# xaskasdf/ntransformer

Measured on AMD Instinct MI355X. Metric: decode tokens/sec (Llama-3.1-8B Q8_0 class, resident weights, greedy, batch 1), higher is better.
Workload: dtype f32; 1 GPU; Llama-3.1-8B-shaped Q8_0 GGUF tensors (seed 20260925), resident in HBM, 16-token prompt, greedy decode; ctx=4096, replicas=1, hipgraph=True

## Files before the change

include/ntk_engine.h:

```cpp
#ifndef NTK_ENGINE_H
#define NTK_ENGINE_H

#include "ntk.h"

#if defined(__GNUC__)
#pragma GCC visibility push(default)
#endif
#ifdef __cplusplus
extern "C" {
#endif

int ntk_rope_kv_store(float* q, const float* k, const float* v, const int* positions, int seq_len, int n_heads, int n_kv_heads, int head_dim,
                      float theta_base, float freq_scale, int interleaved, void* k_cache, void* v_cache, int start_pos, int max_seq, void* stream);
typedef struct ntk_gemv_seg {
    const void* W;
    float*      y;
    int         rows;
    int         dtype;
} ntk_gemv_seg;

int ntk_gemv_fused(const ntk_gemv_seg* segs, int nseg, const float* x, int in_features, const float* norm_w,
                   float eps, const float* resid, int silu_pair, void* stream);

size_t ntk_q8l_bytes(int rows, int in_features);
int ntk_q8l_pack(void* dst, const void* raw, int rows, int in_features, void* stream);
int ntk_q8l_unpack(void* raw, const void* packed, int rows, int in_features, void* stream);

size_t ntk_rp_bytes(int dtype, int rows, int in_features);
int ntk_rp_pack(void* dst, const void* raw, int rows, int in_features, int dtype, void* stream);
int ntk_rp_dequant(float* out, const void* rp, int rows, int in_features, int dtype, void* stream);
int ntk_rp_unpack(void* raw, const void* rp, int rows, int in_features, int dtype, void* stream);
int ntk_gemv_rp(float* y, const void* rp, const float* x, int out_features, int in_features, int weight_dtype, void* stream);
int ntk_gemv_rp_fused(const ntk_gemv_seg* segs, int nseg, const float* x, int in_features, const float* norm_w, float eps,
                      const float* resid, int silu_pair, void* stream);
int ntk_debug_rp_prologue(uint8_t* out, const float* x, const float* norm_w, float eps, int in_features, int nsub, int nwaves, void* stream);
int ntk_debug_mfma_i8_probe(int* D, const int8_t* A, const int8_t* B, void* stream);

int ntk_attention_decode_fused(float* output, const float* q, const float* k, const float* v, void* k_cache,
                               void* v_cache, const int* d_pos, const float* inv_freq, int n_heads, int n_kv_heads,
                               int head_dim, int max_seq, float scale, float theta_base, float freq_scale,
                               void* stream);

size_t ntk_attention_split_scratch_bytes(int n_heads, int head_dim, int nsplit);
int ntk_attention_decode_split(float* output, const float* q, const float* k, const float* v, void* k_cache,
                               void* v_cache, const int* d_pos, const float* inv_freq, int n_heads, int n_kv_heads,
                               int head_dim, int max_seq, float scale, float theta_base, float freq_scale, int nsplit,
                               float* scratch, void* stream);
int ntk_attention_split_scratch_init(float* scratch, int n_heads, void* stream);
int ntk_attention_decode_split_merged(float* output, const float* q, const float* k, const float* v, void* k_cache,
                                      void* v_cache, const int* d_pos, const float* inv_freq, int n_heads, int n_kv_heads,
                                      int head_dim, int max_seq, float scale, float theta_base, float freq_scale, int nsplit,
                                      float* scratch, void* stream);

#define NTK_ATTN_BATCH_MAX 16
typedef struct ntk_kv_batch {
    void* k[NTK_ATTN_BATCH_MAX];
    void* v[NTK_ATTN_BATCH_MAX];
} ntk_kv_batch;
int ntk_attention_decode_batch(float* output, const float* q, const float* k, const float* v, const ntk_kv_batch* caches, const int* positions,
                               int n_rows, const float* inv_freq, int n_heads, int n_kv_heads, int head_dim, int max_seq, float scale,
                               float theta_base, float freq_scale, int nsplit, float* scratch, void* stream);

typedef struct ntk_kv_segments {
    int   n_seg;
    int   row0[NTK_ATTN_BATCH_MAX];
    int   n_rows[NTK_ATTN_BATCH_MAX];
    int   start_pos[NTK_ATTN_BATCH_MAX];
    void* k[NTK_ATTN_BATCH_MAX];
    void* v[NTK_ATTN_BATCH_MAX];
} ntk_kv_segments;
int ntk_kv_segments_validate(const ntk_kv_segments* segs, int total_rows, int max_seq);
int ntk_rope_kv_store_segments(float* q, const float* k, const float* v, const ntk_kv_segments* segs, int n_heads, int n_kv_heads, int head_dim,
                               float theta_base, float freq_scale, int interleaved, int max_seq, void* stream);
int ntk_attention_prefill_segments(float* output, const float* Q, const ntk_kv_segments* segs, int n_heads, int n_kv_heads, int head_dim, int max_seq,
                                   float scale, void* stream);

size_t ntk_kv_q8_cache_bytes(int max_seq, int n_kv_heads, int head_dim);
int ntk_kv_store_q8(void* k_cache, void* v_cache, const float* k, const float* v, int seq_len, int n_kv_heads, int head_dim, int start_pos,
                    int max_seq, void* stream);
int ntk_rope_kv_store_q8(float* q, const float* k, const float* v, const int* positions, int seq_len, int n_heads, int n_kv_heads, int head_dim,
                         float theta_base, float freq_scale, int interleaved, void* k_cache, void* v_cache, int start_pos, int max_seq,
                         void* stream);
int ntk_attention_decode_q8(float* output, const float* q, const float* k, const float* v, void* k_cache, void* v_cache, const int* d_pos,
                            const float* inv_freq, int n_heads, int n_kv_heads, int head_dim, int max_seq, float scale, float theta_base,
                            float freq_scale, int nsplit, float* scratch, void* stream);
int ntk_kv_dequant_q8_f16(void* k_f16, void* v_f16, const void* k_cache, const void* v_cache, int n_rows, int n_kv_heads, int head_dim,
                          int max_seq, void* stream);
int ntk_attention_decode_q8_batch(float* output, const float* q, const float* k, const float* v, const ntk_kv_batch* caches, const int* positions,
                                  int n_rows, const float* inv_freq, int n_heads, int n_kv_heads, int head_dim, int max_seq, float scale,
                                  float theta_base, float freq_scale, int nsplit, float* scratch, void* stream);

int ntk_kv_shift(uint16_t* k_cache, uint16_t* v_cache, int n_layers, int max_seq, int n_kv_heads, int head_dim, int src0, int dst0, int n_rows,
                 const float* inv_freq, float theta_base, float freq_scale, int interleaved, void* stream);
int ntk_kv_shift_q8(void* k_cache_q8, void* v_cache_q8, int n_layers, int max_seq, int n_kv_heads, int head_dim, int src0, int dst0, int n_rows,
                    const float* inv_freq, float theta_base, float freq_scale, int interleaved, void* stream);

int ntk_debug_gemv_fused_form(const ntk_gemv_seg* segs, int nseg, const float* x, int in_features, const float* norm_w, float eps,
                              const float* resid, int silu_pair, int integer_activations, void* stream);

size_t   ntk_tp_comm_bytes(size_t max_floats);
void*    ntk_tp_comm_alloc(size_t bytes);
int      ntk_tp_comm_reset(void* comm, void* stream);
float*   ntk_tp_slot(void* comm, size_t max_floats, unsigned call_index);
int      ntk_tp_allreduce_add(float* hidden, void* const* peers, int rank, int world, size_t max_floats, unsigned call_index, int n, void* stream);
int      ntk_tp_advance_epoch(void* comm, void* stream);
unsigned ntk_tp_error(void* comm);
int      ntk_ipc_export(void* devptr, void* handle64);
int      ntk_ipc_open(const void* handle64, void** devptr);
int      ntk_ipc_close(void* devptr);

int ntk_gemm_quant(float* Y, const void* W, const float* X, int n_tokens, int out_features, int in_features,
                   int weight_dtype, const float* resid, void* stream);

typedef struct ntk_gemm_partials {
    const float* part[3];
    float*       y[3];
    int          rows[3];
    int          nseg, n_tokens, nsplit;
} ntk_gemm_partials;
typedef struct ntk_gemm_desc {
    const ntk_gemv_seg* segs;
    int                 nseg;
    const float*        X;
    int                 n_tokens, in_features;
    const float*        resid;
    void*               workspace;
    size_t              workspace_bytes;
    int                 reuse_x;
    const float*        row_max;
    ntk_gemm_partials*  partials;
    int                 weights_repacked;
    int                 full_form;
} ntk_gemm_desc;
size_t ntk_gemm_quant_workspace_bytes(int in_features, int out_features);
int ntk_gemm_quant_f16(const ntk_gemm_desc* desc, void* stream);
int ntk_reduce_rmsnorm_rowmax(float* hidden, const ntk_gemm_partials* partials, const float* weight, float eps, float* x_out, float* row_max,
                              float* zero_tokens, void* stream);
int ntk_reduce_silu_mul_rowmax(float* output, const ntk_gemm_partials* partials, float* row_max, void* stream);
int ntk_rmsnorm_rowmax(float* output, const float* input, const float* weight, int n_tokens, int hidden_size, float eps, float* row_max,
                       float* zero_tokens, void* stream);
int ntk_silu_mul_rowmax(float* output, const float* gate, const float* up, int n_tokens, int width, float* row_max, void* stream);
int ntk_gemm_prepare_x(const float* X, int n_tokens, int in_features, void* workspace, void* stream);
int ntk_rmsnorm_prepare_x(float* output, const float* input, const float* weight, int n_tokens, int hidden_size, float eps, void* workspace, void* stream);
int ntk_reduce_rmsnorm_prepare_x(float* hidden, const ntk_gemm_partials* partials, const float* weight, float eps, float* x_out, void* workspace, void* stream);
int ntk_silu_mul_prepare_x(float* output, const float* gate, const float* up, int n_tokens, int width, void* workspace, void* stream);
int ntk_reduce_silu_mul_prepare_x(float* output, const ntk_gemm_partials* partials, void* workspace, void* stream);

int ntk_embed_rows(float* out, const void* table, const int* tokens, int n_tokens, int hidden, int dtype,
                   void* stream);

int ntk_argmax(const float* logits, int n, int* d_out_token, int* h_mirror, float* scratch, void* stream);

int ntk_logprob_rows(const float* logits, int n_rows, int vocab, int ld, const int* targets, float* logprob, int* top1, void* stream);

size_t ntk_sample_scratch_bytes(int n);
int ntk_sample_top_k(float* logits, int n, const int* d_recent, int n_recent, float repeat_penalty, float temperature,
                     int top_k, float top_p, float r, int* d_out_token, int* h_mirror, void* scratch, void* stream);
int ntk_repeat_penalty(float* logits, int n, const int* d_recent, int n_recent, float repeat_penalty, void* stream);

#define NTK_SAMPLE_ROWS_MAX 16
typedef struct ntk_sample_rows {
    float temperature[NTK_SAMPLE_ROWS_MAX], top_p[NTK_SAMPLE_ROWS_MAX], repeat_penalty[NTK_SAMPLE_ROWS_MAX], r[NTK_SAMPLE_ROWS_MAX];
    int   top_k[NTK_SAMPLE_ROWS_MAX], n_recent[NTK_SAMPLE_ROWS_MAX];
} ntk_sample_rows;
size_t ntk_sample_rows_scratch_bytes(int n_rows, int vocab);
int ntk_sample_rows_top_k(float* logits, int n_rows, int vocab, int ld, const int* d_recent, int recent_ld, const ntk_sample_rows* rows, int* d_out,
                          int* h_mirror, void* scratch, void* stream);

int ntk_argmax_advance(const float* logits, int n, int* d_out_token, int* h_mirror, unsigned long long* h_ring4, int* d_pos,
                       float* scratch, void* stream);

int ntk_debug_sclk(unsigned long long* d_out2, void* stream);
int ntk_debug_sclk_begin(unsigned* d_flag, unsigned long long* d_out2, void* side_stream);
int ntk_debug_sclk_end(unsigned* d_flag, void* other_stream);

void ntk_debug_malloc_budget(long long bytes);

int ntk_advance_pos(int* d_pos, void* stream);

#ifdef __cplusplus
}
#endif
#if defined(__GNUC__)
#pragma GCC visibility pop
#endif
#endif
```

ntransformer_amd/_lib.py:

```python
from __future__ import annotations

import ctypes as C
import os

_HERE = os.path.dirname(os.path.abspath(__file__))
LIB_PATH = os.environ.get("NTK_LIB_PATH") or os.path.join(_HERE, "libntransformer_hip.so")

NTK_OK = 0
_STATUS = {0: "ok", -1: "unsupported dtype", -2: "bad shape", -3: "HIP launch/runtime error", -4: "misaligned pointer",
           -5: "null pointer", -6: "no usable GPU", -7: "out of memory", -8: "I/O error", -9: "malformed GGUF"}


class NtkError(RuntimeError):
    def __init__(self, status: int, what: str = ""):
        self.status = status
        super().__init__("ntk status %d (%s)%s" % (status, _STATUS.get(status, "?"), (": " + what) if what else ""))


def check(status: int, what: str = "") -> None:
    if status != NTK_OK:
        raise NtkError(status, what)


class KvBatch(C.Structure):
    _fields_ = [("k", C.c_void_p * 16), ("v", C.c_void_p * 16)]


class KvSegments(C.Structure):
    _fields_ = [("n_seg", C.c_int), ("row0", C.c_int * 16), ("n_rows", C.c_int * 16), ("start_pos", C.c_int * 16), ("k", C.c_void_p * 16),
                ("v", C.c_void_p * 16)]


class SampleRows(C.Structure):
    _fields_ = [("temperature", C.c_float * 16), ("top_p", C.c_float * 16), ("repeat_penalty", C.c_float * 16), ("r", C.c_float * 16),
                ("top_k", C.c_int * 16), ("n_recent", C.c_int * 16)]


class GemvSeg(C.Structure):
    _fields_ = [("W", C.c_void_p), ("y", C.c_void_p), ("rows", C.c_int), ("dtype", C.c_int)]


class GemmPartials(C.Structure):
    _fields_ = [("part", C.c_void_p * 3), ("y", C.c_void_p * 3), ("rows", C.c_int * 3), ("nseg", C.c_int), ("n_tokens", C.c_int), ("nsplit", C.c_int)]


class GemmDesc(C.Structure):
    _fields_ = [("segs", C.POINTER(GemvSeg)), ("nseg", C.c_int), ("X", C.c_void_p), ("n_tokens", C.c_int), ("in_features", C.c_int), ("resid", C.c_void_p),
                ("workspace", C.c_void_p), ("workspace_bytes", C.c_size_t), ("reuse_x", C.c_int), ("row_max", C.c_void_p),
                ("partials", C.POINTER(GemmPartials)), ("weights_repacked", C.c_int), ("full_form", C.c_int)]


_lib = None


def lib() -> C.CDLL:
    global _lib
    if _lib is not None:
        return _lib
    if not os.path.exists(LIB_PATH):
        raise ImportError("%s is missing: run `python -c 'import __graft_entry__ as g; g.build()'` "
                          "(hipcc --offload-arch=gfx950); there is no CPU fallback" % LIB_PATH)
    L = C.CDLL(LIB_PATH, mode=C.RTLD_GLOBAL)
    vp, i, f, sz = C.c_void_p, C.c_int, C.c_float, C.c_size_t
    sig = {
        "ntk_abi_version": (i, []),
        "ntk_status_string": (C.c_char_p, [i]),
        "ntk_row_bytes": (sz, [i, C.c_int64]),
        "ntk_device_count": (i, []),
        "ntk_device_init": (i, [i]),
        "ntk_device_name": (i, [C.c_char_p, sz]),
        "ntk_device_mem_info": (i, [C.POINTER(sz), C.POINTER(sz)]),
        "ntk_stream": (vp, [i]),
        "ntk_stream_synchronize": (i, [vp]),
        "ntk_device_synchronize": (i, []),
        "ntk_event_create": (vp, []),
        "ntk_event_destroy": (i, [vp]),
        "ntk_event_record": (i, [vp, vp]),
        "ntk_event_synchronize": (i, [vp]),
        "ntk_event_elapsed_ms": (i, [vp, vp, C.POINTER(f)]),
        "nt_hip_malloc": (vp, [sz]), "nt_hip_free": (None, [vp]),
        "nt_hip_memcpy_h2d": (None, [vp, vp, sz]), "nt_hip_memcpy_d2h": (None, [vp, vp, sz]),
        "nt_hip_memcpy_d2d": (None, [vp, vp, sz]), "nt_hip_memset": (None, [vp, i, sz]),
        "nt_hip_malloc_host": (vp, [sz]), "nt_hip_free_host": (None, [vp]),
        "ntk_memcpy_h2d_async": (i, [vp, vp, sz, vp]), "ntk_memcpy_d2h_async": (i, [vp, vp, sz, vp]),
        "nt_cuda_malloc": (vp, [sz]), "nt_cuda_free": (None, [vp]),
        "nt_cuda_memcpy_h2d": (None, [vp, vp, sz]), "nt_cuda_memcpy_d2h": (None, [vp, vp, sz]),
        "nt_cuda_memcpy_d2d": (None, [vp, vp, sz]), "nt_cuda_memset": (None, [vp, i, sz]),
        "nt_cuda_malloc_host": (vp, [sz]), "nt_cuda_free_host": (None, [vp]),
        "ntk_rmsnorm": (i, [vp, vp, vp, i, i, f, vp]),
        "ntk_rmsnorm_f16": (i, [vp, vp, vp, i, i, f, vp]),
        "ntk_rope": (i, [vp, vp, vp, i, i, i, i, i, f, f, i, vp]),
        "ntk_softmax": (i, [vp, vp, i, i, vp]),
        "ntk_masked_softmax": (i, [vp, vp, vp, i, i, vp]),
        "ntk_gemv": (i, [vp, vp, vp, i, i, i, vp]),
        "ntk_gemv_add": (i, [vp, vp, vp, i, i, i, vp]),
        "ntk_gemm_f32": (i, [vp, vp, vp, i, i, i, vp]),
        "ntk_silu_mul": (i, [vp, vp, vp, i, vp]),
        "ntk_rmsnorm_rowmax": (i, [vp, vp, vp, i, i, f, vp, vp, vp]),
        "ntk_rope_kv_store": (i, [vp, vp, vp, vp, i, i, i, i, f, f, i, vp, vp, i, i, vp]),
        "ntk_silu_mul_rowmax": (i, [vp, vp, vp, i, i, vp, vp]),
        "ntk_add_bias": (i, [vp, vp, i, vp]),
        "ntk_attention_decode": (i, [vp, vp, vp, vp, i, i, i, i, i, f, vp]),
        "ntk_attention_prefill": (i, [vp, vp, vp, vp, i, i, i, i, i, i, f, vp]),
        "ntk_copy_to_kv_cache": (i, [vp, vp, vp, vp, i, i, i, i, i, vp]),
        "ntk_add": (i, [vp, vp, vp, i, vp]),
        "ntk_add_inplace": (i, [vp, vp, i, vp]),
        "ntk_copy": (i, [vp, vp, i, vp]),
        "ntk_cosine_similarity": (i, [vp, vp, vp, i, vp]),
        "ntk_gemv_fused": (i, [C.POINTER(GemvSeg), i, vp, i, vp, f, vp, i, vp]),
        "ntk_debug_gemv_fused_form": (i, [C.POINTER(GemvSeg), i, vp, i, vp, f, vp, i, i, vp]),
        "ntk_q8l_bytes": (sz, [i, i]),
        "ntk_q8l_pack": (i, [vp, vp, i, i, vp]),
        "ntk_q8l_unpack": (i, [vp, vp, i, i, vp]),
        "ntk_rp_bytes": (sz, [i, i, i]),
        "ntk_rp_pack": (i, [vp, vp, i, i, i, vp]),
        "ntk_rp_dequant": (i, [vp, vp, i, i, i, vp]),
        "ntk_rp_unpack": (i, [vp, vp, i, i, i, vp]),
        "ntk_gemv_rp": (i, [vp, vp, vp, i, i, i, vp]),
        "ntk_gemv_rp_fused": (i, [C.POINTER(GemvSeg), i, vp, i, vp, f, vp, i, vp]),
        "ntk_debug_rp_prologue": (i, [vp, vp, vp, f, i, i, i, vp]),
        "ntk_debug_mfma_i8_probe": (i, [vp, vp, vp, vp]),
        "ntk_gemm_quant": (i, [vp, vp, vp, i, i, i, i, vp, vp]),
        "ntk_attention_decode_split": (i, [vp, vp, vp, vp, vp, vp, vp, vp, i, i, i, i, f, f, f, i, vp, vp]),
        "ntk_attention_split_scratch_bytes": (C.c_size_t, [i, i, i]),
        "ntk_attention_split_scratch_init": (i, [vp, i, vp]),
        "ntk_attention_decode_split_merged": (i, [vp, vp, vp, vp, vp, vp, vp, vp, i, i, i, i, f, f, f, i, vp, vp]),
        "ntk_attention_decode_fused": (i, [vp, vp, vp, vp, vp, vp, vp, vp, i, i, i, i, f, f, f, vp]),
        "ntk_attention_decode_batch": (i, [vp, vp, vp, vp, vp, vp, i, vp, i, i, i, i, f, f, f, i, vp, vp]),
        "ntk_kv_segments_validate": (i, [vp, i, i]),
        "ntk_rope_kv_store_segments": (i, [vp, vp, vp, vp, i, i, i, f, f, i, i, vp]),
        "ntk_attention_prefill_segments": (i, [vp, vp, vp, i, i, i, i, f, vp]),
        "ntk_kv_q8_cache_bytes": (C.c_size_t, [i, i, i]),
        "ntk_kv_store_q8": (i, [vp, vp, vp, vp, i, i, i, i, i, vp]),
        "ntk_rope_kv_store_q8": (i, [vp, vp, vp, vp, i, i, i, i, f, f, i, vp, vp, i, i, vp]),
        "ntk_attention_decode_q8": (i, [vp, vp, vp, vp, vp, vp, vp, vp, i, i, i, i, f, f, f, i, vp, vp]),
        "ntk_kv_dequant_q8_f16": (i, [vp, vp, vp, vp, i, i, i, i, vp]),
        "ntk_attention_decode_q8_batch": (i, [vp, vp, vp, vp, vp, vp, i, vp, i, i, i, i, f, f, f, i, vp, vp]),
        "ntk_kv_shift": (i, [vp, vp, i, i, i, i, i, i, i, vp, f, f, i, vp]),
        "ntk_kv_shift_q8": (i, [vp, vp, i, i, i, i, i, i, i, vp, f, f, i, vp]),
        "ntk_embed_rows": (i, [vp, vp, vp, i, i, i, vp]),
        "ntk_argmax": (i, [vp, i, vp, vp, vp, vp]),
        "ntk_logprob_rows": (i, [vp, i, i, i, vp, vp, vp, vp]),
        "ntk_sample_rows_scratch_bytes": (C.c_size_t, [i, i]),
        "ntk_sample_rows_top_k": (i, [vp, i, i, i, vp, i, C.POINTER(SampleRows), vp, vp, vp, vp]),
        "ntk_advance_pos": (i, [vp, vp]),
        "ntk_debug_sclk": (i, [vp, vp]),
        "ntk_debug_sclk_begin": (i, [vp, vp, vp]),
        "ntk_debug_sclk_end": (i, [vp, vp]),
    }
    for name, (res, args) in sig.items():
        fn = getattr(L, name)
        fn.restype = res
        fn.argtypes = args
    _lib = L
    return L


EXPORTS_NTK_H = None
```

ntransformer_amd/csrc/engine/capi.cpp:

```cpp
#include "../../../include/ntransformer.h"
#include "../../../include/ntk_engine.h"
#include "engine.h"

#include <cstdlib>
#include <cstring>
#include <new>
#include <thread>

using nt::Engine;

namespace {
Engine* E(nt_engine_t e) { return static_cast<Engine*>(e); }
nt::SynthSpec to_spec(const nt_synth_spec& s) {
    nt::SynthSpec o;
    o.hidden = s.hidden; o.inter = s.inter; o.layers = s.layers; o.heads = s.heads; o.kv_heads = s.kv_heads;
    o.vocab = s.vocab; o.ctx = s.ctx; o.eps = s.eps; o.theta = s.theta; o.bos = s.bos; o.eos = s.eos;
    o.mix = s.mix ? s.mix : "Q8_0";
    o.seed = s.seed;
    return o;
}
int threads_or_default(int n) {
    if (n > 0) return n;
    const int h = (int)std::thread::hardware_concurrency();
    return h > 0 ? h : 8;
}
}

extern "C" {

nt_engine_t nt_engine_create(void) { return new (std::nothrow) Engine(); }
void nt_engine_destroy(nt_engine_t e) { delete E(e); }

int nt_engine_load(nt_engine_t e, const char* path) { return nt_engine_load_ex(e, path, 4096); }

int nt_engine_load_ex(nt_engine_t e, const char* path, int max_context) {
    if (!e || !path) return NTK_E_NULL;
    try { return E(e)->load(path, max_context > 0 ? max_context : 4096); } catch (...) { return NTK_E_NOMEM; }
}

int nt_engine_load_synthetic(nt_engine_t e, const nt_synth_spec* spec, int max_context) {
    if (!e || !spec) return NTK_E_NULL;
    try { return E(e)->load_synthetic(to_spec(*spec), max_context > 0 ? max_context : 4096); } catch (...) { return NTK_E_NOMEM; }
}

int nt_engine_load_shared(nt_engine_t e, nt_engine_t src, int max_context) {
    if (!e || !src || e == src) return NTK_E_NULL;
    try { return E(e)->load_shared(*E(src), max_context > 0 ? max_context : 4096); } catch (...) { return NTK_E_NOMEM; }
}

int nt_engine_set_option(nt_engine_t e, const char* key, const char* value) {
    if (!e || !key || !value) return NTK_E_NULL;
    const bool on = atoi(value) != 0;
    const std::string k = key;
    if (k == "fused") E(e)->options().fused = on;
    else if (k == "graph") E(e)->options().graph = on;
    else if (k == "batched_prefill") { E(e)->options().batched_prefill = on; E(e)->model().set_batched_prefill(on); }
    else if (k == "device_sampling") E(e)->options().device_sampling = on;
    else if (k == "f16_prefill" || k == "bf16_prefill") E(e)->model().set_bf16_prefill(on);
    else if (k == "fuse_attention") { const int rc = E(e)->model().set_fuse_attention(on); if (rc != NTK_OK) E(e)->set_error(E(e)->model().error()); return rc; }
    else if (k == "kv_cache") {
        const int rc = E(e)->loaded() ? (E(e)->set_error("kv_cache must be set before the model is loaded"), NTK_E_SHAPE) : E(e)->model().set_kv_cache(value);
        if (rc != NTK_OK && !E(e)->loaded()) E(e)->set_error(E(e)->model().error());
        return rc;
    }
    else if (k == "sequences") {
        const int rc = E(e)->loaded() ? (E(e)->set_error("sequences must be set before the model is loaded"), NTK_E_SHAPE) : E(e)->model().set_sequences(atoi(value));
        if (rc != NTK_OK && !E(e)->loaded()) E(e)->set_error(E(e)->model().error());
        return rc;
    }
    else if (k == "batch_kv_q8") {
        const std::string v = value;
        if (v != "0" && v != "1") { E(e)->set_error("batch_kv_q8 must be 0 or 1"); return NTK_E_SHAPE; }
        const int rc = E(e)->loaded() ? (E(e)->set_error("batch_kv_q8 must be set before the model is loaded"), NTK_E_SHAPE) : E(e)->model().set_batch_kv_q8(on);
        if (rc != NTK_OK && !E(e)->loaded()) E(e)->set_error(E(e)->model().error());
        return rc;
    }
    else if (k == "batch_prefill") {
        const std::string v = value;
        if (v != "0" && v != "1") { E(e)->set_error("batch_prefill must be 0 or 1"); return NTK_E_SHAPE; }
        E(e)->options().batch_prefill = on;
    }
    else if (k == "context_shift") {
        const std::string v = value;
        if (v != "0" && v != "1") { E(e)->set_error("context_shift must be 0 or 1"); return NTK_E_SHAPE; }
        E(e)->options().context_shift = on;
    }
    else if (k == "context_keep") {
        char* end = nullptr;
        const long n = strtol(value, &end, 10);
        if (end == value || *end != 0 || n < 0 || n > 0x7FFFFFFF) { E(e)->set_error("context_keep must be an integer >= 0"); return NTK_E_SHAPE; }
        E(e)->options().context_keep = (int)n;
    }
    else if (k == "prefill_row_max") E(e)->model().set_prefill_row_max(on);
    else if (k == "prefill_fused_split") E(e)->model().set_prefill_fused_split(on);
    else if (k == "attention_merge") return E(e)->model().set_attention_merge(on);
    else if (k == "repack") return E(e)->model().set_repack(atoi(value));
    else if (k == "persistent") { E(e)->options().persistent = on; E(e)->model().set_persistent(atoi(value)); }
    else if (k == "score_rows") {
        const int rc = E(e)->model().set_score_rows(atoi(value));
        if (rc != NTK_OK) E(e)->set_error(E(e)->model().error());
        return rc;
    }
    else if (k == "synth_threads") E(e)->options().synth_threads = atoi(value);
    else return NTK_E_SHAPE;
    return NTK_OK;
}

const char* nt_engine_last_error(nt_engine_t e) { return e ? E(e)->error().c_str() : "null engine"; }

void nt_gen_params_default(nt_gen_params* p) {
    if (!p) return;
    const nt::GenerateConfig d;
    p->max_tokens = d.max_tokens; p->temperature = d.temperature; p->top_k = d.top_k; p->top_p = d.top_p;
    p->repeat_penalty = d.repeat_penalty; p->repeat_window = d.repeat_window; p->seed = d.seed; p->stop_at_eos = 1;
}

char* nt_engine_generate(nt_engine_t e, const char* prompt, int max_tokens, float temperature, int top_k, float top_p) {
    if (!e || !prompt || !E(e)->loaded()) return nullptr;
    try {
        nt::GenerateConfig c;
        c.max_tokens = max_tokens; c.temperature = temperature; c.top_k = top_k; c.top_p = top_p;
        c.verbose = false;
        const std::string out = E(e)->generate(prompt, c);
        char* r = static_cast<char*>(malloc(out.size() + 1));
        if (!r) return nullptr;
        memcpy(r, out.c_str(), out.size() + 1);
        return r;
    } catch (...) { return nullptr; }
}
void nt_free(char* p) { free(p); }

int nt_engine_vocab_size(nt_engine_t e) { return e && E(e)->loaded() ? E(e)->model().config().vocab_size : -1; }
int nt_engine_n_layers(nt_engine_t e) { return e && E(e)->loaded() ? E(e)->model().config().n_layers : -1; }
int nt_engine_hidden_size(nt_engine_t e) { return e && E(e)->loaded() ? E(e)->model().config().hidden_size : -1; }
int nt_engine_max_context(nt_engine_t e) { return e && E(e)->loaded() ? E(e)->model().config().max_seq_len : -1; }

int nt_engine_generate_tokens(nt_engine_t e, const int* prompt, int n_prompt, const nt_gen_params* p, int* out, int out_cap) {
    if (!e || !prompt || !p || (!out && out_cap > 0)) return NTK_E_NULL;
    if (n_prompt <= 0) return NTK_E_SHAPE;
    try {
        nt::GenerateConfig c;
        c.max_tokens = p->max_tokens; c.temperature = p->temperature; c.top_k = p->top_k; c.top_p = p->top_p;
        c.repeat_penalty = p->repeat_penalty; c.repeat_window = p->repeat_window; c.seed = p->seed;
        std::vector<int> gen;
        const int rc = E(e)->generate_tokens(std::vector<int>(prompt, prompt + n_prompt), c, gen, p->stop_at_eos != 0);
        if (rc != NTK_OK) return rc;
        const int n = (int)std::min<size_t>(gen.size(), (size_t)out_cap);
        for (int i = 0; i < n; ++i) out[i] = gen[i];
        return n;
    } catch (...) { return NTK_E_NOMEM; }
}

int nt_engine_last_stats(nt_engine_t e, nt_stats* o) {
    if (!e || !o) return NTK_E_NULL;
    const nt::Stats& s = E(e)->last_stats();
    o->prompt_tokens = s.prompt_tokens; o->gen_tokens = s.gen_tokens; o->prefill_ms = s.prefill_ms;
    o->decode_ms = s.decode_ms; o->decode_tok_s = s.decode_tok_s();
    return NTK_OK;
}

int nt_engine_forward(nt_engine_t e, const int* tokens, int n, int start_pos, float* logits_out) {
    if (!e || !tokens || !logits_out) return NTK_E_NULL;
    if (!E(e)->loaded()) return NTK_E_NULL;
    float* d = E(e)->model().forward(tokens, n, start_pos);
    if (!d) return NTK_E_LAUNCH;
    return E(e)->model().copy_logits(logits_out);
}

int nt_engine_seq_forward(nt_engine_t e, int slot, const int* tokens, int n, int start_pos, float* logits_out) {
    if (!e || !tokens || !logits_out) return NTK_E_NULL;
    if (!E(e)->loaded()) return NTK_E_NULL;
    if (slot < 0 || slot >= E(e)->model().sequences()) { E(e)->set_error("seq_forward: no such sequence slot"); return NTK_E_SHAPE; }
    float* d = E(e)->model().forward(tokens, n, start_pos, slot);
    if (!d) { E(e)->set_error(E(e)->model().error()); return NTK_E_LAUNCH; }
    return E(e)->model().copy_logits(logits_out);
}

int nt_engine_decode_batch(nt_engine_t e, const int* slots, const int* tokens, const int* positions, int n, float* logits_out, int* next_out) {
    if (!e || !E(e)->loaded()) return NTK_E_NULL;
    try {
        const int rc = E(e)->model().decode_batch(slots, tokens, positions, n, logits_out, next_out);
        if (rc != NTK_OK) E(e)->set_error(E(e)->model().error());
        return rc;
    } catch (...) { return NTK_E_NOMEM; }
}

int nt_engine_forward_batch(nt_engine_t e, const int* slots, const int* tokens, const int* lens, const int* start_pos, int n, float* logits_out,
                            int* next_out) {
    if (!e || !E(e)->loaded()) return NTK_E_NULL;
    try {
        E(e)->model().set_batched_prefill(E(e)->options().batched_prefill);
        const int rc = E(e)->model().forward_batch(slots, tokens, lens, start_pos, n, logits_out, next_out);
        if (rc != NTK_OK) E(e)->set_error(E(e)->model().error());
        return rc;
    } catch (...) { return NTK_E_NOMEM; }
}

int nt_forward_batch_validate(const int* slots, const int* lens, const int* start_pos, int n, int sequences, int max_seq) {
    return nt::Model::validate_forward_batch(slots, lens, start_pos, n, sequences, max_seq, nullptr);
}

int nt_engine_generate_batch(nt_engine_t e, const int* const* prompts, const int* prompt_lens, int n, const nt_gen_params* p, int* out, int out_stride,
                             int* out_counts) {
    if (!e || !prompts || !prompt_lens || !p || !out || !out_counts) return NTK_E_NULL;
    try { return E(e)->generate_batch(prompts, prompt_lens, n, *p, out, out_stride, out_counts); } catch (...) { return NTK_E_NOMEM; }
}

int nt_engine_decode_batch_sample(nt_engine_t e, const int* slots, const int* tokens, const int* positions, int n, const nt_gen_params* params,
                                  const int* const* recent, const int* n_recent, const float* r, float* logits_out, int* next_out) {
    if (!e || !E(e)->loaded()) return NTK_E_NULL;
    try { return E(e)->decode_batch_sample(slots, tokens, positions, n, params, recent, n_recent, r, logits_out, next_out); } catch (...) { return NTK_E_NOMEM; }
}

int nt_engine_generate_batch_ex(nt_engine_t e, const int* const* prompts, const int* prompt_lens, int n, const nt_gen_params* params, int* out, int out_stride,
                                int* out_counts) {
    if (!e || !prompts || !prompt_lens || !params || !out || !out_counts) return NTK_E_NULL;
    try { return E(e)->generate_batch_ex(prompts, prompt_lens, n, params, out, out_stride, out_counts); } catch (...) { return NTK_E_NOMEM; }
}

int nt_engine_kv_shift(nt_engine_t e, int slot, int keep, int discard, int n_past) {
    if (!e || !E(e)->loaded()) return NTK_E_NULL;
    try {
        const int rc = E(e)->model().kv_shift(slot, keep, discard, n_past);
        if (rc < 0) E(e)->set_error(E(e)->model().error());
        return rc;
    } catch (...) { return NTK_E_NOMEM; }
}

int nt_engine_kv_copy(nt_engine_t e, int src_slot, int dst_slot, int pos0, int n) {
    if (!e || !E(e)->loaded()) return NTK_E_NULL;
    try {
        const int rc = E(e)->model().kv_copy(src_slot, dst_slot, pos0, n);
        if (rc < 0) E(e)->set_error(E(e)->model().error());
        return rc;
    } catch (...) { return NTK_E_NOMEM; }
}

int nt_kv_shift_validate(int slot, int keep, int discard, int n_past, int sequences, int max_seq) {
    return nt::Model::validate_kv_shift(slot, keep, discard, n_past, sequences, max_seq, nullptr);
}
int nt_kv_copy_validate(int src_slot, int dst_slot, int pos0, int n, int sequences, int max_seq) {
    return nt::Model::validate_kv_copy(src_slot, dst_slot, pos0, n, sequences, max_seq, nullptr);
}
int nt_context_shift_discard(int n_past, int keep) { return nt::Model::context_shift_discard(n_past, keep); }

int nt_batch_validate(const int* slots, const int* tokens, const int* positions, int n, int sequences, int max_seq, int vocab) {
    return nt::Model::validate_batch(slots, tokens, positions, n, sequences, max_seq, vocab, nullptr);
}

int nt_engine_score_tokens(nt_engine_t e, const int* tokens, const int* targets, int n, int start_pos, float* logprob_out, int* top1_out) {
    if (!e || !tokens || !targets || !logprob_out) return NTK_E_NULL;
    try {
        const int rc = E(e)->score(tokens, targets, n, start_pos, logprob_out, top1_out);
        if (rc != NTK_OK) return rc;
        int scored = 0;
        for (int i = 0; i < n; ++i) scored += targets[i] >= 0;
        return scored;
    } catch (...) { return NTK_E_NOMEM; }
}

int nt_engine_decode_fused(nt_engine_t e, int token, int pos, int use_graph, float* logits_out) {
    if (!e || !logits_out || !E(e)->loaded()) return NTK_E_NULL;
    nt::Model& m = E(e)->model();
    if (pos < 0 || pos >= m.config().max_seq_len) return NTK_E_SHAPE;
    m.set_device_pos(pos);
    int rc = m.set_device_token(token);
    if (rc != NTK_OK) return rc;
    rc = m.decode_step_fused(false, use_graph != 0);
    if (rc != NTK_OK) return rc;
    rc = m.copy_logits(logits_out);
    if (rc != NTK_OK) return rc;
    return m.check_persistent();
}

int nt_engine_debug_run_layers(nt_engine_t e, const float* hidden_in, int n_tokens, int start_pos, int first_layer, int n_layers, int mode,
                               float* hidden_out) {
    if (!e || !E(e)->loaded()) return NTK_E_NULL;
    return E(e)->model().debug_run_layers(hidden_in, n_tokens, start_pos, first_layer, n_layers, mode, hidden_out);
}
int nt_engine_debug_kv_read(nt_engine_t e, int layer, int pos0, int n, uint16_t* k_out, uint16_t* v_out) {
    if (!e || !E(e)->loaded()) return NTK_E_NULL;
    return E(e)->model().debug_kv(layer, pos0, n, k_out, v_out, false);
}
int nt_engine_debug_kv_read_slot(nt_engine_t e, int slot, int layer, int pos0, int n, uint16_t* k_out, uint16_t* v_out) {
    if (!e || !E(e)->loaded()) return NTK_E_NULL;
    return E(e)->model().debug_kv(layer, pos0, n, k_out, v_out, false, slot);
}
int nt_engine_debug_kv_write(nt_engine_t e, int layer, int pos0, int n, const uint16_t* k, const uint16_t* v) {
    if (!e || !E(e)->loaded()) return NTK_E_NULL;
    return E(e)->model().debug_kv(layer, pos0, n, const_cast<uint16_t*>(k), const_cast<uint16_t*>(v), true);
}
int nt_engine_debug_kv_write_slot(nt_engine_t e, int slot, int layer, int pos0, int n, const uint16_t* k, const uint16_t* v) {
    if (!e || !E(e)->loaded()) return NTK_E_NULL;
    return E(e)->model().debug_kv(layer, pos0, n, const_cast<uint16_t*>(k), const_cast<uint16_t*>(v), true, slot);
}
int nt_engine_debug_kv_inputs_capture(nt_engine_t e, int layer) {
    if (!e || !E(e)->loaded()) return NTK_E_NULL;
    return E(e)->model().debug_kv_inputs_capture(layer);
}
int nt_engine_debug_kv_inputs_read(nt_engine_t e, int n, float* k_out, float* v_out) {
    if (!e || !E(e)->loaded()) return NTK_E_NULL;
    return E(e)->model().debug_kv_inputs_read(n, k_out, v_out);
}
int nt_engine_debug_kv_read_q8(nt_engine_t e, int layer, int pos0, int n, void* k_blocks, void* v_blocks) {
    if (!e || !E(e)->loaded()) return NTK_E_NULL;
    return E(e)->model().debug_kv_q8(layer, pos0, n, static_cast<uint8_t*>(k_blocks), static_cast<uint8_t*>(v_blocks), false);
}
int nt_engine_debug_kv_write_q8(nt_engine_t e, int layer, int pos0, int n, const void* k_blocks, const void* v_blocks) {
    if (!e || !E(e)->loaded()) return NTK_E_NULL;
    return E(e)->model().debug_kv_q8(layer, pos0, n, static_cast<uint8_t*>(const_cast<void*>(k_blocks)), static_cast<uint8_t*>(const_cast<void*>(v_blocks)), true);
}
int nt_engine_debug_kv_read_q8_slot(nt_engine_t e, int slot, int layer, int pos0, int n, void* k_blocks, void* v_blocks) {
    if (!e || !E(e)->loaded()) return NTK_E_NULL;
    return E(e)->model().debug_kv_q8(layer, pos0, n, static_cast<uint8_t*>(k_blocks), static_cast<uint8_t*>(v_blocks), false, slot);
}
int nt_engine_debug_kv_write_q8_slot(nt_engine_t e, int slot, int layer, int pos0, int n, const void* k_blocks, const void* v_blocks) {
    if (!e || !E(e)->loaded()) return NTK_E_NULL;
    return E(e)->model().debug_kv_q8(layer, pos0, n, static_cast<uint8_t*>(const_cast<void*>(k_blocks)), static_cast<uint8_t*>(const_cast<void*>(v_blocks)), true, slot);
}

void* nt_engine_persistent_plan(nt_engine_t e) { return e && E(e)->loaded() ? E(e)->model().persistent_plan() : nullptr; }
int nt_engine_persistent_kind(nt_engine_t e) { return e && E(e)->loaded() ? E(e)->model().persistent_kind() : 0; }
const char* nt_engine_decode_path(nt_engine_t e) { return e && E(e)->loaded() ? E(e)->model().decode_path() : ""; }

int nt_engine_tp_configure(nt_engine_t e, int rank, int world) { return e ? E(e)->model().tp_configure(rank, world) : NTK_E_NULL; }
int nt_engine_tp_export(nt_engine_t e, void* handle64, void** raw) {
    if (!e || !E(e)->loaded()) return NTK_E_NULL;
    return E(e)->model().tp_export(handle64, raw);
}
int nt_engine_tp_connect(nt_engine_t e, const void* handles, void* const* raws) {
    if (!e || !E(e)->loaded()) return NTK_E_NULL;
    return E(e)->model().tp_connect(handles, raws);
}
unsigned nt_engine_tp_error(nt_engine_t e) { return e && E(e)->loaded() ? E(e)->model().tp_error() : 0u; }
int nt_tp_slice_columns(void* dst, const void* src, int dtype, int64_t out_features, int64_t in_features, int rank, int world) {
    return nt::Model::slice_columns(dst, src, dtype, out_features, in_features, rank, world);
}

int nt_engine_decode_greedy_steps(nt_engine_t e, int token, int pos, int n, int* out) {
    if (!e || !E(e)->loaded()) return NTK_E_NULL;
    return E(e)->decode_greedy_steps(token, pos, n, out);
}

int nt_engine_profile_token(nt_engine_t e, int token, int pos, int coarse, float* ms4, int* calls4) {
    if (!e || !ms4 || !calls4 || !E(e)->loaded()) return NTK_E_NULL;
    nt::Model& m = E(e)->model();
    if (pos < 0 || pos >= m.config().max_seq_len) return NTK_E_SHAPE;
    m.set_device_pos(pos);
    const int rc = m.set_device_token(token);
    if (rc != NTK_OK) return rc;
    return m.profile_token(ms4, calls4, coarse != 0);
}

int nt_engine_tokenize(nt_engine_t e, const char* text, int add_bos, int* out, int cap) {
    if (!e || !text || !E(e)->loaded()) return NTK_E_NULL;
    const std::vector<int> ids = E(e)->tokenizer().encode(text, add_bos != 0);
    for (int i = 0; i < (int)ids.size() && i < cap; ++i) out[i] = ids[i];
    return (int)ids.size();
}

int nt_engine_detokenize(nt_engine_t e, const int* ids, int n, char* out, int cap) {
    if (!e || !ids || !E(e)->loaded()) return NTK_E_NULL;
    const std::string s = E(e)->tokenizer().decode(std::vector<int>(ids, ids + n));
    if (out && cap > 0) {
        const size_t k = std::min<size_t>(s.size(), (size_t)cap - 1);
        memcpy(out, s.data(), k);
        out[k] = 0;
    }
    return (int)s.size();
}

uint64_t nt_engine_bytes_per_token(nt_engine_t e, int pos) { return e && E(e)->loaded() ? E(e)->model().bytes_per_token(pos) : 0; }
uint64_t nt_engine_kv_cache_bytes(nt_engine_t e) { return e && E(e)->loaded() ? E(e)->model().kv_cache_bytes() : 0; }
uint64_t nt_engine_weight_bytes(nt_engine_t e) { return e && E(e)->loaded() ? E(e)->model().weight_bytes() : 0; }
uint64_t nt_engine_resident_weight_bytes(nt_engine_t e) { return e && E(e)->loaded() ? E(e)->model().resident_weight_bytes() : 0; }
uint64_t nt_engine_repacked_bytes(nt_engine_t e) { return e && E(e)->loaded() ? E(e)->model().repack_bytes() : 0; }
// ... 137 lines not shown
```

ntransformer_amd/csrc/engine/model.cpp:

```cpp
#include "model_impl.h"
#include <thread>

namespace nt {

Model::~Model() { free_all(); }

void Model::drop_graphs(int slot) {
    for (auto& row : graphs_)
        for (int k = 0; k <= kAttnRegimes; ++k) {
            if (slot >= 0 && k != slot) continue;
            if (row[k]) (void)hipGraphExecDestroy(reinterpret_cast<hipGraphExec_t>(row[k]));
            row[k] = nullptr;
        }
}

void Model::free_all() {
    drop_graphs();
    destroy_persistent_plan();
    persistent_on_ = false;
    for (int r = 0; r < 8; ++r) {
        if (tp_peer_opened_[r] && tp_peers_[r]) (void)ntk_ipc_close(tp_peers_[r]);
        tp_peers_[r] = nullptr;
        tp_peer_opened_[r] = false;
    }
    tp_connected_ = false;
    tp_comm_ = nullptr;
    tp_call_ = 0;
    if (own_stream_ && stream_) (void)hipStreamDestroy(static_cast<hipStream_t>(stream_));
    own_stream_ = false;
    stream_ = nullptr;
    for (void* p : allocs_) nt_hip_free(p);
    allocs_.clear();
    auto free_host = [](auto*& p) { if (p) nt_hip_free_host(p); p = nullptr; };
    free_host(h_token_); free_host(h_ring_); free_host(h_recent_); free_host(h_batch_recent_); free_host(h_batch_next_);
    sample_scratch_ = gemm_ws_ = gemm_ws2_ = nullptr;
    d_recent_ = nullptr;
    attn_sync_ = nullptr;
    shares_weights_ = false;
    layers_.clear();
    token_embd_ = output_norm_ = output_ = DevTensor();
    weight_bytes_ = repack_bytes_ = raw_freed_bytes_ = 0;
    raw_scratch_ = nullptr; raw_scratch_bytes_ = raw_cursor_ = 0; raw_err_ = 0;
    repack_done_ = output_tied_ = false;
    host_pos_ = attn_regime_ = 0;
    kv_.reset();
    batch_logits_ = batch_logprob_ = batch_attn_scratch_ = nullptr; batch_in_ = batch_next_ = batch_recent_ = nullptr; batch_sample_scratch_ = nullptr;
    kv_capture_ = nullptr; kv_capture_layer_ = -1; kv_capture_T_ = 0;
    hidden_ = residual_ = workspace_ = logits_ = argmax_scratch_ = rope_inv_freq_ = attn_scratch_ = row_max_ = nullptr;
    positions_ = tokens_dev_ = d_pos_ = d_token_ = nullptr;
    score_logits_ = score_logprob_ = nullptr; score_targets_ = score_top1_ = nullptr; score_cap_ = 0;
    score_ws_ = nullptr; score_ws_bytes_ = 0;
}

int Model::share_weights(const Model& src, int max_context) {
    if (&src == this) { err_ = "share_weights: a model cannot share its own weights"; return NTK_E_NULL; }
    free_all();
    if (src.layers_.empty()) { err_ = "share_weights: the source model is not loaded"; return NTK_E_NULL; }
    if (src.tp_world_ != 1 || src.shares_weights_) {
        err_ = "share_weights: the source must hold whole tensors of its own (no tensor parallelism, not itself a sharing sequence)";
        return NTK_E_SHAPE;
    }
    cfg_ = src.cfg_;
    cfg_full_ = src.cfg_;
    if (max_context > 0) cfg_.max_seq_len = max_context;
    vocab_ = src.vocab_;
    layers_ = src.layers_;
    token_embd_ = src.token_embd_; output_norm_ = src.output_norm_; output_ = src.output_;
    output_tied_ = src.output_tied_;
    weight_bytes_ = src.weight_bytes_;
    repack_ = src.repack_; repack_wanted_ = src.repack_; repack_done_ = true;
    repack_bytes_ = 0;
    shares_weights_ = true;
    if (src.raw_freed_bytes_ > 0 && src.raw_scratch_bytes_ > 0) {
        void* d = nt_hip_malloc(src.raw_scratch_bytes_);
        if (!d) { err_ = "share_weights: no device memory for the unpack scratch"; free_all(); return NTK_E_NOMEM; }
        allocs_.push_back(d);
        raw_scratch_ = d; raw_scratch_bytes_ = src.raw_scratch_bytes_;
        raw_freed_bytes_ = src.raw_freed_bytes_;
    }
    int rc = own_stream();
    if (rc == NTK_OK) rc = alloc_buffers();
    if (rc != NTK_OK) free_all();
    return rc;
}

int Model::set_attention_merge(bool on) {
    if (on == attn_merge_) return NTK_OK;
    if (!layers_.empty()) {
        NT_TRY(sync());
        drop_graphs();
    }
    attn_merge_ = on;
    return NTK_OK;
}

int Model::set_repack(int level) {
    level = level < 0 ? 0 : level > 3 ? 3 : level;
    if (shares_weights_) { err_ = "set_repack: this sequence shares another model's tensors"; return NTK_E_SHAPE; }
    repack_wanted_ = level;
    if (layers_.empty()) { repack_ = level; return NTK_OK; }
    if (level == 3) level = 2;
    if (level == repack_) return NTK_OK;
    NT_TRY(sync());
    drop_graphs();
    int rc = NTK_OK;
    if (level < 2 && raw_freed_bytes_ > 0) rc = restore_raw_all();
    if (rc == NTK_OK && level > 0 && !repack_done_) {
        rc = repack_all();
        if (rc == NTK_E_NOMEM) { fprintf(stderr, "warning: decode repack incomplete (device memory): the rest stays on the raw path\n"); rc = NTK_OK; err_.clear(); }
    }
    if (rc != NTK_OK) { err_ = std::string("set_repack: ") + ntk_status_string(rc); return rc; }
    repack_ = level;
    if (level == 2) {
        destroy_persistent_plan();
        persistent_on_ = false;
        rc = drop_raw_all();
    }
    return rc;
}

uint64_t Model::bytes_per_token(int pos) const {
    uint64_t b = 0;
    for (const auto& L : layers_)
        for (auto m : kLayerMatrices) b += (L.*m).nbytes;
    b += output_.nbytes;
    b += (uint64_t)(2 * cfg_.n_layers + 1) * cfg_.hidden_size * 4;
    const uint64_t kv_row = kv_.row_bytes();
    b += 2ull * cfg_.n_layers * kv_row * (uint64_t)(pos + 1) + 2ull * cfg_.n_layers * kv_row;
    b += ntk_row_bytes(token_embd_.dtype, cfg_.hidden_size);
    return b;
}

int Model::set_device_token(int token) {
    if (token < 0 || token >= cfg_.vocab_size) { err_ = "token id out of range"; return NTK_E_SHAPE; }
    *h_token_ = token;
    return ntk_memcpy_h2d_async(d_token_, h_token_, 4, stream_);
}
int Model::set_device_pos(int pos) {
    host_pos_ = pos;
    NT_TRY(ntk_memcpy_h2d_async(d_pos_, &pos, 4, stream_));
    NT_TRY(ntk_stream_synchronize(stream_));
    if (h_ring_) memset(h_ring_, 0, 64);
    return NTK_OK;
}
int Model::sync() { return ntk_stream_synchronize(stream_); }
int Model::host_token() const { return *h_token_; }
int Model::copy_logits(float* host) {
    NT_TRY(ntk_memcpy_d2h_async(host, logits_, (size_t)cfg_.vocab_size * 4, stream_));
    return ntk_stream_synchronize(stream_);
}

int Model::sample_on_device(const int* recent, int n_recent, float repeat_penalty, float temperature, int top_k, float top_p, float r) {
    if (!sample_scratch_ || !d_recent_ || !h_recent_) return NTK_E_NOMEM;
    if (n_recent > kRecentCap) { recent += n_recent - kRecentCap; n_recent = kRecentCap; }
    void* s = stream_;
    if (repeat_penalty > 1.0f && n_recent > 0) {
        memcpy(h_recent_, recent, (size_t)n_recent * 4);
        NT_TRY(ntk_memcpy_h2d_async(d_recent_, h_recent_, (size_t)n_recent * 4, s));
    } else {
        n_recent = 0;
    }
    if (temperature <= 0.0f) {
        NT_TRY(ntk_repeat_penalty(logits_, cfg_.vocab_size, d_recent_, n_recent, repeat_penalty, s));
        return ntk_argmax(logits_, cfg_.vocab_size, d_token_, h_token_, argmax_scratch_, s);
    }
    return ntk_sample_top_k(logits_, cfg_.vocab_size, d_recent_, n_recent, repeat_penalty, temperature, top_k, top_p, r, d_token_,
                            h_token_, sample_scratch_, s);
}

int Model::wait_token(int pos, int* token) {
    volatile unsigned long long* slot = h_ring_ + (pos & 3);
    const unsigned want = (unsigned)(pos + 1);
    for (unsigned spins = 0;; ++spins) {
        const unsigned long long v = *slot;
        if ((unsigned)(v >> 32) == want) { *token = (int)(unsigned)v; return NTK_OK; }
#if defined(__x86_64__) || defined(__i386__)
        __builtin_ia32_pause();
#else
        std::this_thread::yield();
#endif
        if ((spins & 0xFFFFu) == 0xFFFFu) {
            const auto now = std::chrono::steady_clock::now();
            if (spins == 0xFFFFu) wait_t0_ = now;
            else if (std::chrono::duration<double>(now - wait_t0_).count() > 2.0) break;
        }
    }
    static bool warned = false;
    if (!warned) { warned = true; fprintf(stderr, "warning: the pinned token ring was not seen updating for 2 s (host memory not coherent with a running kernel?); falling back to a stream synchronisation per token\n"); }
    NT_TRY(ntk_stream_synchronize(stream_));
    const unsigned long long v = *slot;
    if ((unsigned)(v >> 32) != want) { err_ = "decode step finished without publishing its token"; return NTK_E_LAUNCH; }
    *token = (int)(unsigned)v;
    return NTK_OK;
}

int Model::set_sequences(int n) {
    if (n < 1 || n > kMaxSequences) { err_ = "sequences must lie in 1 .. " + std::to_string(kMaxSequences); return NTK_E_SHAPE; }
    sequences_ = n;
    return NTK_OK;
}

int Model::set_batch_kv_q8(bool on) {
    if (!layers_.empty()) { err_ = "batch_kv_q8 must be set before the model is loaded"; return NTK_E_SHAPE; }
    batch_kv_q8_ = on;
    return NTK_OK;
}

int Model::set_kv_cache(const std::string& kind) {
    if (kind != "f16" && kind != "q8_0") { err_ = "kv_cache: unknown format '" + kind + "' (f16 or q8_0)"; return NTK_E_DTYPE; }
    if (!layers_.empty()) { err_ = "kv_cache must be set before the model is loaded"; return NTK_E_SHAPE; }
    const bool q8 = kind == "q8_0";
    if (q8 && fuse_attention_) { err_ = "kv_cache=q8_0 is not supported with the attention-inside-Wo launch (fuse_attention)"; return NTK_E_SHAPE; }
    kv_q8_ = q8;
    return NTK_OK;
}

int Model::set_fuse_attention(bool on) {
    if (on && kv_q8_) { err_ = "fuse_attention (attention inside the Wo launch) is not supported with kv_cache=q8_0"; return NTK_E_SHAPE; }
    fuse_attention_ = on;
    return NTK_OK;
}

bool Model::use_persistent_now() const {
    return persistent_plan_ && persistent_on_ && attn_regime_ == 0 && !prof_;
}

void Model::set_persistent(int level) {
    const bool on = level != 0;
    persistent_on_ = false;
    persistent_wanted_ = level;
    if (on && !experiments_built()) fprintf(stderr, "note: the persistent token kernels are built by experiments/Makefile only (experiments/libntransformer_hip_exp.so); this library decodes with fused launches\n");
    if (persistent_plan_ && persistent_kind_ != (level == 2 ? 2 : 1)) {
        (void)sync();
        destroy_persistent_plan();
    }
    if (!on || tp_world_ != 1 || layers_.empty()) return;
    if (kv_q8_) { fprintf(stderr, "note: the persistent token kernels read the F16 KV cache; kv_cache=q8_0 decodes with fused launches\n"); return; }
    if (raw_freed_bytes_ > 0) (void)set_repack(1);
    if (!persistent_plan_) (void)build_persistent_plan(level == 2 ? 2 : 1);
    persistent_on_ = persistent_plan_ != nullptr;
}

const char* Model::decode_path() const {
    if (persistent_plan_ && persistent_on_ && persistent_kind_ == 2)
        return attn_regime_ == 0 ? "persistent layer engine (1 launch per token: loader / consumer waves, granule hand-offs; fused launches beyond the single-pass attention regime)"
                                 : "fused (5 launches/layer; persistent layer engine below the split-attention regime)";
    if (persistent_plan_ && persistent_on_)
        return attn_regime_ == 0 ? "persistent (1 launch per token in the single-pass attention regime, fused launches beyond)"
                                 : "fused (5 launches/layer; persistent below the split-attention regime)";
    return "fused (5 launches/layer)";
}

int Model::check_persistent() {
    NT_TRY(check_tp());
    return check_experiments();
}

Model::Views Model::views(int T) const {
    const size_t qd = (size_t)T * cfg_.n_heads * cfg_.head_dim, kvd = (size_t)T * cfg_.n_kv_heads * cfg_.head_dim;
    float* const q = workspace_;
    return {q, q + qd, q + qd + kvd, q + qd + 2 * kvd, workspace_, workspace_ + (size_t)T * cfg_.intermediate_size};
}

int Model::init_device() {
    const char* e = getenv("NTK_DEVICE");
    const int st = ntk_device_init(e ? atoi(e) : 0);
    if (st != NTK_OK) err_ = "no usable GPU (HIP device init failed)";
    return st;
}

int Model::own_stream() {
    hipStream_t own = nullptr;
    if (hipStreamCreateWithFlags(&own, hipStreamNonBlocking) != hipSuccess) { err_ = "stream creation failed"; return NTK_E_LAUNCH; }
    stream_ = own;
    own_stream_ = true;
    return NTK_OK;
}

}
```

ntransformer_amd/csrc/engine/model.h:

```cpp
#pragma once
#include <algorithm>
#include <array>
#include <chrono>
#include <cstdint>
#include <string>
#include <vector>
#include "gguf.h"
#include "kv_cache.h"
#include "synth.h"

struct ntk_sample_rows;
struct ntk_kv_segments;

struct ihipGraphExec_t;

namespace nt {

struct DevTensor {
    void* ptr = nullptr;
    int dtype = 0;
    int64_t in_f = 0, out_f = 0;
    size_t nbytes = 0;
    void* rp = nullptr;
    size_t rp_bytes = 0;
};

struct LayerWeights {
    DevTensor attn_norm, wq, wk, wv, wo, ffn_norm, w_gate, w_up, w_down;
};
inline constexpr std::array<DevTensor LayerWeights::*, 7> kLayerMatrices = {&LayerWeights::wq, &LayerWeights::wk, &LayerWeights::wv, &LayerWeights::wo,
                                                                            &LayerWeights::w_gate, &LayerWeights::w_up, &LayerWeights::w_down};

enum Shard { WHOLE, ROWS, COLS };

class Model {
public:
    Model() = default;
    ~Model();
    Model(const Model&) = delete;
    Model& operator=(const Model&) = delete;

    int load(const std::string& gguf_path, int max_context);
    int load_synthetic(const SynthSpec& spec, int max_context, int nthreads);
    int share_weights(const Model& src, int max_context);

    float* forward(const int* tokens, int seq_len, int start_pos, int slot = 0);

    int score(const int* tokens, const int* targets, int seq_len, int start_pos, float* logprob_out, int* top1_out, int slot = 0);

    static constexpr int kMaxSequences = 16;
    int set_sequences(int n);
    int sequences() const { return sequences_; }
    int set_batch_kv_q8(bool on);
    bool batch_kv_q8() const { return batch_kv_q8_; }
    int decode_batch(const int* slots, const int* tokens, const int* positions, int B, float* logits_out, int* next_out);
    static constexpr int kMaxRecent = 4096;
    int decode_batch_sample(const int* slots, const int* tokens, const int* positions, int B, const ntk_sample_rows& rows, const int* const* recent,
                            float* logits_out, float* const* row_logits, int* next_out);
    static int validate_batch(const int* slots, const int* tokens, const int* positions, int B, int sequences, int max_seq, int vocab, std::string* why);
    int forward_batch(const int* slots, const int* tokens_flat, const int* lens, const int* start_pos, int n, float* logits_out, int* next_out);
    static int validate_forward_batch(const int* slots, const int* lens, const int* start_pos, int n, int sequences, int max_seq, std::string* why);
    int kv_shift(int slot, int keep, int discard, int n_past);
    int kv_copy(int src_slot, int dst_slot, int pos0, int n);
    static int validate_kv_shift(int slot, int keep, int discard, int n_past, int sequences, int max_seq, std::string* why);
    static int validate_kv_copy(int src_slot, int dst_slot, int pos0, int n, int sequences, int max_seq, std::string* why);
    static int context_shift_discard(int n_past, int keep) { return std::max(1, (n_past - keep) / 2); }
    int set_score_rows(int rows);

    int decode_step_fused(bool greedy, bool use_graph);
    int set_device_token(int token);
    int set_device_pos(int pos);
    static constexpr int kAttnRegimes = 3;
    static int attention_regime(int pos, int head_dim) {
        if (pos < 544) return 0;
        return pos < (head_dim == 128 ? 3072 : 16384) ? 1 : 2;
    }
    static int attention_splits(int regime, int head_dim) { return regime <= 1 ? 8 : head_dim == 128 ? 32 : 16; }
    static constexpr int kMaxAttnSplits = 32;
    void pick_attention_regime();
    int sync();
    int host_token() const;
    int wait_token(int pos, int* token);
    float* logits_ptr() { return logits_; }
    int copy_logits(float* host);
    int sample_on_device(const int* recent, int n_recent, float repeat_penalty, float temperature, int top_k, float top_p, float r);
    static bool device_sampler_supports(float temperature, int top_k, int vocab) {
        return temperature <= 0.0f || (top_k > 0 && top_k <= 64 && top_k < vocab && vocab <= 131072);
    }

    const ModelConfig& config() const { return cfg_; }
    const GgufVocab& vocab() const { return vocab_; }
    const std::string& error() const { return err_; }
    uint64_t weight_bytes() const { return weight_bytes_; }
    uint64_t bytes_per_token(int pos) const;
    void set_batched_prefill(bool on) { batched_prefill_ = on; }
    void set_persistent(int level);
    int persistent_kind() const { return persistent_plan_ ? persistent_kind_ : 0; }
    int set_fuse_attention(bool on);
    int set_kv_cache(const std::string& kind);
    bool kv_q8() const { return kv_q8_; }
    static int kv_q8_splits(int regime) { return regime == 0 ? 4 : regime == 1 ? 16 : 32; }
    uint64_t kv_cache_bytes() const { return kv_.bytes(); }
    int debug_kv_inputs_capture(int layer);
    int debug_kv_inputs_read(int n, float* k, float* v);
    int debug_kv_q8(int layer, int pos0, int n, uint8_t* k_blocks, uint8_t* v_blocks, bool write, int slot = 0);
    void set_prefill_row_max(bool on) { prefill_row_max_ = on; }
    void set_prefill_fused_split(bool on) { prefill_fused_split_ = on; }
    int set_attention_merge(bool on);
    int set_repack(int level);
    bool repack() const { return repack_ != 0; }
    int repack_level() const { return repack_; }
    uint64_t repack_bytes() const { return repack_bytes_; }
    uint64_t resident_weight_bytes() const { return weight_bytes_ - raw_freed_bytes_ + repack_bytes_ + raw_scratch_bytes_; }
    void set_bf16_prefill(bool on) { bf16_prefill_ = on; }
    bool persistent_available() const { return persistent_plan_ != nullptr; }
    void* persistent_plan() const { return persistent_plan_; }
    const char* decode_path() const;
    int check_persistent();
    int check_tp();
    int debug_run_layers(const float* hidden_in, int T, int start_pos, int first, int count, int mode, float* hidden_out);
    int debug_kv(int layer, int pos0, int n, uint16_t* k, uint16_t* v, bool write, int slot = 0);
    int profile_token(float ms[4], int calls[4], bool coarse);
    void* stream() const { return stream_; }

    int tp_configure(int rank, int world);
    int tp_rank() const { return tp_rank_; }
    int tp_world() const { return tp_world_; }
    int tp_export(void* handle64, void** raw);
    int tp_connect(const void* handles, void* const* raws);
    unsigned tp_error();
    static int slice_columns(void* dst, const void* src, int dtype, int64_t out_f, int64_t in_f, int rank, int world);

private:
    int load_impl(const std::string& gguf_path, int max_context);
    int finish_load();
    int init_device();
    int own_stream();
    int alloc_buffers();
    int upload(DevTensor& dst, const void* host, int dtype, int64_t in_f, int64_t out_f, size_t nbytes);
    int upload_shard(DevTensor& dst, const void* host_full, int dtype, int64_t in_f, int64_t out_f, size_t nbytes_full, Shard how);
    struct TensorSlot { DevTensor* dst; Shard how; int64_t in_f, out_f; };
    bool slot_of(const std::string& name, TensorSlot* slot);
    template <class F> void for_each_projection(F&& fn) { for (auto& L : layers_) for (auto m : kLayerMatrices) fn(L.*m); fn(output_); }
    int repack_all();
    int repack_one(DevTensor& t);
    int drop_raw_all();
    int restore_raw_all();
    void raw_begin() { raw_cursor_ = 0; }
    const void* raw_of(const DevTensor& t);
    int tp_check_shapes();
    int tp_allreduce(float* hidden, int n);
    float* tp_slot() const;
    void free_all();
    void drop_graphs(int slot = -1);
    struct Views { float *q, *k, *v, *attn_out, *gate, *up; };
    Views views(int T) const;
    int enqueue_token(bool greedy);
    int enqueue_layers(int first, int last);
    int decode_project(const DevTensor* const* ws, float* const* ys, int n, const float* x, const DevTensor* norm, const float* resid, int kind,
                       int silu_pair = 0, bool timed = true);
    struct KvTarget { int slot; const int* slots; int max_pos; const ntk_kv_segments* segs; };
    int layers_1to1(int T, int start_pos, int first, int last, const KvTarget& kv = KvTarget{0, nullptr, 0, nullptr});
    int lm_head(float* logits, const float* X, int n, const float* row_max);
    bool lm_head_f16() const;
    int lm_head_workspace(const char* who);
    int batch_buffers();
    int batch_logits(const int* slots, const int* tokens, const int* positions, int B);
    int batch_sample_buffers();
    int score_buffers();
    void prof_mark(int cls, bool begin);
    bool use_persistent_now() const;
    static bool experiments_built();
    int build_persistent_plan(int kind);
    void destroy_persistent_plan();
    int launch_persistent();
    int attention_in_wo(const LayerWeights& L, int layer);
    int check_experiments();

    ModelConfig cfg_;
    GgufVocab vocab_;
    std::string err_;
    std::vector<LayerWeights> layers_;
    DevTensor token_embd_, output_norm_, output_;
    bool output_tied_ = false;
    uint64_t weight_bytes_ = 0;
    std::vector<void*> allocs_;
    bool shares_weights_ = false;

    KvCache kv_;
    bool kv_q8_ = false;
    int sequences_ = 1;
    float* batch_logits_ = nullptr;
    int* batch_in_ = nullptr;
    int batch_host_[3 * 16] = {};
    std::vector<int> packed_tokens_;
    float* batch_logprob_ = nullptr;
    int* batch_next_ = nullptr;
    float* batch_attn_scratch_ = nullptr;
    int* batch_recent_ = nullptr;
    int* h_batch_recent_ = nullptr;
    void* batch_sample_scratch_ = nullptr;
    int* h_batch_next_ = nullptr;
    bool batch_kv_q8_ = false;
    float* kv_capture_ = nullptr;
    int kv_capture_layer_ = -1, kv_capture_T_ = 0;
    float* hidden_ = nullptr;
    float* residual_ = nullptr;
    float* workspace_ = nullptr;
    size_t workspace_floats_ = 0;
    float* logits_ = nullptr;
    int score_rows_ = 256;
    float* score_logits_ = nullptr;
    int score_cap_ = 0;
    int* score_targets_ = nullptr;
    float* score_logprob_ = nullptr;
    int* score_top1_ = nullptr;
    void* score_ws_ = nullptr;
    size_t score_ws_bytes_ = 0;
    int* positions_ = nullptr;
    int* tokens_dev_ = nullptr;
    int* d_pos_ = nullptr;
    int* d_token_ = nullptr;
    int* h_token_ = nullptr;
    unsigned long long* h_ring_ = nullptr;
    std::chrono::steady_clock::time_point wait_t0_;
    float* argmax_scratch_ = nullptr;
    void* sample_scratch_ = nullptr;
    int* d_recent_ = nullptr;
    int* h_recent_ = nullptr;
    static constexpr int kRecentCap = kMaxRecent;
    float* rope_inv_freq_ = nullptr;
    void* stream_ = nullptr;
    bool batched_prefill_ = true;
    struct Timed { int cls; void* a; void* b; int n; bool shared_a; };
    bool prof_coarse_ = false;
    std::vector<Timed>* prof_ = nullptr;
    static constexpr int kPersistentSlot = kAttnRegimes;
    ihipGraphExec_t* graphs_[2][kAttnRegimes + 1] = {};
    int host_pos_ = 0;
    int attn_regime_ = 0;
    float* attn_scratch_ = nullptr;
    bool prefill_row_max_ = true;
    float* row_max_ = nullptr;
    void* gemm_ws_ = nullptr;
    void* gemm_ws2_ = nullptr;
    bool prefill_fused_split_ = true;
    size_t gemm_ws_bytes_ = 0;
    bool bf16_prefill_ = true;
    unsigned* attn_sync_ = nullptr;
    int repack_ = 3;
    int repack_wanted_ = 3;
    bool repack_done_ = false;
    uint64_t repack_bytes_ = 0;
    uint64_t raw_freed_bytes_ = 0;
    void* raw_scratch_ = nullptr;
    size_t raw_scratch_bytes_ = 0, raw_cursor_ = 0;
    int raw_err_ = 0;
    bool attn_merge_ = false;
    bool fuse_attention_ = false;
    int tp_rank_ = 0, tp_world_ = 1;
    void* tp_comm_ = nullptr;
    size_t tp_max_floats_ = 0;
    void* tp_peers_[8] = {nullptr, nullptr, nullptr, nullptr, nullptr, nullptr, nullptr, nullptr};
    bool tp_peer_opened_[8] = {false, false, false, false, false, false, false, false};
    bool tp_connected_ = false;
    unsigned tp_call_ = 0;
    bool own_stream_ = false;
    ModelConfig cfg_full_;
    void* persistent_plan_ = nullptr;
    bool persistent_on_ = false;
    int persistent_wanted_ = 0;
    int persistent_kind_ = 1;
};

}
```

ntransformer_amd/csrc/engine/model_debug.cpp:

```cpp
#include "model_impl.h"

namespace nt {

int Model::debug_run_layers(const float* hidden_in, int T, int start_pos, int first, int count, int mode, float* hidden_out) {
    if (!hidden_in || !hidden_out) return NTK_E_NULL;
    if (T <= 0 || start_pos < 0 || start_pos + T > cfg_.max_seq_len || first < 0 || count < 0 || first + count > cfg_.n_layers) return NTK_E_SHAPE;
    if (mode != 0 && T != 1) return NTK_E_SHAPE;
    if (tp_world_ > 1) return NTK_E_SHAPE;
    const size_t bytes = (size_t)T * cfg_.hidden_size * 4;
    void* s = stream_;
    NT_TRY(ntk_memcpy_h2d_async(hidden_, hidden_in, bytes, s));
    int rc;
    if (mode == 0) {
        std::vector<int> pos(T);
        for (int i = 0; i < T; ++i) pos[i] = start_pos + i;
        NT_TRY(ntk_memcpy_h2d_async(positions_, pos.data(), (size_t)T * 4, s));
        NT_TRY(ntk_stream_synchronize(s));
        rc = layers_1to1(T, start_pos, first, first + count);
    } else {
        NT_TRY(set_device_pos(start_pos));
        pick_attention_regime();
        if (mode == 1) {
            rc = enqueue_layers(first, first + count);
        } else {
            hipStream_t st = static_cast<hipStream_t>(s);
            hipGraphExec_t ex = nullptr;
            rc = capture_graph(st, hipStreamCaptureModeThreadLocal, [&] { return enqueue_layers(first, first + count); }, &ex);
            if (rc == NTK_OK && hipGraphLaunch(ex, st) != hipSuccess) rc = NTK_E_LAUNCH;
            if (rc == NTK_OK) rc = ntk_stream_synchronize(s);
            if (ex) (void)hipGraphExecDestroy(ex);
        }
    }
    if (rc != NTK_OK) return rc;
    NT_TRY(ntk_memcpy_d2h_async(hidden_out, hidden_, bytes, s));
    return ntk_stream_synchronize(s);
}

int Model::debug_kv(int layer, int pos0, int n, uint16_t* k, uint16_t* v, bool write, int slot) {
    if (!k || !v) return NTK_E_NULL;
    if (kv_q8_) { err_ = "debug_kv: the KV cache is q8_0 (use the _q8 form)"; return NTK_E_DTYPE; }
    if (layer < 0 || layer >= cfg_.n_layers || pos0 < 0 || n < 0 || pos0 + n > cfg_.max_seq_len || slot < 0 || slot >= kv_.slots()) return NTK_E_SHAPE;
    KvRange r[2];
    kv_.row_ranges(pos0, n, r);
    uint8_t* const kd = static_cast<uint8_t*>(kv_.k(slot, layer)) + r[0].off;
    uint8_t* const vd = static_cast<uint8_t*>(kv_.v(slot, layer)) + r[0].off;
    void* s = stream_;
    NT_TRY(write ? ntk_memcpy_h2d_async(kd, k, r[0].bytes, s) : ntk_memcpy_d2h_async(k, kd, r[0].bytes, s));
    NT_TRY(write ? ntk_memcpy_h2d_async(vd, v, r[0].bytes, s) : ntk_memcpy_d2h_async(v, vd, r[0].bytes, s));
    return ntk_stream_synchronize(s);
}

int Model::debug_kv_q8(int layer, int pos0, int n, uint8_t* k_blocks, uint8_t* v_blocks, bool write, int slot) {
    if (!k_blocks || !v_blocks) return NTK_E_NULL;
    if (!kv_q8_) { err_ = "debug_kv_q8: the KV cache is f16"; return NTK_E_DTYPE; }
    if (layer < 0 || layer >= cfg_.n_layers || pos0 < 0 || n < 0 || pos0 + n > cfg_.max_seq_len || slot < 0 || slot >= kv_.slots()) return NTK_E_SHAPE;
    if (n == 0) return NTK_OK;
    const size_t nb = (size_t)cfg_.n_kv_heads * cfg_.head_dim / 32;
    KvRange r[2];
    kv_.row_ranges(pos0, n, r);
    const size_t qbytes = r[0].bytes, sbytes = r[1].bytes;
    void* s = stream_;
    std::vector<uint8_t> qh(qbytes), sh(sbytes);
    for (int side = 0; side < 2; ++side) {
        uint8_t* base = static_cast<uint8_t*>(side ? kv_.v(slot, layer) : kv_.k(slot, layer));
        uint8_t *qd = base + r[0].off, *sd = base + r[1].off;
        uint8_t* blocks = side ? v_blocks : k_blocks;
        if (write) {
            for (size_t b = 0; b < (size_t)n * nb; ++b) {
                memcpy(&sh[2 * b], blocks + 34 * b, 2);
                memcpy(&qh[32 * b], blocks + 34 * b + 2, 32);
            }
            NT_TRY(ntk_memcpy_h2d_async(qd, qh.data(), qbytes, s));
            NT_TRY(ntk_memcpy_h2d_async(sd, sh.data(), sbytes, s));
            NT_TRY(ntk_stream_synchronize(s));
        } else {
            NT_TRY(ntk_memcpy_d2h_async(qh.data(), qd, qbytes, s));
            NT_TRY(ntk_memcpy_d2h_async(sh.data(), sd, sbytes, s));
            NT_TRY(ntk_stream_synchronize(s));
            for (size_t b = 0; b < (size_t)n * nb; ++b) {
                memcpy(blocks + 34 * b, &sh[2 * b], 2);
                memcpy(blocks + 34 * b + 2, &qh[32 * b], 32);
            }
        }
    }
    return NTK_OK;
}

int Model::debug_kv_inputs_capture(int layer) {
    if (layers_.empty()) return NTK_E_NULL;
    if (layer >= cfg_.n_layers) return NTK_E_SHAPE;
    kv_capture_layer_ = layer < 0 ? -1 : layer;
    kv_capture_T_ = 0;
    if (layer >= 0 && !kv_capture_) {
        const size_t bytes = 2 * (size_t)cfg_.max_seq_len * cfg_.n_kv_heads * cfg_.head_dim * 4;
        kv_capture_ = (float*)nt_hip_malloc(bytes);
        if (!kv_capture_) { err_ = "debug_kv_inputs_capture: out of device memory"; return NTK_E_NOMEM; }
        allocs_.push_back(kv_capture_);
    }
    return NTK_OK;
}
int Model::debug_kv_inputs_read(int n, float* k, float* v) {
    if (!k || !v) return NTK_E_NULL;
    if (!kv_capture_ || kv_capture_layer_ < 0 || n < 0 || n > kv_capture_T_) return NTK_E_SHAPE;
    const size_t kvd = (size_t)cfg_.n_kv_heads * cfg_.head_dim;
    NT_TRY(ntk_memcpy_d2h_async(k, kv_capture_, (size_t)n * kvd * 4, stream_));
    NT_TRY(ntk_memcpy_d2h_async(v, kv_capture_ + (size_t)cfg_.max_seq_len * kvd, (size_t)n * kvd * 4, stream_));
    return ntk_stream_synchronize(stream_);
}

}
```

ntransformer_amd/csrc/engine/model_decode.cpp:

```cpp
#include "model_impl.h"

namespace nt {

void Model::prof_mark(int cls, bool begin) {
    if (!prof_) return;
    void* s = stream_;
    if (prof_coarse_) {
        if (!begin) return;
        if (!prof_->empty() && prof_->back().cls == cls) { ++prof_->back().n; return; }
        void* e = ntk_event_create();
        ntk_event_record(e, s);
        const bool shared = !prof_->empty();
        if (shared) prof_->back().b = e;
        prof_->push_back({cls, e, nullptr, 1, shared});
        return;
    }
    void* e = ntk_event_create();
    ntk_event_record(e, s);
    if (begin) prof_->push_back({cls, e, nullptr, 1, false}); else prof_->back().b = e;
}

int Model::enqueue_token(bool greedy) {
    const int H = cfg_.hidden_size;
    void* s = stream_;
    tp_call_ = 0;
    prof_mark(2, true);
    const int est = ntk_embed_rows(hidden_, token_embd_.ptr, d_token_, 1, H, token_embd_.dtype, s);
    prof_mark(2, false);
    if (est != NTK_OK && est != NTK_E_DTYPE) return est;
    if (use_persistent_now()) {
        NT_TRY(launch_persistent());
    } else {
        NT_TRY(enqueue_layers(0, cfg_.n_layers));
        const DevTensor* const w = &output_;
        const bool timed = is_quant(w->dtype);
        if (timed) prof_mark(0, true);
        NT_TRY(decode_project(&w, &logits_, 1, hidden_, &output_norm_, nullptr, 16, 0, false));
        if (timed) prof_mark(0, false);
    }
    prof_mark(2, true);
    if (greedy) NT_TRY(ntk_argmax_advance(logits_, cfg_.vocab_size, d_token_, h_token_, h_ring_, d_pos_, argmax_scratch_, s));
    else NT_TRY(ntk_advance_pos(d_pos_, s));
    if (tp_world_ > 1) NT_TRY(ntk_tp_advance_epoch(tp_comm_, s));
    prof_mark(2, false);
    return NTK_OK;
}

int Model::decode_project(const DevTensor* const* ws, float* const* ys, int n, const float* x, const DevTensor* norm, const float* resid, int kind,
                          int silu_pair, bool timed) {
    const int H = cfg_.hidden_size;
    void* s = stream_;
    auto mark = [&](bool begin) { if (timed) prof_mark(0, begin); };
    const float* nw = norm ? (const float*)norm->ptr : nullptr;
    auto one_launch = [&](bool rp, const float* r, int silu) {
        ntk_gemv_seg segs[3];
        if (!rp) raw_begin();
        for (int a = 0; a < n; ++a) segs[a] = {rp ? ws[a]->rp : raw_of(*ws[a]), ys[a], (int)ws[a]->out_f, ws[a]->dtype};
        mark(true);
        const int st = (rp ? ntk_gemv_rp_fused : ntk_gemv_fused)(segs, n, x, (int)ws[0]->in_f, nw, cfg_.norm_eps, r, silu, s);
        mark(false);
        return st;
    };
    bool all_rp = repack_ && (rp_mask() & kind), all_quant = true, mixed = false;
    for (int a = 0; a < n; ++a) {
        all_rp = all_rp && ws[a]->rp != nullptr && ws[a]->in_f == ws[0]->in_f;
        all_quant = all_quant && is_quant(ws[a]->dtype);
        mixed = mixed || ws[a]->dtype != ws[0]->dtype;
    }
    if (all_rp) {
        const int st = one_launch(true, resid, silu_pair);
        if (!not_taken(st)) return st;
    }
    if (n > 1 && !resid && all_quant && mixed) {
        const int st = one_launch(false, nullptr, 0);
        if (!not_taken(st)) return st;
    }
    bool done[3] = {false, false, false};
    for (int a = 0; a < n; ++a) {
        if (done[a]) continue;
        const DevTensor& w = *ws[a];
        if (!is_quant(w.dtype)) {
            const float* xin = x;
            if (nw) {
                NT_TRY(ntk_rmsnorm(residual_ + H, x, nw, 1, (int)w.in_f, cfg_.norm_eps, s));
                xin = residual_ + H;
            }
            float* y = resid ? residual_ : ys[a];
            raw_begin();
            NT_TRY(ntk_gemv(y, raw_of(w), xin, (int)w.out_f, (int)w.in_f, w.dtype, s));
            if (resid) NT_TRY(ntk_add(ys[a], resid, residual_, (int)w.out_f, s));
            done[a] = true;
            continue;
        }
        ntk_gemv_seg segs[3];
        int m = 0;
        raw_begin();
        for (int b = a; b < n; ++b) {
            if (done[b] || ws[b]->dtype != w.dtype) continue;
            segs[m++] = {raw_of(*ws[b]), ys[b], (int)ws[b]->out_f, ws[b]->dtype};
            done[b] = true;
        }
        mark(true);
        NT_TRY(ntk_gemv_fused(segs, m, x, (int)w.in_f, nw, cfg_.norm_eps, resid, silu_pair, s));
        mark(false);
    }
    return NTK_OK;
}

int Model::enqueue_layers(int first, int last_layer) {
    const int H = cfg_.hidden_size, I = cfg_.intermediate_size, hd = cfg_.head_dim, nh = cfg_.n_heads, nkv = cfg_.n_kv_heads;
    void* s = stream_;
    const float scale = 1.0f / sqrtf((float)hd);
    const Views act = views(1);
    auto project_add = [&](const DevTensor& w, const float* x, int kind) -> int {
        const DevTensor* const wp = &w;
        float* y = tp_world_ > 1 ? tp_slot() : hidden_;
        NT_TRY(decode_project(&wp, &y, 1, x, nullptr, tp_world_ > 1 ? nullptr : hidden_, kind));
        return tp_world_ > 1 ? tp_allreduce(hidden_, H) : (int)NTK_OK;
    };

    for (int i = first; i < last_layer; ++i) {
        const LayerWeights& L = layers_[i];
        const DevTensor* const qkv[3] = {&L.wq, &L.wk, &L.wv};
        float* const qkv_out[3] = {act.q, act.k, act.v};
        NT_TRY(decode_project(qkv, qkv_out, 3, hidden_, &L.attn_norm, nullptr, 1));
        const int fused = fuse_attention_ ? attention_in_wo(L, i) : (int)NTK_E_SHAPE;
        if (fused != NTK_OK) {
            if (!not_taken(fused)) return fused;
            prof_mark(1, true);
            if (kv_q8_)
                NT_TRY(ntk_attention_decode_q8(act.attn_out, act.q, act.k, act.v, kv_.k(0, i), kv_.v(0, i), d_pos_, rope_inv_freq_, nh, nkv, hd,
                                               cfg_.max_seq_len, scale, cfg_.rope_theta, cfg_.rope_freq_scale, kv_q8_splits(attn_regime_), attn_scratch_, s));
            else if (attn_regime_ == 0)
                NT_TRY(ntk_attention_decode_fused(act.attn_out, act.q, act.k, act.v, kv_.k_f16(0, i), kv_.v_f16(0, i), d_pos_, rope_inv_freq_, nh, nkv, hd,
                                                  cfg_.max_seq_len, scale, cfg_.rope_theta, cfg_.rope_freq_scale, s));
            else
                NT_TRY((attn_merge_ ? ntk_attention_decode_split_merged : ntk_attention_decode_split)(
                    act.attn_out, act.q, act.k, act.v, kv_.k_f16(0, i), kv_.v_f16(0, i), d_pos_, rope_inv_freq_, nh, nkv, hd, cfg_.max_seq_len, scale,
                    cfg_.rope_theta, cfg_.rope_freq_scale, attention_splits(attn_regime_, hd), attn_scratch_, s));
            prof_mark(1, false);
            NT_TRY(project_add(L.wo, act.attn_out, 2));
        }
        const DevTensor* const ffn[2] = {&L.w_gate, &L.w_up};
        float* const ffn_out[2] = {act.gate, act.up};
        const bool pair = is_quant(L.w_gate.dtype) && L.w_gate.dtype == L.w_up.dtype;
        if (pair) prof_mark(0, true);
        NT_TRY(decode_project(ffn, ffn_out, 2, hidden_, &L.ffn_norm, nullptr, 4, pair, !pair));
        if (pair) prof_mark(0, false);
        else NT_TRY(ntk_silu_mul(act.gate, act.gate, act.up, I, s));
        NT_TRY(project_add(L.w_down, act.gate, 8));
    }
    return NTK_OK;
}

void Model::pick_attention_regime() {
    attn_regime_ = (attn_scratch_ && (cfg_.head_dim == 64 || cfg_.head_dim == 128 || cfg_.head_dim == 256))
                       ? attention_regime(host_pos_, cfg_.head_dim) : 0;
    ++host_pos_;
}

int Model::decode_step_fused(bool greedy, bool use_graph) {
    pick_attention_regime();
    if (!use_graph) return enqueue_token(greedy);
    ihipGraphExec_t*& slot = graphs_[greedy ? 1 : 0][use_persistent_now() ? kPersistentSlot : attn_regime_];
    hipStream_t st = static_cast<hipStream_t>(stream_);
    if (!slot) {
        hipGraphExec_t ex = nullptr;
        NT_TRY(capture_graph(st, tp_world_ > 1 ? hipStreamCaptureModeRelaxed : hipStreamCaptureModeThreadLocal, [&] { return enqueue_token(greedy); }, &ex));
        slot = reinterpret_cast<ihipGraphExec_t*>(ex);
    }
    return hipGraphLaunch(reinterpret_cast<hipGraphExec_t>(slot), st) == hipSuccess ? NTK_OK : NTK_E_LAUNCH;
}

int Model::profile_token(float ms[4], int calls[4], bool coarse) {
    std::vector<Timed> rec;
    rec.reserve(1024);
    prof_ = &rec;
    prof_coarse_ = coarse;
    pick_attention_regime();
    int rc = enqueue_token(true);
    if (coarse && !rec.empty()) {
        void* e = ntk_event_create();
        ntk_event_record(e, stream_);
        rec.back().b = e;
    }
    prof_ = nullptr;
    prof_coarse_ = false;
    if (rc == NTK_OK) rc = ntk_stream_synchronize(stream_);
    for (int c = 0; c < 4; ++c) { ms[c] = 0.0f; calls[c] = 0; }
    for (auto& t : rec) {
        float m = 0.0f;
        if (t.a && t.b && ntk_event_elapsed_ms(t.a, t.b, &m) == NTK_OK) { ms[t.cls] += m; calls[t.cls] += t.n; }
        ++calls[3];
    }
    for (auto& t : rec) {
        if (t.a && !t.shared_a) ntk_event_destroy(t.a);
        if (t.b) ntk_event_destroy(t.b);
    }
    return rc;
}

}
```

ntransformer_amd/csrc/engine/model_load.cpp:

```cpp
#include "model_impl.h"

namespace nt {

int Model::upload(DevTensor& dst, const void* host, int dtype, int64_t in_f, int64_t out_f, size_t nbytes) {
    void* d = nt_hip_malloc(padded_bytes(nbytes));
    if (!d) { err_ = "out of device memory"; return NTK_E_NOMEM; }
    allocs_.push_back(d);
    if (host && nbytes) {
        if (hipMemcpy(d, host, nbytes, hipMemcpyHostToDevice) != hipSuccess) { err_ = "weight upload (H2D copy) failed"; return NTK_E_LAUNCH; }
    }
    dst.ptr = d; dst.dtype = dtype; dst.in_f = in_f; dst.out_f = out_f; dst.nbytes = nbytes;
    weight_bytes_ += nbytes;
    return NTK_OK;
}

int Model::slice_columns(void* dst, const void* src, int dtype, int64_t out_f, int64_t in_f, int rank, int world) {
    if (!dst || !src) return NTK_E_NULL;
    if (world < 1 || rank < 0 || rank >= world || in_f % world != 0) return NTK_E_SHAPE;
    const int64_t in_l = in_f / world;
    const size_t rb_full = ntk_row_bytes(dtype, in_f), rb_loc = ntk_row_bytes(dtype, in_l);
    if (!rb_full || !rb_loc || rb_loc * (size_t)world != rb_full) return NTK_E_SHAPE;
    const uint8_t* s8 = static_cast<const uint8_t*>(src);
    uint8_t* d8 = static_cast<uint8_t*>(dst);
    for (int64_t r = 0; r < out_f; ++r) memcpy(d8 + (size_t)r * rb_loc, s8 + (size_t)r * rb_full + (size_t)rank * rb_loc, rb_loc);
// ... 32 lines not shown
    const int st = load_impl(path, max_context);
    if (st != NTK_OK) free_all();
    return st;
}

int Model::load_impl(const std::string& path, int max_context) {
    free_all();
    fprintf(stderr, "Loading model: %s\n", path.c_str());
    GgufFile f;
    int st = f.open(path);
    if (st != NTK_OK) { err_ = f.error(); fprintf(stderr, "%s\n", err_.c_str()); return st; }
    cfg_ = f.config();
    vocab_ = f.vocab();
    if (cfg_.max_seq_len > max_context) {
        fprintf(stderr, "Note: Capping context from %d to %d tokens (use --ctx-size to change)\n", cfg_.max_seq_len, max_context);
        cfg_.max_seq_len = max_context;
    }
    cfg_.print();
    f.print_info();
    st = init_device();
    if (st != NTK_OK) { fprintf(stderr, "%s\n", err_.c_str()); return st; }

    NT_TRY(tp_check_shapes());
    auto take = [&](const std::string& name) -> int {
        const GgufTensor* t = f.find(name);
        TensorSlot sl;
        if (!t || !slot_of(name, &sl)) { err_ = "Tensor not found: " + name; return NTK_E_FORMAT; }
        const int64_t in_f = sl.in_f, out_f = sl.out_f;
        const bool vec = out_f == 1;
        if (t->numel() != in_f * out_f || (!vec && (t->dims.size() != 2 || t->dims[0] != in_f))) {
            err_ = "Unexpected shape for " + name;
            return NTK_E_SHAPE;
        }
        if (vec && t->dtype != NTK_DT_F32) { err_ = name + " must be F32"; return NTK_E_DTYPE; }
        if (t->nbytes == 0 || !t->known_type) { err_ = "Unsupported tensor type for " + name; return NTK_E_DTYPE; }
        return upload_shard(*sl.dst, f.data(*t), t->dtype, in_f, out_f, t->nbytes, sl.how);
    };
    layers_.resize(cfg_.n_layers);
    NT_TRY(take("token_embd.weight"));
    if (f.find("output.weight")) {
        NT_TRY(take("output.weight"));
    } else {
        output_ = token_embd_;
        output_tied_ = true;
    }
    NT_TRY(take("output_norm.weight"));
    for (int i = 0; i < cfg_.n_layers; ++i)
        for (const auto& e : kLayerTensors) NT_TRY(take("blk." + std::to_string(i) + "." + e.name));
    return finish_load();
}

bool Model::slot_of(const std::string& name, TensorSlot* sl) {
    const int64_t H = cfg_.hidden_size, hd = cfg_.head_dim;
    auto extent = [&](char c) -> int64_t { return c == 'h' ? H : c == 'q' ? cfg_.n_heads * hd : c == 'k' ? cfg_.n_kv_heads * hd : c == 'i' ? cfg_.intermediate_size : 1; };
    if (name == "token_embd.weight") { *sl = {&token_embd_, WHOLE, H, cfg_.vocab_size}; return true; }
    if (name == "output.weight") { *sl = {&output_, WHOLE, H, cfg_.vocab_size}; return true; }
    if (name == "output_norm.weight") { *sl = {&output_norm_, WHOLE, H, 1}; return true; }
    int li = -1, at = 0;
    if (sscanf(name.c_str(), "blk.%d.%n", &li, &at) != 1 || at == 0 || li < 0 || li >= (int)layers_.size()) return false;
    for (const auto& e : kLayerTensors)
        if (name.compare(at, std::string::npos, e.name) == 0) { *sl = {&(layers_[li].*e.member), e.how, extent(e.in), extent(e.out)}; return true; }
    return false;
}

int Model::load_synthetic(const SynthSpec& spec, int max_context, int nthreads) {
    free_all();
    std::vector<SynthTensor> plan;
    if (!synth_plan(spec, plan)) { err_ = "bad synthetic spec"; return NTK_E_SHAPE; }
    cfg_ = ModelConfig();
    cfg_.model_name = "synthetic-" + spec.mix;
    cfg_.vocab_size = spec.vocab; cfg_.hidden_size = spec.hidden; cfg_.intermediate_size = spec.inter;
    cfg_.n_layers = spec.layers; cfg_.n_heads = spec.heads; cfg_.n_kv_heads = spec.kv_heads;
    cfg_.head_dim = spec.hidden / spec.heads;
    cfg_.norm_eps = spec.eps; cfg_.rope_theta = spec.theta;
    cfg_.max_seq_len = std::min(spec.ctx, max_context);
    cfg_.bos_token_id = spec.bos; cfg_.eos_token_id = spec.eos;
    synth_vocab(spec, vocab_.tokens, vocab_.token_types);
    NT_TRY(init_device());
    NT_TRY(tp_check_shapes());

    size_t biggest = 0;
    for (const auto& t : plan) biggest = std::max(biggest, t.nbytes);
    void* stage = nt_hip_malloc_host(biggest);
    if (!stage) { err_ = "pinned staging allocation failed"; return NTK_E_NOMEM; }
    layers_.resize(cfg_.n_layers);
    int rc = NTK_OK;
    for (const auto& t : plan) {
        synth_fill(stage, t, spec.seed, nthreads);
        TensorSlot sl;
        if (!slot_of(t.name, &sl)) { rc = NTK_E_FORMAT; break; }
        rc = upload_shard(*sl.dst, stage, ggml_type_to_dtype((uint32_t)t.ggml_type), t.in_f, t.out_f, t.nbytes, sl.how);
        if (rc != NTK_OK) break;
    }
    nt_hip_free_host(stage);
    if (rc == NTK_OK) rc = finish_load();
    if (rc != NTK_OK) free_all();
    return rc;
}

int Model::finish_load() {
    cfg_full_ = cfg_;
    if (tp_world_ > 1) {
        cfg_.n_heads /= tp_world_;
        cfg_.n_kv_heads /= tp_world_;
        cfg_.intermediate_size /= tp_world_;
        NT_TRY(own_stream());
    } else {
        stream_ = ntk_stream(0);
    }
    if (!stream_) { err_ = "no compute stream"; return NTK_E_NODEVICE; }
    NT_TRY(alloc_buffers());
    repack_ = repack_wanted_;
    if (repack_) {
        const int st = repack_all();
        if (st == NTK_E_NOMEM) {
            int kept = 0;
            for (auto& L : layers_) for (auto m : kLayerMatrices) kept += (L.*m).rp ? 0 : 1;
            fprintf(stderr, "warning: not enough device memory for the decode repack of every matrix: %d projection tensors stay on the raw-GGUF path\n", kept);
            err_.clear();
        } else if (st != NTK_OK) {
            return st;
        }
        if (repack_ == 3) repack_ = 2;
        if (repack_ == 2) NT_TRY(drop_raw_all());
    }
    if (persistent_wanted_) set_persistent(persistent_wanted_);
    size_t fr = 0, tot = 0;
    ntk_device_mem_info(&fr, &tot);
    uint64_t q8_twice = 0;
    for_each_projection([&](DevTensor& t) { if (t.rp && t.ptr && t.dtype == NTK_DT_Q8_0) q8_twice += t.rp_bytes; });
    fprintf(stderr, "Model loaded successfully! (resident on MI355X: %.2f GB of weights%s%s)\nFree VRAM: %.1f GB\n",
            (weight_bytes_ - raw_freed_bytes_) / 1073741824.0, repack_bytes_ ? (" + " + std::to_string(repack_bytes_ / 1073741824.0).substr(0, 5) + " GB repacked for decode").c_str() : "",
            q8_twice ? (", of which " + std::to_string(q8_twice / 1073741824.0).substr(0, 5) + " GB extra: Q8_0 matrices keep their GGUF bytes beside the repack").c_str() : "",
            fr / 1073741824.0);
    return NTK_OK;
}

int Model::repack_one(DevTensor& t) {
    if (t.rp || !t.ptr) return NTK_OK;
    if (t.out_f <= 0 || t.out_f > 0x7FFFFFFF || t.in_f <= 0 || t.in_f > 32768) return NTK_OK;
    const bool q8 = t.dtype == NTK_DT_Q8_0;
    const size_t n = q8 ? ntk_q8l_bytes((int)t.out_f, (int)t.in_f) : ntk_rp_bytes(t.dtype, (int)t.out_f, (int)t.in_f);
    if (n == 0 || n > 0xFFFFFFF0ull) return NTK_OK;
    void* d = nt_hip_malloc(n + 256);
    if (!d) return NTK_E_NOMEM;
    allocs_.push_back(d);
    const int st = q8 ? ntk_q8l_pack(d, t.ptr, (int)t.out_f, (int)t.in_f, stream_) : ntk_rp_pack(d, t.ptr, (int)t.out_f, (int)t.in_f, t.dtype, stream_);
    if (st != NTK_OK) { err_ = std::string("decode repack failed: ") + ntk_status_string(st); return st; }
    t.rp = d;
    t.rp_bytes = n;
    repack_bytes_ += n;
    return NTK_OK;
}

int Model::repack_all() {
    int rc = NTK_OK;
    auto one = [&](DevTensor& t) { const int st = repack_one(t); if (st != NTK_OK && rc == NTK_OK) rc = st; return st; };
    for (auto& L : layers_) {
        if (one(L.*kLayerMatrices[0]) == NTK_E_NOMEM) break;
        for (size_t k = 1; k < kLayerMatrices.size(); ++k) one(L.*kLayerMatrices[k]);
        if (rc == NTK_E_NOMEM) break;
    }
    if (rc != NTK_E_NOMEM) one(output_);
    repack_done_ = true;
    const int sy = ntk_stream_synchronize(stream_);
    return rc != NTK_OK ? rc : sy;
}

int Model::drop_raw_all() {
    size_t need = 0;
    auto goes = [&](const DevTensor& t) { return t.rp && t.dtype != NTK_DT_Q8_0 && !(output_tied_ && t.ptr == token_embd_.ptr); };
    auto grp = [&](std::initializer_list<DevTensor*> ts) {
        size_t g = 0;
        for (DevTensor* t : ts) if (goes(*t)) g += padded_bytes(t->nbytes);
        need = std::max(need, g);
    };
    for (auto& L : layers_) { grp({&L.wq, &L.wk, &L.wv}); grp({&L.wo}); grp({&L.w_gate, &L.w_up}); grp({&L.w_down}); }
    grp({&output_});
    if (need == 0) return NTK_OK;
    if (!raw_scratch_ || raw_scratch_bytes_ < need) {
        void* d = nt_hip_malloc(need);
        if (!d) { fprintf(stderr, "warning: no device memory for the unpack scratch: the GGUF bytes stay resident beside the repack\n"); repack_ = 1; return NTK_OK; }
        allocs_.push_back(d);
        raw_scratch_ = d; raw_scratch_bytes_ = need;
    }
    auto drop = [&](DevTensor& t) {
        if (!t.ptr || !goes(t)) return;
        auto it = std::find(allocs_.begin(), allocs_.end(), t.ptr);
        if (it != allocs_.end()) allocs_.erase(it);
        nt_hip_free(t.ptr);
        t.ptr = nullptr;
        raw_freed_bytes_ += t.nbytes;
    };
    NT_TRY(ntk_stream_synchronize(stream_));
    for_each_projection(drop);
    return NTK_OK;
}

int Model::restore_raw_all() {
    int rc = NTK_OK;
    auto back = [&](DevTensor& t) {
        if (t.ptr || !t.rp || rc != NTK_OK) return;
        void* d = nt_hip_malloc(padded_bytes(t.nbytes));
        if (!d) { rc = NTK_E_NOMEM; return; }
        const int st = ntk_rp_unpack(d, t.rp, (int)t.out_f, (int)t.in_f, t.dtype, stream_);
        if (st != NTK_OK) { nt_hip_free(d); rc = st; return; }
        allocs_.push_back(d);
        t.ptr = d;
        raw_freed_bytes_ -= t.nbytes;
    };
    for_each_projection(back);
    const int sy = ntk_stream_synchronize(stream_);
    return rc != NTK_OK ? rc : sy;
}

const void* Model::raw_of(const DevTensor& t) {
    if (t.ptr) return t.ptr;
    if (!t.rp || !raw_scratch_) { raw_err_ = NTK_E_NULL; return nullptr; }
    const size_t n = padded_bytes(t.nbytes);
    if (raw_cursor_ + n > raw_scratch_bytes_) {
        if (!raw_err_) raw_err_ = NTK_E_NOMEM;
        return nullptr;
    }
    void* d = static_cast<uint8_t*>(raw_scratch_) + raw_cursor_;
    raw_cursor_ += n;
    const int st = ntk_rp_unpack(d, t.rp, (int)t.out_f, (int)t.in_f, t.dtype, stream_);
    if (st != NTK_OK) { raw_err_ = st; return nullptr; }
    return d;
}

int Model::alloc_buffers() {
    const size_t S = (size_t)cfg_.max_seq_len, H = (size_t)cfg_.hidden_size;
    const size_t per = (size_t)cfg_.n_kv_heads * cfg_.head_dim;
    auto dev = [&](size_t bytes, bool zero) -> void* {
        void* p = nt_hip_malloc(bytes + 256);
        if (p) { allocs_.push_back(p); if (zero) nt_hip_memset(p, 0, bytes); }
        return p;
    };
    if (S * per * sizeof(uint16_t) >= 0xF0000000ull) { err_ = "context too long: one layer's K cache must stay below 3.75 GiB (32-bit row offsets)"; return NTK_E_SHAPE; }
    if (kv_q8_) {
        if (cfg_.head_dim != 128 || cfg_.n_kv_heads <= 0 || cfg_.n_heads % cfg_.n_kv_heads != 0 || cfg_.n_heads / cfg_.n_kv_heads > 16) {
            err_ = "kv_cache=q8_0 needs head_dim 128 and at most 16 query heads per KV head (this model: head_dim " + std::to_string(cfg_.head_dim) +
                   ", " + std::to_string(cfg_.n_kv_heads > 0 ? cfg_.n_heads / cfg_.n_kv_heads : 0) + " query heads per KV head)";
            return NTK_E_SHAPE;
        }
        if (tp_world_ > 1) { err_ = "kv_cache=q8_0 is not supported with tensor parallelism"; return NTK_E_SHAPE; }
        if (fuse_attention_) { err_ = "kv_cache=q8_0 is not supported with the attention-inside-Wo launch (fuse_attention)"; return NTK_E_SHAPE; }
    }
    if (sequences_ > 1) {
        if (kv_q8_ && !batch_kv_q8_) { err_ = "sequences > 1 is not supported with kv_cache=q8_0"; return NTK_E_SHAPE; }
        if (tp_world_ > 1) { err_ = "sequences > 1 is not supported with tensor parallelism"; return NTK_E_SHAPE; }
        if ((size_t)sequences_ > S) { err_ = "sequences = " + std::to_string(sequences_) + " needs a context of at least as many positions (this load: " + std::to_string(S) + ")"; return NTK_E_SHAPE; }
    }
    NT_TRY(kv_.allocate(KvGeom{cfg_.n_layers, cfg_.max_seq_len, cfg_.n_kv_heads, cfg_.head_dim}, kv_q8_, sequences_, dev, &err_));
    hidden_ = (float*)dev(std::max<size_t>(S, 2) * H * 4, false);
    residual_ = (float*)dev(std::max<size_t>(S, 2) * H * 4, false);
    logits_ = (float*)dev((size_t)cfg_.vocab_size * 4, false);
    const size_t attn_ws = S * (size_t)(2 * cfg_.n_heads + 2 * cfg_.n_kv_heads) * cfg_.head_dim;
    const size_t ffn_ws = 2 * S * (size_t)cfg_.intermediate_size;
    workspace_floats_ = std::max(attn_ws, ffn_ws);
    workspace_ = (float*)dev(workspace_floats_ * 4, false);
    positions_ = (int*)dev(S * 4, false);
    tokens_dev_ = (int*)dev(S * 4, false);
    d_pos_ = (int*)dev(64, true);
    d_token_ = (int*)dev(64, true);
    argmax_scratch_ = (float*)dev(2 * 1024 * 4, false);
    rope_inv_freq_ = (float*)dev((size_t)cfg_.head_dim / 2 * 4 + 64, false);
    row_max_ = (float*)dev((size_t)S * 2 * 4, true);
    attn_scratch_ = (float*)dev(ntk_attention_split_scratch_bytes(cfg_.n_heads, cfg_.head_dim, kMaxAttnSplits), true);
    h_token_ = (int*)nt_hip_malloc_host(64);
    h_ring_ = (unsigned long long*)nt_hip_malloc_host(64);
    if (h_ring_) memset(h_ring_, 0, 64);
    sample_scratch_ = dev(ntk_sample_scratch_bytes(cfg_.vocab_size), false);
    attn_sync_ = (unsigned*)dev(4096, true);
    {
        const int H = cfg_.hidden_size, I = cfg_.intermediate_size, qkv = (cfg_.n_heads + 2 * cfg_.n_kv_heads) * cfg_.head_dim;
        const int shapes[][2] = {{H, qkv}, {H, cfg_.n_heads * cfg_.head_dim}, {H, cfg_.n_kv_heads * cfg_.head_dim}, {cfg_.n_heads * cfg_.head_dim, H},
                                 {H, 2 * I}, {H, I}, {I, H}};
        gemm_ws_bytes_ = 0;
        for (const auto& sh : shapes) gemm_ws_bytes_ = std::max(gemm_ws_bytes_, ntk_gemm_quant_workspace_bytes(sh[0], sh[1]));
    }
    gemm_ws_ = dev(gemm_ws_bytes_, false);
    gemm_ws2_ = dev(gemm_ws_bytes_, false);
    if (tp_world_ > 1) {
        tp_max_floats_ = S * H;
        tp_comm_ = ntk_tp_comm_alloc(ntk_tp_comm_bytes(tp_max_floats_));
        if (tp_comm_) allocs_.push_back(tp_comm_);
        if (!tp_comm_ || ntk_tp_comm_reset(tp_comm_, nullptr) != NTK_OK || ntk_device_synchronize() != NTK_OK) { err_ = "communication buffer allocation failed"; return NTK_E_NOMEM; }
    }
    d_recent_ = (int*)dev(kRecentCap * 4, false);
    h_recent_ = (int*)nt_hip_malloc_host(kRecentCap * 4);
    if (!kv_.k(0) || !kv_.v(0) || !hidden_ || !residual_ || !logits_ || !workspace_ || !positions_ || !tokens_dev_ ||
        !d_pos_ || !d_token_ || !argmax_scratch_ || !h_token_ || !h_ring_) {
        err_ = "buffer allocation failed";
        return NTK_E_NOMEM;
    }
    *h_token_ = 0;
    if (rope_inv_freq_) {
        std::vector<float> f((size_t)cfg_.head_dim / 2);
        for (int i = 0; i < cfg_.head_dim / 2; ++i) f[i] = 1.0f / powf(cfg_.rope_theta, (2.0f * i) / cfg_.head_dim);
        nt_hip_memcpy_h2d(rope_inv_freq_, f.data(), f.size() * 4);
    }
    if (sequences_ > 1) { NT_TRY(batch_buffers()); NT_TRY(batch_sample_buffers()); }
    return NTK_OK;
}

}
```

ntransformer_amd/csrc/gemv.hip:

```cpp
#include "gemv_core.hip.h"
#ifdef NTK_EXPERIMENTS
#include "ntk_experiments.h"
#endif
#include <algorithm>
#include <cmath>
#include <cstdio>
#include <cstdlib>

namespace ntk {

#ifdef NTK_EXPERIMENTS
#include "gemv_attfuse.hip.h"
#else
struct AttnFuse {};
#endif

enum { NS_ANY = 0, NS_ONE = 1, NS_SPLIT = 2 };
template <int DT, bool NORM, bool XFAST, bool A16, bool ATT = false, bool XI = false, bool LM = false, int NSF = NS_ANY>
__device__ __forceinline__ void gemv_quant_body(const GemvParams& p, const int bid, const int nblk, const AttnFuse* attp = nullptr) {
    using F = Fmt<DT>;
    static_assert(!LM || (DT == NTK_DT_Q8_0 && !A16 && !ATT && !XI), "lane-major rows: Q8_0");
    static_assert(NSF == NS_ANY || LM, "compile-time slice forms: the lane-major kernels");
    constexpr int NL = LM ? 4 : F::NL;
    constexpr int STAGE = LM ? 0 : NL * 1024 + 64;
    extern __shared__ __attribute__((aligned(16))) uint8_t smem[];
#ifdef NTK_GEMV_TRACE
    unsigned long long gv_t[GT_EV] = {0, 0, 0, 0, 0, 0, 0, 0, 0, 0, 0, 0, 0, 0};
#endif
    GV_STAMP(0);
#ifndef NTK_GEMV_NO_KARG_PREFETCH
    {
        const auto* ka = __builtin_amdgcn_kernarg_segment_ptr();
        unsigned d0, d1, d2, d3, d4;
        asm volatile("s_load_dword %0, %5, 0x0\n\ts_load_dword %1, %5, 0x40\n\ts_load_dword %2, %5, 0x80\n\ts_load_dword %3, %5, 0xc0\n\t"
                     "s_load_dword %4, %5, 0x100\n\ts_waitcnt lgkmcnt(0)"
                     : "=&s"(d0), "=&s"(d1), "=&s"(d2), "=&s"(d3), "=&s"(d4) : "s"(ka) : "memory");
        __builtin_amdgcn_sched_barrier(0);
    }
#endif

    const int tid = threadIdx.x;
    constexpr int XIT = 8, WIT = 4;
    u32x4 xv[XIT], wv[WIT];
    if constexpr (XFAST && !ATT) {
        const int step0 = (int)blockDim.x * 4;
#pragma unroll
        for (int i = 0; i < XIT; ++i) {
            xv[i] = u32x4{0u, 0u, 0u, 0u};
            if (i * step0 < p.in) xv[i] = *reinterpret_cast<const u32x4*>(p.x + min(tid * 4 + i * step0, p.in - 4));
        }
        if constexpr (NORM) {
#pragma unroll
            for (int i = 0; i < WIT; ++i) {
                wv[i] = u32x4{0u, 0u, 0u, 0u};
                if (i * step0 < p.in) wv[i] = *reinterpret_cast<const u32x4*>(p.norm_w + min(tid * 4 + i * step0, p.in - 4));
            }
        }
        GV_STAMP(7);
    }
    const int lane = tid & 63;
    const int wave = __builtin_amdgcn_readfirstlane(tid >> 6);
    const int ns = NSF == NS_ONE ? 1 : p.ns;
    const bool single = NSF == NS_ANY ? p.ns == 1 : NSF == NS_ONE;
    const int nwaves = ns * p.rw;
    const int s = wave % ns;
    const int g = wave / ns;
    constexpr bool norm = NORM;

    const size_t image_bytes = (size_t)std::min(ns, 4) * 64 * XPITCH * 4;
    const size_t stage0 = single ? image_bytes : 0;
    const size_t regionA = single ? image_bytes + (size_t)nwaves * STAGE : std::max((size_t)nwaves * STAGE, image_bytes);
    float* part = reinterpret_cast<float*>(smem + regionA);
    float* red = part + 2 * p.rw * ns * RB;
    const size_t lds_floats_total = regionA / 4 + (size_t)(2 * p.rw * ns * RB + 16 + 16);

    uint8_t* stage = smem + stage0 + (size_t)wave * STAGE;
    const int my_len = min(p.slice_cols, p.in - s * p.slice_cols);
    const int ncols = min(64, max(0, my_len - 64 * lane));
    const unsigned slice_byte0 = (unsigned)((size_t)s * p.slice_cols / F::BW * F::BB);
    const unsigned slice_bytes = (unsigned)(my_len / F::BW * F::BB);
    const int group = bid * p.rw + g;
    const int ngroups = nblk * p.rw;
    const int mats = p.silu_pair ? 2 : 1;
    const int n_my = (p.total_rows > group) ? ((p.total_rows - 1 - group) / ngroups + 1) * mats : 0;

    static_assert(MAX_SEG == 3, "locate / seg_y: unrolled for three segments");
    const int seg_rows0 = p.seg[0].rows, seg_rows1 = p.seg[1].rows;
    float* const seg_y0 = p.seg[0].y;
    float* const seg_y1 = p.seg[1].y;
    float* const seg_y2 = p.seg[2].y;
    auto locate = [&](int q, int& seg, int& row) {
        int r = group + (q >> (mats - 1)) * ngroups;
        if (p.silu_pair) { seg = q & 1; row = r; return; }
        seg = 0;
        if (p.nseg > 1 && r >= seg_rows0) {
            r -= seg_rows0; seg = 1;
            if (p.nseg > 2 && r >= seg_rows1) { r -= seg_rows1; seg = 2; }
        }
        row = r;
    };
    auto seg_y = [&](int seg) { return seg == 0 ? seg_y0 : seg == 1 ? seg_y1 : seg_y2; };
    int cu_seg = 0, cu_row = group, cu_rows = p.silu_pair ? 0x7fffffff : p.seg[0].rows;
    auto cursor_normalise = [&]() {
        while (cu_seg + 1 < p.nseg && cu_row >= cu_rows) { cu_row -= cu_rows; ++cu_seg; cu_rows = p.seg[cu_seg].rows; }
    };
    if (!p.silu_pair) cursor_normalise();
    auto cursor_advance = [&]() {
        if (p.silu_pair) {
            if (cu_seg == 0) { cu_seg = 1; } else { cu_seg = 0; cu_row += ngroups; }
        } else {
            cu_row += ngroups;
            cursor_normalise();
        }
    };

    u32x4 pf[NL], pf2[LM ? NL : 1];
    uint32_t pf_sc = 0u, pf2_sc = 0u;
    const int lm_nl = my_len >> 6, lm_lane = min(lane, max(lm_nl - 1, 0));
    unsigned pre_off[NL];
    if constexpr (A16) {
        const unsigned last0 = (slice_bytes - 1u) & ~15u;
#pragma unroll
        for (int j = 0; j < NL; ++j) pre_off[j] = min(16u * (unsigned)(lane + 64 * j), last0);
    }
    int pf_seg = 0, pf_row = 0, pf_shift = 0;
    float pf_res = 0.0f;
    auto issue = [&]() {
        pf_seg = cu_seg; pf_row = cu_row;
        if (p.resid != nullptr && single) {
            int idx = cu_row;
            asm volatile("" : "+v"(idx));
            pf_res = p.resid[idx];
        }
        if constexpr (LM) return;
        const unsigned rel = (unsigned)p.seg[cu_seg].delta + (unsigned)cu_row * p.row_bytes + slice_byte0;
        pf_shift = (int)(rel & 15u);
        const unsigned nbytes = (rel & 15u) + slice_bytes;
        const unsigned last = (nbytes - 1u) & ~15u;
        const uint8_t* a = p.seg[cu_seg].W + (rel & ~15u);
#pragma unroll
        for (int j = 0; j < NL; ++j) {
            unsigned off;
            if constexpr (A16) off = pre_off[j]; else off = min(16u * (unsigned)(lane + 64 * j), last);
            pf[j] = __builtin_nontemporal_load(reinterpret_cast<const u32x4*>(a + off));
        }
    };
    auto issue_lm = [&](u32x4 (&c)[NL], uint32_t& sc) {
        const uint8_t* a = p.seg[cu_seg].W + ((unsigned)cu_row * p.row_bytes + slice_byte0);
#pragma unroll
        for (int j = 0; j < NL; ++j)
            c[j] = __builtin_nontemporal_load(reinterpret_cast<const u32x4*>(a + 16u * (unsigned)(j * lm_nl + lm_lane)));
        sc = __builtin_nontemporal_load(reinterpret_cast<const uint32_t*>(a + 64u * (unsigned)lm_nl + 4u * (unsigned)lm_lane));
    };
    auto issue_first = [&]() { issue(); if constexpr (LM) issue_lm(pf, pf_sc); };
    if (n_my <= 0) { cu_seg = 0; cu_row = 0; }

    f32x2 x2[32];
    XInt xi;
    static_assert(!XI || (XFAST && !ATT && ((DT == NTK_DT_Q4_K && A16) || DT == NTK_DT_Q6_K)), "integer activations: fast prologue, Q4_K (aligned rows) / Q6_K");
    {
        float* ximg = reinterpret_cast<float*>(smem);
        constexpr int GS = 4;
        auto img_index = [&](int c, int g0) {
            if (single) return (c >> 6) * XPITCH + (c & 63);
            const int sp = c / p.slice_cols, cc = c - sp * p.slice_cols;
            return ((sp - g0) * 64 + (cc >> 6)) * XPITCH + (cc & 63);
        };
        const int step = (int)blockDim.x * 4;
        const int dummy = (int)(lds_floats_total - 16);
        const bool have_lo = ncols > 0, have_hi = ncols > 32;
        auto read_own_row = [&](int g0) {
            const float* xrow = ximg + ((s - g0) * 64 + lane) * XPITCH;
            const float* xr0 = xrow, *xr1 = xrow + 32;
            if constexpr (DT == NTK_DT_Q6_K) {
                xr0 = ximg + ((s - g0) * 64 + (lane & ~1)) * XPITCH + 32 * (lane & 1);
                xr1 = xr0 + XPITCH;
            }
#pragma unroll
            for (int j = 0; j < 64; j += 4) {
                const float4 v = *reinterpret_cast<const float4*>((j < 32 ? xr0 : xr1 - 32) + j);
                const bool have = j < 32 ? have_lo : have_hi;
                x2[j / 2] = f32x2{have ? v.x : 0.0f, have ? v.y : 0.0f};
                x2[j / 2 + 1] = f32x2{have ? v.z : 0.0f, have ? v.w : 0.0f};
            }
        };
        if constexpr (XFAST) {
            if constexpr (ATT) {
#ifdef NTK_EXPERIMENTS
                issue_first();
                att_wait(*attp);
#pragma unroll
                for (int i = 0; i < XIT; ++i) xv[i] = asm_load16_sc1(p.x, 4u * (unsigned)min(tid * 4 + i * step, p.in - 4));
                asm volatile("s_waitcnt vmcnt(0)" : "+v"(xv[0]), "+v"(xv[1]), "+v"(xv[2]), "+v"(xv[3]), "+v"(xv[4]), "+v"(xv[5]), "+v"(xv[6]), "+v"(xv[7]));
#endif
            } else {
#ifndef NTK_GEMV_NO_XWAIT
            asm volatile("" : "+v"(xv[0]), "+v"(xv[1]), "+v"(xv[2]), "+v"(xv[3]), "+v"(xv[4]), "+v"(xv[5]), "+v"(xv[6]), "+v"(xv[7]));
            if constexpr (NORM) asm volatile("" : "+v"(wv[0]), "+v"(wv[1]), "+v"(wv[2]), "+v"(wv[3]));
#endif
            issue_first();
            GV_STAMP(8);
            }
            __builtin_amdgcn_sched_barrier(0);
            GV_STAMP(1);
            float rms_inv = 1.0f;
            if constexpr (NORM) {
                float ssq = 0.0f;
#pragma unroll
                for (int i = 0; i < WIT; ++i) {
                    const float m = (tid * 4 + i * step < p.in) ? 1.0f : 0.0f;
                    const float x0 = __uint_as_float(xv[i].x), x1 = __uint_as_float(xv[i].y), x2_ = __uint_as_float(xv[i].z), x3 = __uint_as_float(xv[i].w);
                    ssq = fmaf(x0 * m, x0, ssq); ssq = fmaf(x1 * m, x1, ssq); ssq = fmaf(x2_ * m, x2_, ssq); ssq = fmaf(x3 * m, x3, ssq);
                }
                ssq = wave_sum(ssq);
                if (lane == 0) red[wave] = ssq;
                __syncthreads();
                float tot = 0.0f;
                for (int w = 0; w < nwaves; ++w) tot += red[w];
                rms_inv = 1.0f / sqrtf(tot / (float)p.in + p.eps);
#pragma unroll
                for (int i = 0; i < WIT; ++i) {
                    xv[i].x = __float_as_uint(__uint_as_float(xv[i].x) * rms_inv * __uint_as_float(wv[i].x));
                    xv[i].y = __float_as_uint(__uint_as_float(xv[i].y) * rms_inv * __uint_as_float(wv[i].y));
                    xv[i].z = __float_as_uint(__uint_as_float(xv[i].z) * rms_inv * __uint_as_float(wv[i].z));
                    xv[i].w = __float_as_uint(__uint_as_float(xv[i].w) * rms_inv * __uint_as_float(wv[i].w));
                }
            }
            if constexpr (XI) {
                uint8_t* dimg = smem;
                auto xi_store = [&](const u32x4 q, const int sp, const int cc, const bool live) {
                    const float v0 = live ? __uint_as_float(q.x) : 0.0f, v1 = live ? __uint_as_float(q.y) : 0.0f,
                                v2 = live ? __uint_as_float(q.z) : 0.0f, v3 = live ? __uint_as_float(q.w) : 0.0f;
                    float am = fmaxf(fmaxf(fabsf(v0), fabsf(v1)), fmaxf(fabsf(v2), fabsf(v3)));
                    am = fmaxf(am, dpp_or_self<DPP_QUAD_1032, 0xF>(am));
                    am = fmaxf(am, dpp_or_self<DPP_QUAD_2301, 0xF>(am));
                    am = fmaxf(am, dpp_or_self<DPP_ROW_HALF_MIRROR, 0xF>(am));
                    float sm = (v0 + v1) + (v2 + v3);
                    sm += dpp_or_zero<DPP_QUAD_1032, 0xF>(sm);
                    sm += dpp_or_zero<DPP_QUAD_2301, 0xF>(sm);
                    const int e = am > 0.0f ? __builtin_amdgcn_frexp_expf(am) : 0;
                    const float up = __builtin_ldexpf(1.0f, 22 - e), inv = __builtin_ldexpf(1.0f, e - 22);
                    const uint32_t x0 = __float_as_uint(fmaf(v0, up, 12582912.0f)) - 0x4B400000u, x1 = __float_as_uint(fmaf(v1, up, 12582912.0f)) - 0x4B400000u,
                                   x2i = __float_as_uint(fmaf(v2, up, 12582912.0f)) - 0x4B400000u, x3 = __float_as_uint(fmaf(v3, up, 12582912.0f)) - 0x4B400000u;
                    const uint32_t ta = __builtin_amdgcn_perm(x1, x0, 0x05010400u);
                    const uint32_t tb = __builtin_amdgcn_perm(x1, x0, 0x07030602u);
                    const uint32_t tc = __builtin_amdgcn_perm(x3, x2i, 0x05010400u);
                    const uint32_t td = __builtin_amdgcn_perm(x3, x2i, 0x07030602u);
                    const uint32_t p0 = __builtin_amdgcn_perm(tc, ta, 0x05040100u);
                    const uint32_t p1 = __builtin_amdgcn_perm(tc, ta, 0x07060302u);
                    const uint32_t p2 = __builtin_amdgcn_perm(td, tb, 0x05040100u);
                    if (live) {
                        uint8_t* row = dimg + (size_t)(sp * 64 + (cc >> 6)) * (XPITCH * 4);
                        *reinterpret_cast<uint32_t*>(row + (cc & 63)) = p0;
                        *reinterpret_cast<uint32_t*>(row + 64 + (cc & 63)) = p1;
                        *reinterpret_cast<uint32_t*>(row + 128 + (cc & 63)) = p2;
                        float* meta = reinterpret_cast<float*>(row + 192);
                        if ((cc & 31) == 0) meta[(cc >> 5) & 1] = inv;
                        if ((cc & 15) == 0) meta[2 + ((cc >> 4) & 3)] = sm;
                    }
                };
                auto xi_read = [&](const int g0) {
                    const bool have_lo_ = ncols > 0, have_hi_ = ncols > 32;
                    const uint8_t* rowA = dimg + (size_t)((s - g0) * 64 + lane) * (XPITCH * 4);
                    const uint8_t* rowB = rowA;
                    int offA = 0, offB = 32;
                    if constexpr (DT == NTK_DT_Q6_K) {
                        rowA = dimg + (size_t)((s - g0) * 64 + (lane & ~1)) * (XPITCH * 4);
                        rowB = rowA + XPITCH * 4;
                        offA = offB = 32 * (lane & 1);
                    }
#pragma unroll
                    for (int pl = 0; pl < 3; ++pl)
#pragma unroll
                        for (int k4 = 0; k4 < 4; ++k4) {
                            const uint8_t* src = (k4 < 2 ? rowA + offA : rowB + offB) + 64 * pl + 16 * (k4 & 1);
                            const u32x4 v = *reinterpret_cast<const u32x4*>(src);
                            const bool have = k4 < 2 ? have_lo_ : have_hi_;
                            xi.d[pl][4 * k4] = have ? v.x : 0u; xi.d[pl][4 * k4 + 1] = have ? v.y : 0u;
                            xi.d[pl][4 * k4 + 2] = have ? v.z : 0u; xi.d[pl][4 * k4 + 3] = have ? v.w : 0u;
                        }
                    const float* mA = reinterpret_cast<const float*>(rowA + 192);
                    const float* mB = reinterpret_cast<const float*>(rowB + 192);
                    xi.inv[0] = have_lo_ ? mA[offA >> 5] : 0.0f;
                    xi.inv[1] = have_hi_ ? mB[offB >> 5] : 0.0f;
                    xi.sx[0] = have_lo_ ? mA[2 + (offA >> 4)] : 0.0f; xi.sx[1] = have_lo_ ? mA[3 + (offA >> 4)] : 0.0f;
                    xi.sx[2] = have_hi_ ? mB[2 + (offB >> 4)] : 0.0f; xi.sx[3] = have_hi_ ? mB[3 + (offB >> 4)] : 0.0f;
                };
                int isp = 0, icc = tid * 4;
#pragma unroll
                for (int i = 0; i < XIT; ++i) {
                    if (i * step >= p.in) continue;
                    xi_store(xv[i], isp, icc, tid * 4 + i * step < p.in);
                    icc += step;
                    if (icc >= p.slice_cols) { icc -= p.slice_cols; ++isp; }
                }
                __syncthreads();
                xi_read(0);
            } else
            {
                const int cend = min(p.in, GS * p.slice_cols);
                int isp = 0, icc = tid * 4;
#pragma unroll
                for (int i = 0; i < XIT; ++i) {
                    if (i * step >= cend) continue;
                    const int c = tid * 4 + i * step;
                    *reinterpret_cast<u32x4*>(ximg + (c < cend ? (isp * 64 + (icc >> 6)) * XPITCH + (icc & 63) : dummy)) = xv[i];
                    icc += step;
                    if (icc >= p.slice_cols) { icc -= p.slice_cols; ++isp; }
                }
                for (int c = XIT * step + tid * 4; c < cend; c += step)
                    *reinterpret_cast<float4*>(ximg + img_index(c, 0)) = *reinterpret_cast<const float4*>(p.x + c);
                GV_STAMP(9);
                __syncthreads();
                GV_STAMP(10);
                if (s < GS) read_own_row(0);
#ifdef NTK_GEMV_TRACE
                asm volatile("s_waitcnt lgkmcnt(0)" ::: "memory");
                GV_STAMP(11);
#endif
            }
            if constexpr (!XI)
            for (int g0 = GS; g0 < ns; g0 += GS) {
                const int cbeg = g0 * p.slice_cols, cend = min(p.in, (g0 + GS) * p.slice_cols);
                __syncthreads();
                for (int c = cbeg + tid * 4; c < cend; c += step)
                    *reinterpret_cast<float4*>(ximg + img_index(c, g0)) = *reinterpret_cast<const float4*>(p.x + c);
                __syncthreads();
                if (s >= g0 && s < g0 + GS) read_own_row(g0);
            }
        } else {
            issue_first();
            float rms_inv = 1.0f;
            if (NORM && !(kAblate & 1)) {
                float ssq = 0.0f;
                for (int c = tid; c < p.in; c += blockDim.x) ssq = fmaf(p.x[c], p.x[c], ssq);
                ssq = wave_sum(ssq);
                if (lane == 0) red[wave] = ssq;
                __syncthreads();
                float tot = 0.0f;
                for (int w = 0; w < nwaves; ++w) tot += red[w];
                rms_inv = 1.0f / sqrtf(tot / (float)p.in + p.eps);
            }
            for (int g0 = 0; g0 < ns; g0 += GS) {
                const int cbeg = g0 * p.slice_cols, cend = min(p.in, (g0 + GS) * p.slice_cols);
                if (g0 > 0) __syncthreads();
                if (!(kAblate & 1)) {
                    for (int c = cbeg + tid; c < cend; c += blockDim.x)
                        ximg[img_index(c, g0)] = NORM ? p.x[c] * rms_inv * p.norm_w[c] : p.x[c];
                }
                __syncthreads();
                if (s >= g0 && s < g0 + GS) read_own_row(g0);
            }
        }
        if ((kAblate & 1) || XI) {
#pragma unroll
            for (int j = 0; j < 32; ++j) x2[j] = f32x2{1.0f, 1.0f};
        }
        if (!single && !LM) __syncthreads();
        GV_STAMP(2);
    }
    float sx16[4], sx32[2];
#pragma unroll
    for (int r = 0; r < 4; ++r) {
        float t = 0.0f;
#pragma unroll
        for (int j = 0; j < 8; ++j) t += x2[8 * r + j].x + x2[8 * r + j].y;
        sx16[r] = t;
    }
    sx32[0] = sx16[0] + sx16[1];
    sx32[1] = sx16[2] + sx16[3];
    if constexpr (DT == NTK_DT_Q4_K) {
#pragma unroll
        for (int j = 16; j < 32; ++j) x2[j] *= 0.0625f;
    }
    if constexpr (DT == NTK_DT_Q4_0) {
#pragma unroll
        for (int j = 0; j < 32; ++j) if ((j & 8) != 0) x2[j] *= 0.0625f;
    }
    float gate_carry = 0.0f;
    float pair_g = 0.0f, pair_u = 0.0f;
    auto silu_flush = [&](const int last_pair) {
        const int base = last_pair & ~63;
        if (lane <= last_pair - base) {
            const int row = group + (base + lane) * ngroups;
            p.seg[0].y[row] = pair_g / (1.0f + expf(-pair_g)) * pair_u;
        }
    };

    float res_pf = 0.0f;
    auto prefetch_resid = [&](int b) {
        if (p.resid == nullptr || s != 0 || lane >= RB || b * RB + lane >= n_my) return;
        int seg, row;
        locate(b * RB + lane, seg, row);
        res_pf = p.resid[row];
    };
    if (!single) prefetch_resid(0);
    auto combine = [&](int b, int cnt) {
        if (s != 0) return;
        const float* pg = part + (size_t)(b & 1) * p.rw * ns * RB + (size_t)(g * ns) * RB;
        float t = 0.0f;
        if (lane < cnt)
            for (int ss = 0; ss < ns; ++ss) t += pg[ss * RB + lane];
        const float nxt = __shfl_down(t, 1, 64);
        if (lane < cnt) {
            int seg, row;
            locate(b * RB + lane, seg, row);
            if (p.silu_pair) {
                if ((lane & 1) == 0) seg_y0[row] = t / (1.0f + expf(-t)) * nxt;
            } else {
                float v = t;
                if (p.resid != nullptr && seg == 0) v = res_pf + v;
                seg_y(seg)[row] = v;
            }
        }
        prefetch_resid(b + 1);
    };

    auto row_step = [&](const int q, u32x4 (&cur)[NL], uint32_t& cur_sc, u32x4 (&nxt)[LM ? NL : 1], uint32_t& nxt_sc) __attribute__((always_inline)) {
        const int seg = pf_seg, row = pf_row, shift = A16 ? 0 : pf_shift;
        const float res = pf_res;
        float acc;
        if constexpr (LM) {
            asm volatile("" : "+v"(cur[0]), "+v"(cur[1]), "+v"(cur[2]), "+v"(cur[3]), "+v"(cur_sc));
#ifdef NTK_GEMV_TRACE
            if (q == 0) GV_STAMP(3);
            if (q == n_my - 1) GV_STAMP(5);
#endif
            if (q + 1 < n_my) { cursor_advance(); issue(); issue_lm(nxt, nxt_sc); }
            __builtin_amdgcn_sched_barrier(0);
            acc = dot_q8_regs(cur, cur_sc, ncols, x2);
        } else {
#pragma unroll
            for (int j = 0; j < NL; ++j) {
                if (kAblate & 4) { asm volatile("" ::"v"(pf[j])); continue; }
                *reinterpret_cast<u32x4*>(stage + 16 * (lane + 64 * j)) = pf[j];
            }
            __builtin_amdgcn_wave_barrier();
#ifdef NTK_GEMV_TRACE
            if (q == 0) GV_STAMP(3);
            if (q == n_my - 1) GV_STAMP(5);
#endif
            if (q + 1 < n_my) { cursor_advance(); issue(); }
            if constexpr (XI && DT == NTK_DT_Q6_K) acc = DotI<DT>::run(stage, shift, lane, ncols, xi);
            else if constexpr (XI) acc = DotI<DT>::run(stage, lane, ncols, xi);
            else acc = (kAblate & 2) ? x2[0].x + (float)q : Dot<DT, A16>::run(stage, shift, lane, ncols, x2, sx16, sx32);
            __builtin_amdgcn_wave_barrier();
        }
        const float tot = wave_sum_lane63(acc);
#ifdef NTK_GEMV_TRACE
        if (q == 0) { asm volatile("" :: "v"(tot)); GV_STAMP(4); }
#endif

        if (single) {
            if (p.silu_pair) {
                const float t63 = __int_as_float(__builtin_amdgcn_readlane(__float_as_int(tot), 63));
                const int pi = (q >> 1) & 63;
                if ((q & 1) == 0) { if (lane == pi) pair_g = t63; }
                else {
                    if (lane == pi) pair_u = t63;
                    if (pi == 63 || q == n_my - 1) silu_flush(q >> 1);
                }
            } else if (lane == 63) {
                float v = tot;
                if (p.resid != nullptr && seg == 0) v = res + v;
                p.seg[seg].y[row] = v;
            }
        } else {
            const int b = q / RB, i = q % RB;
            if (lane == 63) part[(size_t)(b & 1) * p.rw * ns * RB + (size_t)(g * ns + s) * RB + i] = tot;
            if (i == RB - 1) {
                __syncthreads();
                combine(b, RB);
            }
        }
    };
    for (int q = 0; q < n_my; ++q) {
        row_step(q, pf, pf_sc, pf2, pf2_sc);
        if constexpr (LM) { if (++q < n_my) row_step(q, pf2, pf2_sc, pf, pf_sc); }
    }
    if (!single) {
        int done = n_my / RB;
        if (n_my % RB) {
            __syncthreads();
            combine(done, n_my % RB);
            ++done;
        }
        for (; done < p.nbatch; ++done) __syncthreads();
    }
#ifdef NTK_EXPERIMENTS
    if constexpr (ATT) att_finish(*attp, nblk);
#endif
#ifdef NTK_GEMV_TRACE
    GV_STAMP(6);
    if (tid == 0 && bid < GT_WG) {
        gv_t[13] = (unsigned long long)n_my;
        for (int e = 0; e < GT_EV; ++e) g_gemv_trace[p.trace_slot & (GT_SLOTS - 1)][bid][e] = gv_t[e];
    }
#endif
}

template <bool NORM, bool XFAST, int NSF>
__global__ __launch_bounds__(512, Fmt<NTK_DT_Q8_0>::MINW) void gemv_q8l_kernel(const GemvParams p) {
    gemv_quant_body<NTK_DT_Q8_0, NORM, XFAST, false, false, false, true, NSF>(p, (int)blockIdx.x, (int)gridDim.x);
}
template <bool UNPACK>
__global__ __launch_bounds__(256) void q8l_pack_kernel(uint8_t* __restrict__ dst, const uint8_t* __restrict__ src, const int rows, const int in,
                                                       const int slice_cols) {
    const int lanes_row = in >> 6;
    const size_t t = (size_t)blockIdx.x * blockDim.x + threadIdx.x;
    if (t >= (size_t)rows * lanes_row) return;
    const int row = (int)(t / lanes_row), gl = (int)(t % lanes_row);
    const int lanes_slice = slice_cols >> 6, sl = gl / lanes_slice, l = gl - sl * lanes_slice;
    const int nl = min(lanes_slice, lanes_row - sl * lanes_slice);
    const size_t row0 = (size_t)row * lanes_row * 68;
    uint32_t* file = reinterpret_cast<uint32_t*>(const_cast<uint8_t*>(UNPACK ? dst : src) + row0 + (size_t)gl * 68);
    uint8_t* slice = const_cast<uint8_t*>(UNPACK ? src : dst) + row0 + (size_t)sl * lanes_slice * 68;
    uint32_t w[17], q[16], sc;
    if constexpr (!UNPACK) {
#pragma unroll
        for (int k = 0; k < 17; ++k) w[k] = file[k];
#pragma unroll
        for (int k = 0; k < 8; ++k) { q[k] = (w[k] >> 16) | (w[k + 1] << 16); q[8 + k] = w[9 + k]; }
        sc = (w[0] & 0xFFFFu) | (w[8] & 0xFFFF0000u);
#pragma unroll
        for (int j = 0; j < 4; ++j) *reinterpret_cast<u32x4*>(slice + (size_t)(j * nl + l) * 16) = u32x4{q[4 * j], q[4 * j + 1], q[4 * j + 2], q[4 * j + 3]};
        *reinterpret_cast<uint32_t*>(slice + (size_t)64 * nl + 4 * l) = sc;
    } else {
#pragma unroll
        for (int j = 0; j < 4; ++j) {
            const u32x4 v = *reinterpret_cast<const u32x4*>(slice + (size_t)(j * nl + l) * 16);
            q[4 * j] = v.x; q[4 * j + 1] = v.y; q[4 * j + 2] = v.z; q[4 * j + 3] = v.w;
        }
        sc = *reinterpret_cast<const uint32_t*>(slice + (size_t)64 * nl + 4 * l);
        w[0] = (sc & 0xFFFFu) | (q[0] << 16);
#pragma unroll
        for (int k = 1; k < 8; ++k) w[k] = (q[k - 1] >> 16) | (q[k] << 16);
        w[8] = (q[7] >> 16) | (sc & 0xFFFF0000u);
#pragma unroll
        for (int k = 0; k < 8; ++k) w[9 + k] = q[8 + k];
#pragma unroll
        for (int k = 0; k < 17; ++k) file[k] = w[k];
    }
}

#ifdef NTK_EXPERIMENTS
template <int DT>
__global__ __launch_bounds__(512, Fmt<DT>::MINW) void gemv_quant_att_kernel(const GemvParams p, const AttnFuse att) {
    extern __shared__ __attribute__((aligned(16))) uint8_t att_smem[];
    const int nh = att.n_heads;
    if ((int)blockIdx.x < nh) {
        att_produce(att, reinterpret_cast<float*>(att_smem), (int)blockIdx.x);
        return;
    }
    gemv_quant_body<DT, false, true, A16_OK<DT>, true>(p, (int)blockIdx.x - nh, (int)gridDim.x - nh, &att);
}
#endif

template <int DT, bool NORM, bool XFAST, bool A16>
__global__ __launch_bounds__(512, Fmt<DT>::MINW) void gemv_quant_kernel(const GemvParams p) {
    gemv_quant_body<DT, NORM, XFAST, A16>(p, (int)blockIdx.x, (int)gridDim.x);
}
template <int DT, bool NORM>
__global__ __launch_bounds__(512, Fmt<DT>::MINW) void gemv_quant_xi_kernel(const GemvParams p) {
    gemv_quant_body<DT, NORM, true, A16_OK<DT>, false, true>(p, (int)blockIdx.x, (int)gridDim.x);
}
template <int DTA, int DTB, bool NORM>
__global__ __launch_bounds__(512, 4) void gemv_quant_pair_kernel(const GemvParams pa, const GemvParams pb, const int split) {
    if ((int)blockIdx.x < split) gemv_quant_body<DTA, NORM, true, A16_OK<DTA>>(pa, (int)blockIdx.x, split);
    else gemv_quant_body<DTB, NORM, true, A16_OK<DTB>>(pb, (int)blockIdx.x - split, (int)gridDim.x - split);
}

#ifdef NTK_EXPERIMENTS
#include "gemv_colsplit.hip.h"
#endif

template <typename T, bool ADD>
__global__ __launch_bounds__(256) void gemv_dense_kernel(float* __restrict__ y, const T* __restrict__ W,
                                                         const float* __restrict__ x, int out, int in) {
    const int lane = threadIdx.x & 63;
    const int wave = blockIdx.x * (blockDim.x >> 6) + (threadIdx.x >> 6);
    const int nwaves = gridDim.x * (blockDim.x >> 6);
    constexpr int V = 16 / (int)sizeof(T);
    for (int r = wave; r < out; r += nwaves) {
        const T* w = W + (size_t)r * in;
        float acc = 0.0f;
        int done = 0;
        if ((reinterpret_cast<uintptr_t>(w) & 15) == 0 && (reinterpret_cast<uintptr_t>(x) & 15) == 0) {
            const int nv = in / V;
            for (int i = lane; i < nv; i += 64) {
                const u32x4 raw = __builtin_nontemporal_load(reinterpret_cast<const u32x4*>(w) + i);
                if constexpr (sizeof(T) == 4) {
                    const float4 xv = *reinterpret_cast<const float4*>(x + 4 * i);
                    acc = fmaf(__uint_as_float(raw.x), xv.x, acc); acc = fmaf(__uint_as_float(raw.y), xv.y, acc);
                    acc = fmaf(__uint_as_float(raw.z), xv.z, acc); acc = fmaf(__uint_as_float(raw.w), xv.w, acc);
                } else {
                    const float4 x0 = *reinterpret_cast<const float4*>(x + 8 * i);
                    const float4 x1 = *reinterpret_cast<const float4*>(x + 8 * i + 4);
                    acc = fmaf(h2f((uint16_t)(raw.x & 0xFFFF)), x0.x, acc); acc = fmaf(h2f((uint16_t)(raw.x >> 16)), x0.y, acc);
                    acc = fmaf(h2f((uint16_t)(raw.y & 0xFFFF)), x0.z, acc); acc = fmaf(h2f((uint16_t)(raw.y >> 16)), x0.w, acc);
                    acc = fmaf(h2f((uint16_t)(raw.z & 0xFFFF)), x1.x, acc); acc = fmaf(h2f((uint16_t)(raw.z >> 16)), x1.y, acc);
                    acc = fmaf(h2f((uint16_t)(raw.w & 0xFFFF)), x1.z, acc); acc = fmaf(h2f((uint16_t)(raw.w >> 16)), x1.w, acc);
                }
            }
            done = nv * V;
        }
        for (int i = done + lane; i < in; i += 64) {
            float wv;
            if constexpr (sizeof(T) == 4) wv = (float)w[i]; else wv = h2f((uint16_t)w[i]);
            acc = fmaf(wv, x[i], acc);
        }
        acc = wave_sum(acc);
        if (lane == 0) y[r] = ADD ? y[r] + acc : acc;
    }
}

static bool is_quant(int dt) {
    return dt == NTK_DT_Q8_0 || dt == NTK_DT_Q4_0 || dt == NTK_DT_Q4_K || dt == NTK_DT_Q5_K || dt == NTK_DT_Q6_K;
}

struct GemvLaunch {
    GemvParams p;
    int grid, nwaves;
    size_t lds;
    bool xfast, a16;
};

static bool raise_lds_limit(const void* fn) {
    return hipFuncSetAttribute(fn, hipFuncAttributeMaxDynamicSharedMemorySize, 160 * 1024) == hipSuccess;
}

template <int DT>
static int prepare_quant(const ntk_gemv_seg* segs, int nseg, const float* x, int in, const float* norm_w, float eps,
                         const float* resid, int silu_pair, int max_wg, GemvLaunch& L, bool lm = false) {
    using F = Fmt<DT>;
    if (in <= 0 || in % F::BW != 0) return NTK_E_SHAPE;
    GemvParams& p = L.p;
    p = GemvParams{};
    long total = 0;
    const size_t row_bytes = (size_t)in / F::BW * F::BB;
    for (int i = 0; i < nseg; ++i) {
        if (segs[i].rows < 0) return NTK_E_SHAPE;
        if (segs[i].rows > 0 && (!segs[i].W || !segs[i].y)) return NTK_E_NULL;
        if ((size_t)segs[i].rows * row_bytes > 0xFFFFFFF0ull) return NTK_E_SHAPE;
        const uintptr_t w = reinterpret_cast<uintptr_t>(segs[i].W);
        if (w & 1) return NTK_E_ALIGN;
        p.seg[i].W = reinterpret_cast<const uint8_t*>(w & ~(uintptr_t)15);
        p.seg[i].delta = (int)(w & 15);
        p.seg[i].y = segs[i].y;
        p.seg[i].rows = segs[i].rows;
        total += segs[i].rows;
    }
    if (silu_pair) {
        if (nseg != 2 || segs[0].rows != segs[1].rows || resid) return NTK_E_SHAPE;
        total = segs[0].rows;
    }
    p.nseg = nseg;
    p.total_rows = (int)total;
    p.x = x;
    p.in = in;
    if (!gemv_slices(in, F::BW == 256 ? 256 : 64, p.ns, p.slice_cols)) return NTK_E_SHAPE;
    static const int env_waves = std::max(1, NTK_TUNE_ENV_INT("NTK_GEMV_WAVES", 8));
    p.rw = std::max(1, env_waves / p.ns);
    L.nwaves = p.ns * p.rw;
    p.x_vec = ((reinterpret_cast<uintptr_t>(x) & 15) == 0 &&
               (!norm_w || (reinterpret_cast<uintptr_t>(norm_w) & 15) == 0) && (p.slice_cols % 4 == 0)) ? 1 : 0;
    p.norm_w = norm_w;
    p.eps = eps;
    p.resid = resid;
    p.silu_pair = silu_pair;
    p.row_bytes = (unsigned)row_bytes;
    const int mats = silu_pair ? 2 : 1;
    int grid = (int)std::min<long>((total + p.rw - 1) / p.rw, max_wg);
    grid = std::max(grid, 1);
    L.grid = grid;
    const long ngroups = (long)grid * p.rw;
    const long rows_per_group = (total + ngroups - 1) / ngroups;
    p.nbatch = (int)((rows_per_group * mats + RB - 1) / RB);
    const int STAGE = lm ? 0 : F::NL * 1024 + 64;
    const size_t image_bytes = (size_t)std::min(p.ns, 4) * 64 * XPITCH * 4;
    const size_t regionA = p.ns == 1 ? image_bytes + (size_t)L.nwaves * STAGE : std::max((size_t)L.nwaves * STAGE, image_bytes);
    L.lds = regionA + (size_t)(2 * p.rw * p.ns * RB + 16 + 16) * sizeof(float);
    L.xfast = p.x_vec && (in % 4 == 0) && in >= 4 && !(kAblate & 1) && (!norm_w || in <= 4 * 4 * 64 * L.nwaves) &&
              (p.ns == 1 || 4 * 64 * L.nwaves <= p.slice_cols);
    bool a16 = (DT == NTK_DT_Q4_K || DT == NTK_DT_Q5_K);
    for (int i = 0; i < nseg; ++i) a16 = a16 && p.seg[i].delta == 0;
    L.a16 = a16;
    return NTK_OK;
}

constexpr size_t kXiMinBytes = (size_t)48 << 20;
enum { XI_DEFAULT = -1, XI_NEVER = 0, XI_ALWAYS = 1 };

static int max_workgroups() {
    static const int max_wg = std::max(1, NTK_TUNE_ENV_INT("NTK_GEMV_MAX_WG", 512));
    return max_wg;
}

template <int DT>
static int launch_quant(const ntk_gemv_seg* segs, int nseg, const float* x, int in, const float* norm_w, float eps,
                        const float* resid, int silu_pair, hipStream_t st, int xi_mode = XI_DEFAULT) {
    GemvLaunch L;
    const int rc = prepare_quant<DT>(segs, nseg, x, in, norm_w, eps, resid, silu_pair, max_workgroups(), L);
    if (rc != NTK_OK) return rc;
    if (L.p.total_rows == 0) return NTK_OK;
    using KernelFn = void (*)(const GemvParams);
    static const KernelFn table[2][2][2] = {
        {{gemv_quant_kernel<DT, false, false, false>, gemv_quant_kernel<DT, false, false, A16_OK<DT>>},
         {gemv_quant_kernel<DT, false, true, false>, gemv_quant_kernel<DT, false, true, A16_OK<DT>>}},
        {{gemv_quant_kernel<DT, true, false, false>, gemv_quant_kernel<DT, true, false, A16_OK<DT>>},
         {gemv_quant_kernel<DT, true, true, false>, gemv_quant_kernel<DT, true, true, A16_OK<DT>>}}};
    if (L.lds > 64 * 1024) {
        static bool once = [] {
            bool ok = true;
            for (int a = 0; a < 2; ++a)
                for (int b = 0; b < 2; ++b)
                    for (int c = 0; c < 2; ++c)
                        ok = ok && hipFuncSetAttribute((const void*)table[a][b][c], hipFuncAttributeMaxDynamicSharedMemorySize,
                                                       160 * 1024) == hipSuccess;
            return ok;
        }();
        if (!once || L.lds > 160 * 1024) return NTK_E_SHAPE;
    }
#ifdef NTK_EXPERIMENTS
    if constexpr (DT == NTK_DT_Q8_0) {
        static const int cs_mode = NTK_TUNE_ENV_INT("NTK_GEMV_COLSPLIT", 0);
        bool cs = cs_mode != 0 && in == CS_COLS && L.xfast && !(kAblate & 7);
        for (int i = 0; i < nseg && cs; ++i) cs = L.p.seg[i].delta == 0;
        if (cs) {
            const int total = L.p.total_rows, mats = silu_pair ? 2 : 1;
            const int cgrid = std::min(total, max_workgroups());
            const size_t items = (size_t)((total + cgrid - 1) / cgrid) * mats;
            const size_t clds = (size_t)8 * CS_RBT * CS_STRIPE + items * 8 * sizeof(float) + 64;
            using CFn = void (*)(const GemvParams);
            static const CFn ct[2] = {gemv_q8_colsplit_kernel<false>, gemv_q8_colsplit_kernel<true>};
            static const bool ok = raise_lds_limit((const void*)ct[0]) && raise_lds_limit((const void*)ct[1]);
            if (ok && clds <= 150 * 1024) {
                hipLaunchKernelGGL(ct[norm_w ? 1 : 0], dim3(cgrid), dim3(512), clds, st, L.p);
                return last_launch_status();
            }
        }
    }
#endif
    const dim3 g(L.grid), b(64 * L.nwaves);
#ifdef NTK_GEMV_TRACE
    static int trace_counter = 0;
    L.p.trace_slot = trace_counter++;
#endif
    if constexpr (DT == NTK_DT_Q4_K || DT == NTK_DT_Q6_K) {
        const size_t launch_bytes = (size_t)L.p.total_rows * (silu_pair ? 2 : 1) * L.p.row_bytes;
        const bool want = xi_mode == XI_ALWAYS || (xi_mode == XI_DEFAULT && launch_bytes >= kXiMinBytes);
        if (want && L.xfast && (L.a16 || DT == NTK_DT_Q6_K) && L.p.ns <= 2 && in <= 8 * 4 * 64 * L.nwaves) {
            using XFn = void (*)(const GemvParams);
            static const XFn xt[2] = {gemv_quant_xi_kernel<DT, false>, gemv_quant_xi_kernel<DT, true>};
            if (L.lds > 64 * 1024) {
                static bool once2 = hipFuncSetAttribute((const void*)xt[0], hipFuncAttributeMaxDynamicSharedMemorySize, 160 * 1024) == hipSuccess &&
                                    hipFuncSetAttribute((const void*)xt[1], hipFuncAttributeMaxDynamicSharedMemorySize, 160 * 1024) == hipSuccess;
                if (!once2) return NTK_E_SHAPE;
            }
            hipLaunchKernelGGL(xt[norm_w ? 1 : 0], g, b, L.lds, st, L.p);
            return last_launch_status();
        }
    }
    hipLaunchKernelGGL(table[norm_w ? 1 : 0][L.xfast ? 1 : 0][L.a16 ? 1 : 0], g, b, L.lds, st, L.p);
    return last_launch_status();
}

static size_t q8l_bytes(int rows, int in) {
    int ns, sc;
    return rows > 0 && q8l_layout(in, ns, sc) ? (size_t)rows * (size_t)(in / 32 * 34) : 0;
}

static int q8l_pack(void* dst, const void* raw, int rows, int in, bool unpack, hipStream_t st) {
    int ns, sc;
    if (rows <= 0 || !q8l_layout(in, ns, sc)) return NTK_E_SHAPE;
    if ((reinterpret_cast<uintptr_t>(unpack ? raw : dst) & 15) || (reinterpret_cast<uintptr_t>(unpack ? dst : raw) & 3)) return NTK_E_ALIGN;
    const size_t n = (size_t)rows * (in / 64);
    if ((n + 255) / 256 > 0x7FFFFFFFull) return NTK_E_SHAPE;
    const dim3 g((unsigned)((n + 255) / 256)), b(256);
    uint8_t* d = static_cast<uint8_t*>(dst);
    const uint8_t* r = static_cast<const uint8_t*>(raw);
    if (unpack) hipLaunchKernelGGL(q8l_pack_kernel<true>, g, b, 0, st, d, r, rows, in, sc);
    else hipLaunchKernelGGL(q8l_pack_kernel<false>, g, b, 0, st, d, r, rows, in, sc);
    return last_launch_status();
}

int q8l_gemv_fused(const ntk_gemv_seg* segs, int nseg, const float* x, int in, const float* norm_w, float eps, const float* resid,
                   int silu_pair, hipStream_t st) {
    int ns, sc;
    if (!q8l_layout(in, ns, sc)) return NTK_E_SHAPE;
    for (int i = 0; i < nseg; ++i)
        if (reinterpret_cast<uintptr_t>(segs[i].W) & 15) return NTK_E_ALIGN;
    GemvLaunch L;
    const int rc = prepare_quant<NTK_DT_Q8_0>(segs, nseg, x, in, norm_w, eps, resid, silu_pair, max_workgroups(), L, true);
    if (rc != NTK_OK) return rc;
    if (L.p.total_rows == 0) return NTK_OK;
    using KernelFn = void (*)(const GemvParams);
#define Q8L_FORMS(NORM, XFAST) {gemv_q8l_kernel<NORM, XFAST, NS_ONE>, gemv_q8l_kernel<NORM, XFAST, NS_SPLIT>}
    static const KernelFn table[2][2][2] = {{Q8L_FORMS(false, false), Q8L_FORMS(false, true)}, {Q8L_FORMS(true, false), Q8L_FORMS(true, true)}};
#undef Q8L_FORMS
    if (L.lds > 64 * 1024) {
        static const bool once = [] {
            bool ok = true;
            for (int a = 0; a < 2; ++a)
                for (int b = 0; b < 2; ++b)
                    for (int c = 0; c < 2; ++c) ok = ok && raise_lds_limit((const void*)table[a][b][c]);
            return ok;
        }();
        if (!once || L.lds > 160 * 1024) return NTK_E_SHAPE;
    }
#ifdef NTK_GEMV_TRACE
    static int trace_counter = 0;
    L.p.trace_slot = trace_counter++;
#endif
    hipLaunchKernelGGL(table[norm_w ? 1 : 0][L.xfast ? 1 : 0][L.p.ns == 1 ? 0 : 1], dim3(L.grid), dim3(64 * L.nwaves), L.lds, st, L.p);
    return last_launch_status();
}

#ifdef NTK_EXPERIMENTS
template <int DT>
static int launch_att(const AttnFuse& att, const ntk_gemv_seg* seg, int in, const float* resid, hipStream_t st) {
    GemvLaunch L;
    const int rc = prepare_quant<DT>(seg, 1, att.out, in, nullptr, 0.0f, resid, 0, max_workgroups(), L);
    if (rc != NTK_OK) return rc;
    if (!L.xfast || L.nwaves != 8 || L.p.seg[0].delta != 0 || L.p.total_rows == 0 || L.grid < 1) return NTK_E_ALIGN;
    const size_t att_lds = sizeof(float) * ((size_t)3 * att.hd + 16 + (size_t)8 * att.hd);
    if (att_lds > L.lds) return NTK_E_SHAPE;
    if (L.lds > 64 * 1024) {
        static bool once = hipFuncSetAttribute((const void*)gemv_quant_att_kernel<DT>, hipFuncAttributeMaxDynamicSharedMemorySize, 160 * 1024) == hipSuccess;
        if (!once || L.lds > 160 * 1024) return NTK_E_SHAPE;
    }
    hipLaunchKernelGGL(gemv_quant_att_kernel<DT>, dim3(L.grid + att.n_heads), dim3(64 * L.nwaves), L.lds, st, L.p, att);
    return last_launch_status();
}
#endif

template <int DTA, int DTB>
static int launch_pair(const ntk_gemv_seg* sa, int na, const ntk_gemv_seg* sb, int nb, const float* x, int in, const float* norm_w,
                       float eps, hipStream_t st) {
    const double ba = (double)Fmt<DTA>::BB / Fmt<DTA>::BW, bb = (double)Fmt<DTB>::BB / Fmt<DTB>::BW;
    long ra = 0, rb = 0;
    for (int i = 0; i < na; ++i) ra += sa[i].rows;
    for (int i = 0; i < nb; ++i) rb += sb[i].rows;
    if (ra <= 0 || rb <= 0) return NTK_E_SHAPE;
    const int total_wg = max_workgroups();
    int wa = (int)(total_wg * (ra * ba) / (ra * ba + rb * bb) + 0.5);
    wa = std::min(std::max(wa, 1), total_wg - 1);
    GemvLaunch A, B;
    int rc = prepare_quant<DTA>(sa, na, x, in, norm_w, eps, nullptr, 0, wa, A);
    if (rc == NTK_OK) rc = prepare_quant<DTB>(sb, nb, x, in, norm_w, eps, nullptr, 0, total_wg - wa, B);
    if (rc != NTK_OK) return rc;
    if (!A.xfast || !B.xfast || A.nwaves != B.nwaves || A.a16 != A16_OK<DTA> || B.a16 != A16_OK<DTB>) return NTK_E_ALIGN;
    for (int i = 0; i < na; ++i) if (A.p.seg[i].delta != 0 && A16_OK<DTA>) return NTK_E_ALIGN;
    using PairFn = void (*)(const GemvParams, const GemvParams, int);
    const size_t lds = std::max(A.lds, B.lds);
    static const PairFn table[2] = {gemv_quant_pair_kernel<DTA, DTB, false>, gemv_quant_pair_kernel<DTA, DTB, true>};
    if (lds > 64 * 1024) {
        static bool once = hipFuncSetAttribute((const void*)table[0], hipFuncAttributeMaxDynamicSharedMemorySize, 160 * 1024) == hipSuccess &&
                           hipFuncSetAttribute((const void*)table[1], hipFuncAttributeMaxDynamicSharedMemorySize, 160 * 1024) == hipSuccess;
        if (!once || lds > 160 * 1024) return NTK_E_SHAPE;
    }
    hipLaunchKernelGGL(table[norm_w ? 1 : 0], dim3(A.grid + B.grid), dim3(64 * A.nwaves), lds, st, A.p, B.p, A.grid);
    return last_launch_status();
}

static int dispatch_quant(int dt, const ntk_gemv_seg* segs, int nseg, const float* x, int in, const float* norm_w,
                          float eps, const float* resid, int silu_pair, hipStream_t st, int xi_mode = XI_DEFAULT) {
    switch (dt) {
        case NTK_DT_Q8_0: return launch_quant<NTK_DT_Q8_0>(segs, nseg, x, in, norm_w, eps, resid, silu_pair, st);
        case NTK_DT_Q4_0: return launch_quant<NTK_DT_Q4_0>(segs, nseg, x, in, norm_w, eps, resid, silu_pair, st);
        case NTK_DT_Q4_K: return launch_quant<NTK_DT_Q4_K>(segs, nseg, x, in, norm_w, eps, resid, silu_pair, st, xi_mode);
        case NTK_DT_Q5_K: return launch_quant<NTK_DT_Q5_K>(segs, nseg, x, in, norm_w, eps, resid, silu_pair, st);
        case NTK_DT_Q6_K: return launch_quant<NTK_DT_Q6_K>(segs, nseg, x, in, norm_w, eps, resid, silu_pair, st, xi_mode);
        default: return NTK_E_DTYPE;
    }
}

template <bool ADD>
static int launch_dense(float* y, const void* W, const float* x, int out, int in, int dt, hipStream_t st) {
    if (out == 0) return NTK_OK;
    const int grid = std::min((out + 3) / 4, 2048);
    if (dt == NTK_DT_F32)
        hipLaunchKernelGGL((gemv_dense_kernel<float, ADD>), dim3(grid), dim3(256), 0, st, y, (const float*)W, x, out, in);
    else
        hipLaunchKernelGGL((gemv_dense_kernel<uint16_t, ADD>), dim3(grid), dim3(256), 0, st, y, (const uint16_t*)W, x, out, in);
    return last_launch_status();
}

}

extern "C" {

#ifdef NTK_GEMV_TRACE
NTK_EXTRA_API int ntk_debug_gemv_trace(unsigned long long* out, size_t n) {
    return hipMemcpyFromSymbol(out, HIP_SYMBOL(ntk::g_gemv_trace), n * sizeof(unsigned long long)) == hipSuccess ? 0 : -3;
}
#endif

size_t ntk_q8l_bytes(int rows, int in_features) { return ntk::q8l_bytes(rows, in_features); }
int ntk_q8l_pack(void* dst, const void* raw, int rows, int in_features, void* stream) {
    if (!dst || !raw) return NTK_E_NULL;
    return ntk::q8l_pack(dst, raw, rows, in_features, false, ntk::resolve_stream(stream));
}
int ntk_q8l_unpack(void* raw, const void* packed, int rows, int in_features, void* stream) {
    if (!raw || !packed) return NTK_E_NULL;
    return ntk::q8l_pack(raw, packed, rows, in_features, true, ntk::resolve_stream(stream));
}

int ntk_gemv(float* y, const void* W, const float* x, int out_features, int in_features, int weight_dtype, void* stream) {
    if (!y || !W || !x) return NTK_E_NULL;
    if (out_features < 0 || in_features <= 0) return NTK_E_SHAPE;
    hipStream_t st = ntk::resolve_stream(stream);
    if (weight_dtype == NTK_DT_F32 || weight_dtype == NTK_DT_F16)
        return ntk::launch_dense<false>(y, W, x, out_features, in_features, weight_dtype, st);
    if (!ntk::is_quant(weight_dtype)) return NTK_E_DTYPE;
    ntk_gemv_seg seg{W, y, out_features, weight_dtype};
    return ntk::dispatch_quant(weight_dtype, &seg, 1, x, in_features, nullptr, 0.0f, nullptr, 0, st);
}

int ntk_gemv_add(float* y, const void* W, const float* x, int out_features, int in_features, int weight_dtype, void* stream) {
    if (!y || !W || !x) return NTK_E_NULL;
    if (out_features < 0 || in_features <= 0) return NTK_E_SHAPE;
    if (weight_dtype != NTK_DT_F16) return NTK_E_DTYPE;
    return ntk::launch_dense<true>(y, W, x, out_features, in_features, weight_dtype, ntk::resolve_stream(stream));
}

#ifdef NTK_EXPERIMENTS
int ntk_attention_gemv_fused(float* attn_out, const float* q, const float* k, const float* v, void* k_cache, void* v_cache,
                             const int* d_pos, const float* inv_freq, int n_heads, int n_kv_heads, int head_dim, int max_seq,
                             float scale, float theta_base, float freq_scale, const ntk_gemv_seg* wo, const float* resid,
                             unsigned* sync3, void* stream) {
    if (!attn_out || !q || !k || !v || !k_cache || !v_cache || !d_pos || !wo || !wo->W || !wo->y || !sync3) return NTK_E_NULL;
    if (n_heads <= 0 || n_kv_heads <= 0 || n_heads % n_kv_heads != 0 || max_seq <= 0) return NTK_E_SHAPE;
    if (head_dim != 64 && head_dim != 128 && head_dim != 256) return NTK_E_SHAPE;
    if ((reinterpret_cast<uintptr_t>(k_cache) & 15) || (reinterpret_cast<uintptr_t>(v_cache) & 15)) return NTK_E_ALIGN;
    ntk::AttnFuse a{};
    a.q = q; a.k = k; a.v = v; a.out = attn_out;
    a.kc = static_cast<uint16_t*>(k_cache); a.vc = static_cast<uint16_t*>(v_cache);
    a.d_pos = d_pos; a.inv_freq = inv_freq; a.sync = sync3;
    a.n_heads = n_heads; a.n_kv_heads = n_kv_heads; a.hd = head_dim; a.max_seq = max_seq;
    a.scale = scale; a.theta = theta_base; a.fscale = freq_scale;
    const int in = n_heads * head_dim;
    hipStream_t st = ntk::resolve_stream(stream);
    switch (wo->dtype) {
        case NTK_DT_Q8_0: return ntk::launch_att<NTK_DT_Q8_0>(a, wo, in, resid, st);
        case NTK_DT_Q4_0: return ntk::launch_att<NTK_DT_Q4_0>(a, wo, in, resid, st);
        case NTK_DT_Q4_K: return ntk::launch_att<NTK_DT_Q4_K>(a, wo, in, resid, st);
        case NTK_DT_Q5_K: return ntk::launch_att<NTK_DT_Q5_K>(a, wo, in, resid, st);
        case NTK_DT_Q6_K: return ntk::launch_att<NTK_DT_Q6_K>(a, wo, in, resid, st);
        default: return NTK_E_DTYPE;
    }
}
#endif

static int gemv_fused_form(const ntk_gemv_seg* segs, int nseg, const float* x, int in_features, const float* norm_w, float eps,
                           const float* resid, int silu_pair, void* stream, int xi_mode) {
    if (!segs || !x) return NTK_E_NULL;
    if (nseg < 1 || nseg > ntk::MAX_SEG) return NTK_E_SHAPE;
    ntk_gemv_seg a[3], b[3];
    int na = 0, nb = 0;
    for (int i = 0; i < nseg; ++i) {
        if (!ntk::is_quant(segs[i].dtype)) return NTK_E_DTYPE;
        if (segs[i].dtype == segs[0].dtype) a[na++] = segs[i];
        else if (nb == 0 || segs[i].dtype == b[0].dtype) b[nb++] = segs[i];
        else return NTK_E_DTYPE;
    }
    hipStream_t st = ntk::resolve_stream(stream);
    if (nb == 0) return ntk::dispatch_quant(segs[0].dtype, segs, nseg, x, in_features, norm_w, eps, resid, silu_pair, st, xi_mode);
    if (resid || silu_pair) return NTK_E_DTYPE;
    const int da = a[0].dtype, db = b[0].dtype;
    if (da == NTK_DT_Q4_K && db == NTK_DT_Q6_K) return ntk::launch_pair<NTK_DT_Q4_K, NTK_DT_Q6_K>(a, na, b, nb, x, in_features, norm_w, eps, st);
    if (da == NTK_DT_Q6_K && db == NTK_DT_Q4_K) return ntk::launch_pair<NTK_DT_Q4_K, NTK_DT_Q6_K>(b, nb, a, na, x, in_features, norm_w, eps, st);
    if (da == NTK_DT_Q4_K && db == NTK_DT_Q5_K) return ntk::launch_pair<NTK_DT_Q4_K, NTK_DT_Q5_K>(a, na, b, nb, x, in_features, norm_w, eps, st);
    if (da == NTK_DT_Q5_K && db == NTK_DT_Q4_K) return ntk::launch_pair<NTK_DT_Q4_K, NTK_DT_Q5_K>(b, nb, a, na, x, in_features, norm_w, eps, st);
    return NTK_E_DTYPE;
}

int ntk_gemv_fused(const ntk_gemv_seg* segs, int nseg, const float* x, int in_features, const float* norm_w, float eps,
                   const float* resid, int silu_pair, void* stream) {
    return gemv_fused_form(segs, nseg, x, in_features, norm_w, eps, resid, silu_pair, stream, ntk::XI_DEFAULT);
}
int ntk_debug_gemv_fused_form(const ntk_gemv_seg* segs, int nseg, const float* x, int in_features, const float* norm_w, float eps,
                              const float* resid, int silu_pair, int integer_activations, void* stream) {
    if (integer_activations < -1 || integer_activations > 1) return NTK_E_SHAPE;
    return gemv_fused_form(segs, nseg, x, in_features, norm_w, eps, resid, silu_pair, stream, integer_activations);
}

}
```

ntransformer_amd/ops.py:

```python
from __future__ import annotations

import ctypes as C
from typing import Optional, Sequence

import numpy as np

from . import _lib
from ._lib import GemvSeg, check


class DeviceBuffer:

    def __init__(self, nbytes: int):
        self.nbytes = int(nbytes)
        self.ptr = _lib.lib().nt_hip_malloc(max(self.nbytes, 1))
        if not self.ptr:
            raise _lib.NtkError(-7, "hipMalloc(%d)" % nbytes)

    @classmethod
    def from_numpy(cls, a: np.ndarray) -> "DeviceBuffer":
        a = np.ascontiguousarray(a)
        b = cls(a.nbytes)
        if a.nbytes:
            _lib.lib().nt_hip_memcpy_h2d(b.ptr, a.ctypes.data_as(C.c_void_p), a.nbytes)
        return b

    @classmethod
    def zeros(cls, nbytes: int) -> "DeviceBuffer":
        b = cls(nbytes)
        _lib.lib().nt_hip_memset(b.ptr, 0, nbytes)
        return b

    def upload(self, a: np.ndarray, offset: int = 0) -> None:
        a = np.ascontiguousarray(a)
        assert offset + a.nbytes <= self.nbytes
        _lib.lib().nt_hip_memcpy_h2d(self.ptr + offset, a.ctypes.data_as(C.c_void_p), a.nbytes)

    def numpy(self, dtype=np.float32, count: Optional[int] = None, offset: int = 0) -> np.ndarray:
        dt = np.dtype(dtype)
        n = (self.nbytes - offset) // dt.itemsize if count is None else count
        out = np.empty(n, dt)
        check(_lib.lib().ntk_stream_synchronize(None), "stream sync")
        if n:
            _lib.lib().nt_hip_memcpy_d2h(out.ctypes.data_as(C.c_void_p), self.ptr + offset, out.nbytes)
        return out

    def at(self, byte_offset: int) -> int:
        return self.ptr + byte_offset

    def free(self) -> None:
        if self.ptr:
            _lib.lib().nt_hip_free(self.ptr)
            self.ptr = None

    def __del__(self):
        try:
            self.free()
        except Exception:
            pass


def _p(x) -> Optional[int]:
    if x is None:
        return None
    return x.ptr if isinstance(x, DeviceBuffer) else int(x)


def init(device_id: int = 0) -> None:
    check(_lib.lib().ntk_device_init(device_id), "ntk_device_init")


def synchronize(stream=None) -> None:
    check(_lib.lib().ntk_stream_synchronize(stream), "stream sync")


def launch_rmsnorm(output, input, weight, batch_size, hidden_size, eps, stream=None):
    check(_lib.lib().ntk_rmsnorm(_p(output), _p(input), _p(weight), batch_size, hidden_size, eps, stream), "rmsnorm")


def launch_rmsnorm_f16(output, input, weight, batch_size, hidden_size, eps, stream=None):
    check(_lib.lib().ntk_rmsnorm_f16(_p(output), _p(input), _p(weight), batch_size, hidden_size, eps, stream), "rmsnorm_f16")


def launch_rope(q, k, positions, batch_size, seq_len, n_heads, n_kv_heads, head_dim, theta_base, freq_scale,
                interleaved, stream=None):
    check(_lib.lib().ntk_rope(_p(q), _p(k), _p(positions), batch_size, seq_len, n_heads, n_kv_heads, head_dim,
                              theta_base, freq_scale, int(bool(interleaved)), stream), "rope")


def launch_softmax(output, input, rows, cols, stream=None):
    check(_lib.lib().ntk_softmax(_p(output), _p(input), rows, cols, stream), "softmax")


def launch_masked_softmax(output, input, mask, rows, cols, stream=None):
    check(_lib.lib().ntk_masked_softmax(_p(output), _p(input), _p(mask), rows, cols, stream), "masked_softmax")


def launch_gemv(y, W, x, out_features, in_features, weight_dtype, stream=None):
    check(_lib.lib().ntk_gemv(_p(y), _p(W), _p(x), out_features, in_features, int(weight_dtype), stream), "gemv")


def launch_gemv_add(y, W, x, out_features, in_features, weight_dtype, stream=None):
    check(_lib.lib().ntk_gemv_add(_p(y), _p(W), _p(x), out_features, in_features, int(weight_dtype), stream), "gemv_add")


def launch_gemm_f32(Cm, A, B, M, N, K, stream=None):
    check(_lib.lib().ntk_gemm_f32(_p(Cm), _p(A), _p(B), M, N, K, stream), "gemm_f32")


def launch_silu_mul(output, gate, up, size, stream=None):
    check(_lib.lib().ntk_silu_mul(_p(output), _p(gate), _p(up), size, stream), "silu_mul")


def launch_add_bias(y, bias, size, stream=None):
    check(_lib.lib().ntk_add_bias(_p(y), _p(bias), size, stream), "add_bias")


def launch_attention_decode(output, q, k_cache, v_cache, seq_len, n_heads, n_kv_heads, head_dim, max_seq, scale, stream=None):
    check(_lib.lib().ntk_attention_decode(_p(output), _p(q), _p(k_cache), _p(v_cache), seq_len, n_heads, n_kv_heads,
                                          head_dim, max_seq, scale, stream), "attention_decode")


def launch_attention_prefill(output, Q, k_cache, v_cache, seq_len, start_pos, n_heads, n_kv_heads, head_dim, max_seq,
                             scale, stream=None):
    check(_lib.lib().ntk_attention_prefill(_p(output), _p(Q), _p(k_cache), _p(v_cache), seq_len, start_pos, n_heads,
                                           n_kv_heads, head_dim, max_seq, scale, stream), "attention_prefill")


def launch_copy_to_kv_cache(k_cache, v_cache, k, v, seq_len, n_kv_heads, head_dim, start_pos, max_seq, stream=None):
    check(_lib.lib().ntk_copy_to_kv_cache(_p(k_cache), _p(v_cache), _p(k), _p(v), seq_len, n_kv_heads, head_dim,
                                          start_pos, max_seq, stream), "copy_to_kv_cache")


def launch_add(out, a, b, size, stream=None):
    check(_lib.lib().ntk_add(_p(out), _p(a), _p(b), size, stream), "add")


def launch_add_inplace(a, b, size, stream=None):
    check(_lib.lib().ntk_add_inplace(_p(a), _p(b), size, stream), "add_inplace")


def launch_copy(dst, src, size, stream=None):
    check(_lib.lib().ntk_copy(_p(dst), _p(src), size, stream), "copy")


def launch_cosine_similarity(result, a, b, size, stream=None):
    check(_lib.lib().ntk_cosine_similarity(_p(result), _p(a), _p(b), size, stream), "cosine_similarity")


def gemv_fused(segs: Sequence[tuple], x, in_features, norm_w=None, eps=0.0, resid=None, silu_pair=False, stream=None,
               integer_activations=None):
    arr = (GemvSeg * len(segs))()
    for i, (W, y, rows, dt) in enumerate(segs):
        arr[i].W, arr[i].y, arr[i].rows, arr[i].dtype = _p(W), _p(y), rows, int(dt)
    if integer_activations is None:
        check(_lib.lib().ntk_gemv_fused(arr, len(segs), _p(x), in_features, _p(norm_w), eps, _p(resid), int(silu_pair),
                                        stream), "gemv_fused")
    else:
        check(_lib.lib().ntk_debug_gemv_fused_form(arr, len(segs), _p(x), in_features, _p(norm_w), eps, _p(resid), int(silu_pair),
                                                   1 if integer_activations else 0, stream), "gemv_fused_form")


def q8l_bytes(rows, in_features) -> int:
    return int(_lib.lib().ntk_q8l_bytes(rows, in_features))


def q8l_pack(raw, rows, in_features, stream=None) -> "DeviceBuffer":
    n = q8l_bytes(rows, in_features)
    if n == 0:
        raise _lib.NtkError(-2, "q8l_pack: shape without a lane-major form")
    dst = DeviceBuffer(n + 256)
    check(_lib.lib().ntk_q8l_pack(_p(dst), _p(raw), rows, in_features, stream), "q8l_pack")
    synchronize(stream)
    return dst


def q8l_unpack(packed, rows, in_features, nbytes, stream=None) -> "DeviceBuffer":
    dst = DeviceBuffer(nbytes + 256)
    check(_lib.lib().ntk_q8l_unpack(_p(dst), _p(packed), rows, in_features, stream), "q8l_unpack")
    synchronize(stream)
    return dst


def rp_bytes(dtype, rows, in_features) -> int:
    return int(_lib.lib().ntk_rp_bytes(int(dtype), rows, in_features))


def rp_pack(raw, rows, in_features, dtype, stream=None) -> "DeviceBuffer":
    n = rp_bytes(dtype, rows, in_features)
    if n == 0:
        raise _lib.NtkError(-1, "rp_pack: dtype / shape without a repacked form")
    dst = DeviceBuffer(n + 256)
    check(_lib.lib().ntk_rp_pack(_p(dst), _p(raw), rows, in_features, int(dtype), stream), "rp_pack")
    synchronize(stream)
    return dst


def rp_unpack(rp, rows, in_features, dtype, nbytes, stream=None) -> "DeviceBuffer":
    dst = DeviceBuffer(nbytes + 256)
    check(_lib.lib().ntk_rp_unpack(_p(dst), _p(rp), rows, in_features, int(dtype), stream), "rp_unpack")
    synchronize(stream)
    return dst


def gemv_rp_fused(segs: Sequence[tuple], x, in_features, norm_w=None, eps=0.0, resid=None, silu_pair=False, stream=None):
    arr = (GemvSeg * len(segs))()
    for i, (W, y, rows, dt) in enumerate(segs):
        arr[i].W, arr[i].y, arr[i].rows, arr[i].dtype = _p(W), _p(y), rows, int(dt)
    check(_lib.lib().ntk_gemv_rp_fused(arr, len(segs), _p(x), in_features, _p(norm_w), eps, _p(resid), int(silu_pair),
                                       stream), "gemv_rp_fused")


def _gemm_quant_f16(segs, X, n_tokens, in_features, resid=None, row_max=None, partials=None, stream=None, keep=None, repacked=False, workspace=None,
                    reuse_x=0, full_form=False):
    L = _lib.lib()
    L.ntk_gemm_quant_workspace_bytes.restype = C.c_size_t
    n = int(L.ntk_gemm_quant_workspace_bytes(C.c_int(in_features), C.c_int(sum(r for _, _, r, _ in segs))))
    ws = workspace if workspace is not None else DeviceBuffer(n)
    arr = (GemvSeg * len(segs))()
    for i, (W, y, rows, dt) in enumerate(segs):
        arr[i].W, arr[i].y, arr[i].rows, arr[i].dtype = _p(W), _p(y), rows, int(dt)
    d = _lib.GemmDesc()
    d.segs, d.nseg, d.X, d.n_tokens, d.in_features, d.resid = arr, len(segs), _p(X), n_tokens, in_features, _p(resid)
    d.workspace, d.workspace_bytes, d.reuse_x, d.row_max = ws.ptr, n, int(reuse_x), _p(row_max)
    d.partials = C.pointer(partials) if partials is not None else None
    d.weights_repacked = 1 if repacked else 0
    d.full_form = 1 if full_form else 0
    L.ntk_gemm_quant_f16.argtypes = [C.POINTER(_lib.GemmDesc), C.c_void_p]
    st = L.ntk_gemm_quant_f16(C.byref(d), stream)
    if keep is not None:
        keep.append(ws)
    else:
        synchronize()
    return st


def gemm_quant_f16_prepared(segs, X, n_tokens, in_features, resid=None, row_max=None, stream=None):
    L = _lib.lib()
    L.ntk_gemm_quant_workspace_bytes.restype = C.c_size_t
    n = int(L.ntk_gemm_quant_workspace_bytes(C.c_int(in_features), C.c_int(sum(r for _, _, r, _ in segs))))
    ws = DeviceBuffer(n)
    arr = (GemvSeg * len(segs))()
    for i, (W, y, rows, dt) in enumerate(segs):
        arr[i].W, arr[i].y, arr[i].rows, arr[i].dtype = _p(W), _p(y), rows, int(dt)
    d = _lib.GemmDesc()
    d.segs, d.nseg, d.X, d.n_tokens, d.in_features, d.resid = arr, len(segs), _p(X), n_tokens, in_features, _p(resid)
    d.workspace, d.workspace_bytes, d.reuse_x, d.row_max = ws.ptr, n, 0, _p(row_max)
    L.ntk_gemm_quant_f16.argtypes = [C.POINTER(_lib.GemmDesc), C.c_void_p]

    def call(_keep=(ws, arr, d)):
        return L.ntk_gemm_quant_f16(C.byref(d), stream)
    return call


def gemm_quant_ws_multi(segs, X, n_tokens, in_features, stream=None, repacked=False):
    return _gemm_quant_f16(segs, X, n_tokens, in_features, stream=stream, repacked=repacked)


def gemm_quant_ws(Y, W, X, n_tokens, out_features, in_features, dtype, resid=None, stream=None, repacked=False):
    st = _gemm_quant_f16([(W, Y, out_features, dtype)], X, n_tokens, in_features, resid=resid, stream=stream, repacked=repacked)
    synchronize()
    return st


def gemm_quant_ws_rm(Y, W, X, n_tokens, out_features, in_features, dtype, row_max, resid=None, stream=None):
    st = _gemm_quant_f16([(W, Y, out_features, dtype)], X, n_tokens, in_features, resid=resid, row_max=row_max, stream=stream)
    synchronize()
    return st


def gemm_deferred_then_consumer(kind, W, X, n_tokens, rows, in_features, dtype, row_max=None, **kw):
    L = _lib.lib()
    pt = _lib.GemmPartials()
    keep = []
    if kind == "norm":
        y = DeviceBuffer(n_tokens * rows * 4)
        in_place = kw.get("in_place", True)
        check(_gemm_quant_f16([(W, kw["hidden"] if in_place else y, rows, dtype)], X, n_tokens, in_features, resid=kw["hidden"] if in_place else None,
                              row_max=row_max, partials=pt, keep=keep), "gemm deferred")
        L.ntk_reduce_rmsnorm_rowmax.argtypes = [C.c_void_p, C.POINTER(_lib.GemmPartials), C.c_void_p, C.c_float, C.c_void_p, C.c_void_p, C.c_void_p, C.c_void_p]
        check(L.ntk_reduce_rmsnorm_rowmax(_p(kw["hidden"]), C.byref(pt), _p(kw["weight"]), kw["eps"], _p(kw["x_out"]), _p(kw["row_max_out"]), _p(kw.get("zero")), None),
              "reduce_rmsnorm_rowmax")
    else:
        yg, yu = DeviceBuffer(n_tokens * rows * 4), DeviceBuffer(n_tokens * rows * 4)
        check(_gemm_quant_f16([(W[0], yg, rows, dtype), (W[1], yu, rows, dtype)], X, n_tokens, in_features, row_max=row_max, partials=pt, keep=keep),
              "gemm multi deferred")
        L.ntk_reduce_silu_mul_rowmax.argtypes = [C.c_void_p, C.POINTER(_lib.GemmPartials), C.c_void_p, C.c_void_p]
        check(L.ntk_reduce_silu_mul_rowmax(_p(kw["output"]), C.byref(pt), _p(kw["row_max_out"]), None), "reduce_silu_mul_rowmax")
    synchronize()
    return int(pt.nsplit)


def rope_kv_store(q, k, v, positions, seq_len, n_heads, n_kv_heads, head_dim, theta_base, freq_scale, interleaved, k_cache, v_cache, start_pos, max_seq):
    check(_lib.lib().ntk_rope_kv_store(_p(q), _p(k), _p(v), _p(positions), seq_len, n_heads, n_kv_heads, head_dim, theta_base, freq_scale,
                                       int(bool(interleaved)), _p(k_cache), _p(v_cache), start_pos, max_seq, None), "rope_kv_store")


def gemm_workspace(in_features, rows):
    L = _lib.lib()
    L.ntk_gemm_quant_workspace_bytes.restype = C.c_size_t
    return DeviceBuffer(int(L.ntk_gemm_quant_workspace_bytes(C.c_int(in_features), C.c_int(rows))))


def prepare_x(kind, workspace, n_tokens, width, **kw):
    L = _lib.lib()
    vp, i, f = C.c_void_p, C.c_int, C.c_float
    if kind == "x":
        L.ntk_gemm_prepare_x.argtypes = [vp, i, i, vp, vp]
        st = L.ntk_gemm_prepare_x(_p(kw["X"]), n_tokens, width, workspace.ptr, None)
    elif kind == "rmsnorm":
        L.ntk_rmsnorm_prepare_x.argtypes = [vp, vp, vp, i, i, f, vp, vp]
        st = L.ntk_rmsnorm_prepare_x(_p(kw["output"]), _p(kw["input"]), _p(kw["weight"]), n_tokens, width, kw["eps"], workspace.ptr, None)
    elif kind == "silu":
        L.ntk_silu_mul_prepare_x.argtypes = [vp, vp, vp, i, i, vp, vp]
        st = L.ntk_silu_mul_prepare_x(_p(kw["output"]), _p(kw["gate"]), _p(kw["up"]), n_tokens, width, workspace.ptr, None)
    elif kind == "reduce_rmsnorm":
        L.ntk_reduce_rmsnorm_prepare_x.argtypes = [vp, C.POINTER(_lib.GemmPartials), vp, f, vp, vp, vp]
        st = L.ntk_reduce_rmsnorm_prepare_x(_p(kw["hidden"]), C.byref(kw["partials"]), _p(kw["weight"]), kw["eps"], _p(kw["x_out"]), workspace.ptr, None)
    else:
        L.ntk_reduce_silu_mul_prepare_x.argtypes = [vp, C.POINTER(_lib.GemmPartials), vp, vp]
        st = L.ntk_reduce_silu_mul_prepare_x(_p(kw["output"]), C.byref(kw["partials"]), workspace.ptr, None)
    synchronize()
    return st


def launch_rmsnorm_rowmax(output, input, weight, n_tokens, hidden_size, eps, row_max, zero_tokens=None, stream=None):
    check(_lib.lib().ntk_rmsnorm_rowmax(_p(output), _p(input), _p(weight), n_tokens, hidden_size, eps, _p(row_max), _p(zero_tokens), stream), "rmsnorm_rowmax")


def launch_silu_mul_rowmax(output, gate, up, n_tokens, width, row_max, stream=None):
    check(_lib.lib().ntk_silu_mul_rowmax(_p(output), _p(gate), _p(up), n_tokens, width, _p(row_max), stream), "silu_mul_rowmax")


def sample_top_k(logits, n, recent, n_recent, repeat_penalty, temperature, top_k, top_p, r, d_out, stream=None):
    L = _lib.lib()
    L.ntk_sample_scratch_bytes.restype = C.c_size_t
    scratch = DeviceBuffer(int(L.ntk_sample_scratch_bytes(C.c_int(n))))
    L.ntk_sample_top_k.argtypes = [C.c_void_p, C.c_int, C.c_void_p, C.c_int, C.c_float, C.c_float, C.c_int, C.c_float, C.c_float,
                                   C.c_void_p, C.c_void_p, C.c_void_p, C.c_void_p]
    st = L.ntk_sample_top_k(_p(logits), n, _p(recent), n_recent, repeat_penalty, temperature, top_k, top_p, r, _p(d_out), None,
                            _p(scratch), stream)
    synchronize()
    return st


def sample_rows_top_k(logits, n_rows, vocab, ld, recent, recent_ld, rows, d_out, stream=None, null=()):
    L = _lib.lib()
    if not isinstance(rows, _lib.SampleRows):
        sr = _lib.SampleRows()
        for b, (temperature, top_k, top_p, repeat_penalty, r, n_recent) in enumerate(rows):
            sr.temperature[b], sr.top_k[b], sr.top_p[b], sr.repeat_penalty[b], sr.r[b], sr.n_recent[b] = temperature, top_k, top_p, repeat_penalty, r, n_recent
        rows = sr
    scratch = DeviceBuffer(int(L.ntk_sample_rows_scratch_bytes(min(max(n_rows, 1), 16), min(max(vocab, 1), 1 << 20))))
    arg = lambda name, v: None if name in null else v
    st = L.ntk_sample_rows_top_k(arg("logits", _p(logits)), n_rows, vocab, ld, _p(recent), recent_ld, arg("rows", C.pointer(rows)), arg("d_out", _p(d_out)), None,
                                 arg("scratch", _p(scratch)), stream)
    synchronize()
    return st


def gemm_quant(Y, W, X, n_tokens, out_features, in_features, dtype, resid=None, stream=None):
    check(_lib.lib().ntk_gemm_quant(_p(Y), _p(W), _p(X), n_tokens, out_features, in_features, int(dtype), _p(resid),
                                    stream), "gemm_quant")


def attention_decode_fused(output, q, k, v, k_cache, v_cache, d_pos, n_heads, n_kv_heads, head_dim, max_seq, scale,
                           theta_base, freq_scale=1.0, inv_freq=None, stream=None):
    check(_lib.lib().ntk_attention_decode_fused(_p(output), _p(q), _p(k), _p(v), _p(k_cache), _p(v_cache), _p(d_pos),
                                                _p(inv_freq), n_heads, n_kv_heads, head_dim, max_seq, scale, theta_base,
                                                freq_scale, stream), "attention_decode_fused")


def attention_decode_split(output, q, k, v, k_cache, v_cache, d_pos, n_heads, n_kv_heads, head_dim, max_seq, scale,
                           theta_base, nsplit, freq_scale=1.0, inv_freq=None, stream=None):
    scratch = DeviceBuffer(int(_lib.lib().ntk_attention_split_scratch_bytes(n_heads, head_dim, nsplit)))
    check(_lib.lib().ntk_attention_decode_split(_p(output), _p(q), _p(k), _p(v), _p(k_cache), _p(v_cache), _p(d_pos),
                                                _p(inv_freq), n_heads, n_kv_heads, head_dim, max_seq, scale, theta_base,
                                                freq_scale, nsplit, _p(scratch), stream), "attention_decode_split")
    synchronize()
    return None


def attention_decode_split_merged(output, q, k, v, k_cache, v_cache, d_pos, n_heads, n_kv_heads, head_dim, max_seq, scale,
                                  theta_base, nsplit, freq_scale=1.0, inv_freq=None, stream=None, launches=1):
    scratch = DeviceBuffer(int(_lib.lib().ntk_attention_split_scratch_bytes(n_heads, head_dim, nsplit)))
    check(_lib.lib().ntk_attention_split_scratch_init(_p(scratch), n_heads, stream), "attention_split_scratch_init")
    for _ in range(launches):
        check(_lib.lib().ntk_attention_decode_split_merged(_p(output), _p(q), _p(k), _p(v), _p(k_cache), _p(v_cache), _p(d_pos),
                                                           _p(inv_freq), n_heads, n_kv_heads, head_dim, max_seq, scale, theta_base,
                                                           freq_scale, nsplit, _p(scratch), stream), "attention_decode_split_merged")
    synchronize()
    return None


def attention_decode_batch(output, q, k, v, k_caches, v_caches, positions, n_rows, n_heads, n_kv_heads, head_dim, max_seq, scale,
                           theta_base, nsplit=1, freq_scale=1.0, inv_freq=None, stream=None, table=True):
    L = _lib.lib()
    kv = _lib.KvBatch()
    for b, (kc, vc) in enumerate(zip(k_caches, v_caches)):
        kv.k[b], kv.v[b] = _p(kc), _p(vc)
    scratch = DeviceBuffer(max(n_rows, 1) * int(L.ntk_attention_split_scratch_bytes(n_heads, head_dim, nsplit)))
    check(L.ntk_attention_decode_batch(_p(output), _p(q), _p(k), _p(v), C.addressof(kv) if table else None, _p(positions), n_rows, _p(inv_freq),
                                       n_heads, n_kv_heads, head_dim, max_seq, scale, theta_base, freq_scale, nsplit, _p(scratch), stream),
          "attention_decode_batch")
    synchronize()
    return None


def kv_segments(segments, k_caches=None, v_caches=None, n_seg=None, row0=None):
    d = _lib.KvSegments()
    d.n_seg = len(segments) if n_seg is None else n_seg
    row = 0
    for s, (n, start) in enumerate(segments[:16]):
        d.row0[s], d.n_rows[s], d.start_pos[s] = (row if row0 is None else row0[s]), n, start
        row += n
        for side, caches in ((d.k, k_caches), (d.v, v_caches)):
            c = caches[s] if caches is not None else None
            side[s] = c if c is None or isinstance(c, int) else _p(c)
    return d


def kv_segments_validate(desc, total_rows, max_seq) -> int:
    return int(_lib.lib().ntk_kv_segments_validate(C.addressof(desc) if desc is not None else None, int(total_rows), int(max_seq)))


def rope_kv_store_segments(q, k, v, desc, n_heads, n_kv_heads, head_dim, theta_base, max_seq, freq_scale=1.0, interleaved=False, stream=None) -> int:
    return int(_lib.lib().ntk_rope_kv_store_segments(_p(q), _p(k), _p(v), C.addressof(desc) if desc is not None else None, n_heads, n_kv_heads, head_dim,
                                                     theta_base, freq_scale, int(interleaved), max_seq, stream))


def attention_prefill_segments(output, Q, desc, n_heads, n_kv_heads, head_dim, max_seq, scale, stream=None) -> int:
    return int(_lib.lib().ntk_attention_prefill_segments(_p(output), _p(Q), C.addressof(desc) if desc is not None else None, n_heads, n_kv_heads, head_dim,
                                                         max_seq, scale, stream))


def embed_rows(out, table, tokens, n_tokens, hidden, dtype, stream=None, allow_unsupported=False):
    st = _lib.lib().ntk_embed_rows(_p(out), _p(table), _p(tokens), n_tokens, hidden, int(dtype), stream)
    if not (allow_unsupported and st == -1):
        check(st, "embed_rows")
    return st


def argmax(logits, n, d_out_token, scratch, h_mirror=None, stream=None):
    check(_lib.lib().ntk_argmax(_p(logits), n, _p(d_out_token), _p(h_mirror), _p(scratch), stream), "argmax")


def logprob_rows(logits, n_rows, vocab, ld, targets, logprob, top1=None, stream=None):
    check(_lib.lib().ntk_logprob_rows(_p(logits), n_rows, vocab, ld, _p(targets), _p(logprob), _p(top1), stream), "logprob_rows")


def advance_pos(d_pos, stream=None):
    check(_lib.lib().ntk_advance_pos(_p(d_pos), stream), "advance_pos")


def sclk_mhz(stream=None) -> float:
    import numpy as np
    b = DeviceBuffer.zeros(24)
    check(_lib.lib().ntk_debug_sclk(_p(b), stream), "sclk probe")
    synchronize(stream)
    v = b.numpy(np.uint64)
    return 100.0 * float(v[0]) / max(float(v[1]), 1.0)


class SclkSpan:

    def __enter__(self):
        L = _lib.lib()
        self.flag, self.out = DeviceBuffer.zeros(8), DeviceBuffer.zeros(24)
        self.mhz = None
        check(L.ntk_debug_sclk_begin(_p(self.flag), _p(self.out), L.ntk_stream(1)), "sclk begin")
        return self

    def __exit__(self, *exc):
        import numpy as np
        L = _lib.lib()
        check(L.ntk_debug_sclk_end(_p(self.flag), L.ntk_stream(2)), "sclk end")
        check(L.ntk_stream_synchronize(L.ntk_stream(2)), "sync")
        check(L.ntk_stream_synchronize(L.ntk_stream(1)), "sync")
        v = self.out.numpy(np.uint64)
        if v[1] > 0:
            self.mhz = 100.0 * float(v[0]) / float(v[1])
        return False
```

Baseline: 553.8 tokens/s.

## Place decode activations in a static device arena so GEMV prologue loads x early

Adds a __device__ global arena holding the hidden state, attention output and FFN gate activations, and makes the batch-1 decode path use those buffers. When the GEMV input pointer matches an arena slot, specialised lane-major Q8_0 kernel variants load x from the compile-time symbol address before waiting on the kernel-argument loads. This overlaps the activation fetch with kernarg latency at the start of each of the roughly five GEMV launches per layer. The cost is a process-wide single-owner arena per device, new template instantiations, hardcoded 4096/14336 input widths, and a fallback to the old path when ownership, shapes or configuration do not fit.

```diff
diff --git a/include/ntk_engine.h b/include/ntk_engine.h
--- a/include/ntk_engine.h
+++ b/include/ntk_engine.h
@@ -33,6 +33,17 @@
 int ntk_gemv_rp(float* y, const void* rp, const float* x, int out_features, int in_features, int weight_dtype, void* stream);
 int ntk_gemv_rp_fused(const ntk_gemv_seg* segs, int nseg, const float* x, int in_features, const float* norm_w, float eps,
                       const float* resid, int silu_pair, void* stream);
+#define NTK_ARENA_HIDDEN 1
+#define NTK_ARENA_ATTN_OUT 2
+#define NTK_ARENA_GATE 3
+#define NTK_ARENA_HIDDEN_FLOATS 8192
+#define NTK_ARENA_ATTN_FLOATS 8192
+#define NTK_ARENA_GATE_FLOATS 32768
+int ntk_decode_arena_acquire(void);
+void ntk_decode_arena_release(int device);
+float* ntk_decode_arena_slot(int slot);
+int ntk_debug_gemv_static_x(void);
+
 int ntk_debug_rp_prologue(uint8_t* out, const float* x, const float* norm_w, float eps, int in_features, int nsub, int nwaves, void* stream);
 int ntk_debug_mfma_i8_probe(int* D, const int8_t* A, const int8_t* B, void* stream);
 
diff --git a/ntransformer_amd/_lib.py b/ntransformer_amd/_lib.py
--- a/ntransformer_amd/_lib.py
+++ b/ntransformer_amd/_lib.py
@@ -118,6 +118,8 @@
         "ntk_rp_unpack": (i, [vp, vp, i, i, i, vp]),
         "ntk_gemv_rp": (i, [vp, vp, vp, i, i, i, vp]),
         "ntk_gemv_rp_fused": (i, [C.POINTER(GemvSeg), i, vp, i, vp, f, vp, i, vp]),
+        "ntk_decode_arena_acquire": (i, []), "ntk_decode_arena_release": (None, [i]),
+        "ntk_decode_arena_slot": (vp, [i]), "ntk_debug_gemv_static_x": (i, []),
         "ntk_debug_rp_prologue": (i, [vp, vp, vp, f, i, i, i, vp]),
         "ntk_debug_mfma_i8_probe": (i, [vp, vp, vp, vp]),
         "ntk_gemm_quant": (i, [vp, vp, vp, i, i, i, i, vp, vp]),
diff --git a/ntransformer_amd/csrc/engine/capi.cpp b/ntransformer_amd/csrc/engine/capi.cpp
--- a/ntransformer_amd/csrc/engine/capi.cpp
+++ b/ntransformer_amd/csrc/engine/capi.cpp
@@ -72,6 +72,13 @@
         const std::string v = value;
         if (v != "0" && v != "1") { E(e)->set_error("batch_kv_q8 must be 0 or 1"); return NTK_E_SHAPE; }
         const int rc = E(e)->loaded() ? (E(e)->set_error("batch_kv_q8 must be set before the model is loaded"), NTK_E_SHAPE) : E(e)->model().set_batch_kv_q8(on);
+        if (rc != NTK_OK && !E(e)->loaded()) E(e)->set_error(E(e)->model().error());
+        return rc;
+    }
+    else if (k == "static_activations") {
+        const std::string v = value;
+        if (v != "0" && v != "1") { E(e)->set_error("static_activations must be 0 or 1"); return NTK_E_SHAPE; }
+        const int rc = E(e)->loaded() ? (E(e)->set_error("static_activations must be set before the model is loaded"), NTK_E_SHAPE) : E(e)->model().set_static_activations(on);
         if (rc != NTK_OK && !E(e)->loaded()) E(e)->set_error(E(e)->model().error());
         return rc;
     }
diff --git a/ntransformer_amd/csrc/engine/model.cpp b/ntransformer_amd/csrc/engine/model.cpp
--- a/ntransformer_amd/csrc/engine/model.cpp
+++ b/ntransformer_amd/csrc/engine/model.cpp
@@ -31,6 +31,10 @@
     stream_ = nullptr;
     for (void* p : allocs_) nt_hip_free(p);
     allocs_.clear();
+    if (arena_owner_) ntk_decode_arena_release(arena_device_);
+    arena_owner_ = false;
+    arena_device_ = -1;
+    hidden1_ = arena_attn_ = arena_gate_ = nullptr;
     auto free_host = [](auto*& p) { if (p) nt_hip_free_host(p); p = nullptr; };
     free_host(h_token_); free_host(h_ring_); free_host(h_recent_); free_host(h_batch_recent_); free_host(h_batch_next_);
     sample_scratch_ = gemm_ws_ = gemm_ws2_ = nullptr;
@@ -206,6 +210,12 @@
     return NTK_OK;
 }
 
+int Model::set_static_activations(bool on) {
+    if (!layers_.empty()) { err_ = "static_activations must be set before the model is loaded"; return NTK_E_SHAPE; }
+    static_act_ = on;
+    return NTK_OK;
+}
+
 int Model::set_kv_cache(const std::string& kind) {
     if (kind != "f16" && kind != "q8_0") { err_ = "kv_cache: unknown format '" + kind + "' (f16 or q8_0)"; return NTK_E_DTYPE; }
     if (!layers_.empty()) { err_ = "kv_cache must be set before the model is loaded"; return NTK_E_SHAPE; }
@@ -248,7 +258,7 @@
     if (persistent_plan_ && persistent_on_)
         return attn_regime_ == 0 ? "persistent (1 launch per token in the single-pass attention regime, fused launches beyond)"
                                  : "fused (5 launches/layer; persistent below the split-attention regime)";
-    return "fused (5 launches/layer)";
+    return arena_owner_ ? "fused (5 launches/layer; static activations)" : "fused (5 launches/layer)";
 }
 
 int Model::check_persistent() {
@@ -256,10 +266,12 @@
     return check_experiments();
 }
 
-Model::Views Model::views(int T) const {
+Model::Views Model::views(int T, bool fused) const {
     const size_t qd = (size_t)T * cfg_.n_heads * cfg_.head_dim, kvd = (size_t)T * cfg_.n_kv_heads * cfg_.head_dim;
     float* const q = workspace_;
-    return {q, q + qd, q + qd + kvd, q + qd + 2 * kvd, workspace_, workspace_ + (size_t)T * cfg_.intermediate_size};
+    Views v{q, q + qd, q + qd + kvd, q + qd + 2 * kvd, workspace_, workspace_ + (size_t)T * cfg_.intermediate_size};
+    if (fused && T == 1 && arena_owner_) { v.attn_out = arena_attn_; v.gate = arena_gate_; }
+    return v;
 }
 
 int Model::init_device() {
diff --git a/ntransformer_amd/csrc/engine/model.h b/ntransformer_amd/csrc/engine/model.h
--- a/ntransformer_amd/csrc/engine/model.h
+++ b/ntransformer_amd/csrc/engine/model.h
@@ -52,6 +52,8 @@
     int set_sequences(int n);
     int sequences() const { return sequences_; }
     int set_batch_kv_q8(bool on);
+    int set_static_activations(bool on);
+    bool static_activations_active() const { return arena_owner_; }
     bool batch_kv_q8() const { return batch_kv_q8_; }
     int decode_batch(const int* slots, const int* tokens, const int* positions, int B, float* logits_out, int* next_out);
     static constexpr int kMaxRecent = 4096;
@@ -154,7 +156,7 @@
     void free_all();
     void drop_graphs(int slot = -1);
     struct Views { float *q, *k, *v, *attn_out, *gate, *up; };
-    Views views(int T) const;
+    Views views(int T, bool fused = false) const;
     int enqueue_token(bool greedy);
     int enqueue_layers(int first, int last);
     int decode_project(const DevTensor* const* ws, float* const* ys, int n, const float* x, const DevTensor* norm, const float* resid, int kind,
@@ -205,6 +207,12 @@
     float* kv_capture_ = nullptr;
     int kv_capture_layer_ = -1, kv_capture_T_ = 0;
     float* hidden_ = nullptr;
+    float* hidden1_ = nullptr;
+    bool static_act_ = true;
+    bool arena_owner_ = false;
+    int arena_device_ = -1;
+    float* arena_attn_ = nullptr;
+    float* arena_gate_ = nullptr;
     float* residual_ = nullptr;
     float* workspace_ = nullptr;
     size_t workspace_floats_ = 0;
diff --git a/ntransformer_amd/csrc/engine/model_debug.cpp b/ntransformer_amd/csrc/engine/model_debug.cpp
--- a/ntransformer_amd/csrc/engine/model_debug.cpp
+++ b/ntransformer_amd/csrc/engine/model_debug.cpp
@@ -9,7 +9,8 @@
     if (tp_world_ > 1) return NTK_E_SHAPE;
     const size_t bytes = (size_t)T * cfg_.hidden_size * 4;
     void* s = stream_;
-    NT_TRY(ntk_memcpy_h2d_async(hidden_, hidden_in, bytes, s));
+    float* const hid = mode == 0 ? hidden_ : hidden1_;
+    NT_TRY(ntk_memcpy_h2d_async(hid, hidden_in, bytes, s));
     int rc;
     if (mode == 0) {
         std::vector<int> pos(T);
@@ -32,7 +33,7 @@
         }
     }
     if (rc != NTK_OK) return rc;
-    NT_TRY(ntk_memcpy_d2h_async(hidden_out, hidden_, bytes, s));
+    NT_TRY(ntk_memcpy_d2h_async(hidden_out, hid, bytes, s));
     return ntk_stream_synchronize(s);
 }
 
diff --git a/ntransformer_amd/csrc/engine/model_decode.cpp b/ntransformer_amd/csrc/engine/model_decode.cpp
--- a/ntransformer_amd/csrc/engine/model_decode.cpp
+++ b/ntransformer_amd/csrc/engine/model_decode.cpp
@@ -25,7 +25,7 @@
     void* s = stream_;
     tp_call_ = 0;
     prof_mark(2, true);
-    const int est = ntk_embed_rows(hidden_, token_embd_.ptr, d_token_, 1, H, token_embd_.dtype, s);
+    const int est = ntk_embed_rows(hidden1_, token_embd_.ptr, d_token_, 1, H, token_embd_.dtype, s);
     prof_mark(2, false);
     if (est != NTK_OK && est != NTK_E_DTYPE) return est;
     if (use_persistent_now()) {
@@ -35,7 +35,7 @@
         const DevTensor* const w = &output_;
         const bool timed = is_quant(w->dtype);
         if (timed) prof_mark(0, true);
-        NT_TRY(decode_project(&w, &logits_, 1, hidden_, &output_norm_, nullptr, 16, 0, false));
+        NT_TRY(decode_project(&w, &logits_, 1, hidden1_, &output_norm_, nullptr, 16, 0, false));
         if (timed) prof_mark(0, false);
     }
     prof_mark(2, true);
@@ -111,19 +111,19 @@
     const int H = cfg_.hidden_size, I = cfg_.intermediate_size, hd = cfg_.head_dim, nh = cfg_.n_heads, nkv = cfg_.n_kv_heads;
     void* s = stream_;
     const float scale = 1.0f / sqrtf((float)hd);
-    const Views act = views(1);
+    const Views act = views(1, true);
     auto project_add = [&](const DevTensor& w, const float* x, int kind) -> int {
         const DevTensor* const wp = &w;
-        float* y = tp_world_ > 1 ? tp_slot() : hidden_;
-        NT_TRY(decode_project(&wp, &y, 1, x, nullptr, tp_world_ > 1 ? nullptr : hidden_, kind));
-        return tp_world_ > 1 ? tp_allreduce(hidden_, H) : (int)NTK_OK;
+        float* y = tp_world_ > 1 ? tp_slot() : hidden1_;
+        NT_TRY(decode_project(&wp, &y, 1, x, nullptr, tp_world_ > 1 ? nullptr : hidden1_, kind));
+        return tp_world_ > 1 ? tp_allreduce(hidden1_, H) : (int)NTK_OK;
     };
 
     for (int i = first; i < last_layer; ++i) {
         const LayerWeights& L = layers_[i];
         const DevTensor* const qkv[3] = {&L.wq, &L.wk, &L.wv};
         float* const qkv_out[3] = {act.q, act.k, act.v};
-        NT_TRY(decode_project(qkv, qkv_out, 3, hidden_, &L.attn_norm, nullptr, 1));
+        NT_TRY(decode_project(qkv, qkv_out, 3, hidden1_, &L.attn_norm, nullptr, 1));
         const int fused = fuse_attention_ ? attention_in_wo(L, i) : (int)NTK_E_SHAPE;
         if (fused != NTK_OK) {
             if (!not_taken(fused)) return fused;
@@ -145,7 +145,7 @@
         float* const ffn_out[2] = {act.gate, act.up};
         const bool pair = is_quant(L.w_gate.dtype) && L.w_gate.dtype == L.w_up.dtype;
         if (pair) prof_mark(0, true);
-        NT_TRY(decode_project(ffn, ffn_out, 2, hidden_, &L.ffn_norm, nullptr, 4, pair, !pair));
+        NT_TRY(decode_project(ffn, ffn_out, 2, hidden1_, &L.ffn_norm, nullptr, 4, pair, !pair));
         if (pair) prof_mark(0, false);
         else NT_TRY(ntk_silu_mul(act.gate, act.gate, act.up, I, s));
         NT_TRY(project_add(L.w_down, act.gate, 8));
diff --git a/ntransformer_amd/csrc/engine/model_load.cpp b/ntransformer_amd/csrc/engine/model_load.cpp
--- a/ntransformer_amd/csrc/engine/model_load.cpp
+++ b/ntransformer_amd/csrc/engine/model_load.cpp
@@ -358,7 +358,16 @@
         nt_hip_memcpy_h2d(rope_inv_freq_, f.data(), f.size() * 4);
     }
     if (sequences_ > 1) { NT_TRY(batch_buffers()); NT_TRY(batch_sample_buffers()); }
-    return NTK_OK;
-}
-
-}
+    hidden1_ = hidden_;
+    const bool fits = H <= NTK_ARENA_HIDDEN_FLOATS && (size_t)cfg_.n_heads * cfg_.head_dim <= NTK_ARENA_ATTN_FLOATS &&
+                      (size_t)cfg_.intermediate_size <= NTK_ARENA_GATE_FLOATS;
+    if (static_act_ && fits && !shares_weights_ && tp_world_ == 1 && !experiments_built() && (arena_device_ = ntk_decode_arena_acquire()) >= 0) {
+        arena_owner_ = true;
+        hidden1_ = ntk_decode_arena_slot(NTK_ARENA_HIDDEN);
+        arena_attn_ = ntk_decode_arena_slot(NTK_ARENA_ATTN_OUT);
+        arena_gate_ = ntk_decode_arena_slot(NTK_ARENA_GATE);
+    }
+    return NTK_OK;
+}
+
+}
diff --git a/ntransformer_amd/csrc/gemv.hip b/ntransformer_amd/csrc/gemv.hip
--- a/ntransformer_amd/csrc/gemv.hip
+++ b/ntransformer_amd/csrc/gemv.hip
@@ -3,7 +3,10 @@
 #include "ntk_experiments.h"
 #endif
 #include <algorithm>
+#include <atomic>
 #include <cmath>
+#include <cstddef>
+#include <mutex>
 #include <cstdio>
 #include <cstdlib>
 
@@ -16,11 +19,25 @@
 #endif
 
 enum { NS_ANY = 0, NS_ONE = 1, NS_SPLIT = 2 };
-template <int DT, bool NORM, bool XFAST, bool A16, bool ATT = false, bool XI = false, bool LM = false, int NSF = NS_ANY>
+
+enum { XS_NONE = 0, XS_HIDDEN = NTK_ARENA_HIDDEN, XS_ATTN = NTK_ARENA_ATTN_OUT, XS_GATE = NTK_ARENA_GATE };
+struct DecodeArena {
+    float hidden[NTK_ARENA_HIDDEN_FLOATS];
+    float attn_out[NTK_ARENA_ATTN_FLOATS];
+    float gate[NTK_ARENA_GATE_FLOATS];
+};
+__device__ __attribute__((aligned(256))) DecodeArena g_decode_arena;
+template <int XS> struct XSlot { static constexpr int IN = XS == XS_GATE ? 14336 : 4096; };
+template <int XS> __device__ __forceinline__ const float* xslot_ptr() {
+    return XS == XS_HIDDEN ? g_decode_arena.hidden : XS == XS_ATTN ? g_decode_arena.attn_out : g_decode_arena.gate;
+}
+
+template <int DT, bool NORM, bool XFAST, bool A16, bool ATT = false, bool XI = false, bool LM = false, int NSF = NS_ANY, int XS = XS_NONE>
 __device__ __forceinline__ void gemv_quant_body(const GemvParams& p, const int bid, const int nblk, const AttnFuse* attp = nullptr) {
     using F = Fmt<DT>;
     static_assert(!LM || (DT == NTK_DT_Q8_0 && !A16 && !ATT && !XI), "lane-major rows: Q8_0");
     static_assert(NSF == NS_ANY || LM, "compile-time slice forms: the lane-major kernels");
+    static_assert(XS == XS_NONE || (LM && XFAST && NSF != NS_ANY), "early-x forms: the lane-major kernels, fast prologue");
     constexpr int NL = LM ? 4 : F::NL;
     constexpr int STAGE = LM ? 0 : NL * 1024 + 64;
     extern __shared__ __attribute__((aligned(16))) uint8_t smem[];
@@ -29,19 +46,45 @@
 #endif
     GV_STAMP(0);
 #ifndef NTK_GEMV_NO_KARG_PREFETCH
-    {
-        const auto* ka = __builtin_amdgcn_kernarg_segment_ptr();
-        unsigned d0, d1, d2, d3, d4;
+    const auto* ka = __builtin_amdgcn_kernarg_segment_ptr();
+    unsigned d0, d1, d2, d3, d4;
+    if constexpr (XS == XS_NONE) {
         asm volatile("s_load_dword %0, %5, 0x0\n\ts_load_dword %1, %5, 0x40\n\ts_load_dword %2, %5, 0x80\n\ts_load_dword %3, %5, 0xc0\n\t"
                      "s_load_dword %4, %5, 0x100\n\ts_waitcnt lgkmcnt(0)"
                      : "=&s"(d0), "=&s"(d1), "=&s"(d2), "=&s"(d3), "=&s"(d4) : "s"(ka) : "memory");
-        __builtin_amdgcn_sched_barrier(0);
-    }
+    } else {
+        asm volatile("s_load_dword %0, %5, 0x0\n\ts_load_dword %1, %5, 0x40\n\ts_load_dword %2, %5, 0x80\n\ts_load_dword %3, %5, 0xc0\n\t"
+                     "s_load_dword %4, %5, 0x100"
+                     : "=&s"(d0), "=&s"(d1), "=&s"(d2), "=&s"(d3), "=&s"(d4) : "s"(ka) : "memory");
+    }
+    __builtin_amdgcn_sched_barrier(0);
 #endif
 
     const int tid = threadIdx.x;
     constexpr int XIT = 8, WIT = 4;
     u32x4 xv[XIT], wv[WIT];
+    if constexpr (XS != XS_NONE) {
+        constexpr int IN = XSlot<XS>::IN, step0 = 512 * 4;
+        const float* const xs = xslot_ptr<XS>();
+#pragma unroll
+        for (int i = 0; i < XIT; ++i) {
+            xv[i] = u32x4{0u, 0u, 0u, 0u};
+            if (i * step0 < IN) xv[i] = *reinterpret_cast<const u32x4*>(xs + min(tid * 4 + i * step0, IN - 4));
+        }
+        GV_STAMP(7);
+        __builtin_amdgcn_sched_barrier(0);
+#ifndef NTK_GEMV_NO_KARG_PREFETCH
+        asm volatile("s_waitcnt lgkmcnt(0)" : "+s"(d0), "+s"(d1), "+s"(d2), "+s"(d3), "+s"(d4) : : "memory");
+        __builtin_amdgcn_sched_barrier(0);
+#endif
+        if constexpr (NORM) {
+#pragma unroll
+            for (int i = 0; i < WIT; ++i) {
+                wv[i] = u32x4{0u, 0u, 0u, 0u};
+                if (i * step0 < IN) wv[i] = *reinterpret_cast<const u32x4*>(p.norm_w + min(tid * 4 + i * step0, IN - 4));
+            }
+        }
+    } else
     if constexpr (XFAST && !ATT) {
         const int step0 = (int)blockDim.x * 4;
 #pragma unroll
@@ -499,9 +542,9 @@
 #endif
 }
 
-template <bool NORM, bool XFAST, int NSF>
+template <bool NORM, bool XFAST, int NSF, int XS = XS_NONE>
 __global__ __launch_bounds__(512, Fmt<NTK_DT_Q8_0>::MINW) void gemv_q8l_kernel(const GemvParams p) {
-    gemv_quant_body<NTK_DT_Q8_0, NORM, XFAST, false, false, false, true, NSF>(p, (int)blockIdx.x, (int)gridDim.x);
+    gemv_quant_body<NTK_DT_Q8_0, NORM, XFAST, false, false, false, true, NSF, XS>(p, (int)blockIdx.x, (int)gridDim.x);
 }
 template <bool UNPACK>
 __global__ __launch_bounds__(256) void q8l_pack_kernel(uint8_t* __restrict__ dst, const uint8_t* __restrict__ src, const int rows, const int in,
@@ -784,9 +827,49 @@
     return last_launch_status();
 }
 
+constexpr int kArenaDevices = 16;
+struct ArenaDev {
+    std::atomic<int> known{0};
+    std::atomic<int> owned{0};
+    const float* addr[4] = {nullptr, nullptr, nullptr, nullptr};
+};
+static ArenaDev g_arena_dev[kArenaDevices];
+static std::mutex g_arena_mu;
+static thread_local int t_last_static_x = XS_NONE;
+
+static ArenaDev* arena_dev(bool lookup) {
+    int dev = -1;
+    if (hipGetDevice(&dev) != hipSuccess || dev < 0 || dev >= kArenaDevices) return nullptr;
+    ArenaDev& a = g_arena_dev[dev];
+    if (a.known.load(std::memory_order_acquire) == 0 && lookup) {
+        std::lock_guard<std::mutex> lk(g_arena_mu);
+        if (a.known.load(std::memory_order_relaxed) == 0) {
+            void* base = nullptr;
+            const bool ok = hipGetSymbolAddress(&base, HIP_SYMBOL(g_decode_arena)) == hipSuccess && base != nullptr;
+            if (ok) {
+                auto* f = static_cast<const float*>(base);
+                a.addr[XS_HIDDEN] = f + offsetof(DecodeArena, hidden) / 4;
+                a.addr[XS_ATTN] = f + offsetof(DecodeArena, attn_out) / 4;
+                a.addr[XS_GATE] = f + offsetof(DecodeArena, gate) / 4;
+            }
+            a.known.store(ok ? 1 : -1, std::memory_order_release);
+        }
+    }
+    return a.known.load(std::memory_order_acquire) == 1 ? &a : nullptr;
+}
+static int static_x_slot(const float* x, int in) {
+    const ArenaDev* a = arena_dev(false);
+    if (!a) return XS_NONE;
+    if (x == a->addr[XS_HIDDEN] && in == XSlot<XS_HIDDEN>::IN) return XS_HIDDEN;
+    if (x == a->addr[XS_ATTN] && in == XSlot<XS_ATTN>::IN) return XS_ATTN;
+    if (x == a->addr[XS_GATE] && in == XSlot<XS_GATE>::IN) return XS_GATE;
+    return XS_NONE;
+}
+
 int q8l_gemv_fused(const ntk_gemv_seg* segs, int nseg, const float* x, int in, const float* norm_w, float eps, const float* resid,
                    int silu_pair, hipStream_t st) {
     int ns, sc;
+    t_last_static_x = XS_NONE;
     if (!q8l_layout(in, ns, sc)) return NTK_E_SHAPE;
     for (int i = 0; i < nseg; ++i)
         if (reinterpret_cast<uintptr_t>(segs[i].W) & 15) return NTK_E_ALIGN;
@@ -812,7 +895,19 @@
     static int trace_counter = 0;
     L.p.trace_slot = trace_counter++;
 #endif
-    hipLaunchKernelGGL(table[norm_w ? 1 : 0][L.xfast ? 1 : 0][L.p.ns == 1 ? 0 : 1], dim3(L.grid), dim3(64 * L.nwaves), L.lds, st, L.p);
+    KernelFn fn = table[norm_w ? 1 : 0][L.xfast ? 1 : 0][L.p.ns == 1 ? 0 : 1];
+    if (L.xfast && L.nwaves == 8) {
+        const int xs = static_x_slot(x, in);
+        KernelFn early = nullptr;
+        if (xs == XS_HIDDEN && L.p.ns == 1 && norm_w) early = gemv_q8l_kernel<true, true, NS_ONE, XS_HIDDEN>;
+        else if (xs == XS_ATTN && L.p.ns == 1 && !norm_w) early = gemv_q8l_kernel<false, true, NS_ONE, XS_ATTN>;
+        else if (xs == XS_GATE && L.p.ns > 1 && !norm_w) {
+            static const bool raised = raise_lds_limit((const void*)gemv_q8l_kernel<false, true, NS_SPLIT, XS_GATE>);
+            if (raised || L.lds <= 64 * 1024) early = gemv_q8l_kernel<false, true, NS_SPLIT, XS_GATE>;
+        }
+        if (early && L.lds <= 160 * 1024) { fn = early; t_last_static_x = xs; }
+    }
+    hipLaunchKernelGGL(fn, dim3(L.grid), dim3(64 * L.nwaves), L.lds, st, L.p);
     return last_launch_status();
 }
 
@@ -896,6 +991,20 @@
 }
 #endif
 
+int ntk_decode_arena_acquire(void) {
+    ntk::ArenaDev* a = ntk::arena_dev(true);
+    int free_ = 0;
+    return a && a->owned.compare_exchange_strong(free_, 1) ? (int)(a - ntk::g_arena_dev) : -1;
+}
+void ntk_decode_arena_release(int device) {
+    if (device >= 0 && device < ntk::kArenaDevices) ntk::g_arena_dev[device].owned.store(0);
+}
+float* ntk_decode_arena_slot(int slot) {
+    const ntk::ArenaDev* a = ntk::arena_dev(true);
+    return a && slot >= NTK_ARENA_HIDDEN && slot <= NTK_ARENA_GATE ? const_cast<float*>(a->addr[slot]) : nullptr;
+}
+int ntk_debug_gemv_static_x(void) { return ntk::t_last_static_x; }
+
 size_t ntk_q8l_bytes(int rows, int in_features) { return ntk::q8l_bytes(rows, in_features); }
 int ntk_q8l_pack(void* dst, const void* raw, int rows, int in_features, void* stream) {
     if (!dst || !raw) return NTK_E_NULL;
diff --git a/ntransformer_amd/ops.py b/ntransformer_amd/ops.py
--- a/ntransformer_amd/ops.py
+++ b/ntransformer_amd/ops.py
@@ -209,6 +209,25 @@
         arr[i].W, arr[i].y, arr[i].rows, arr[i].dtype = _p(W), _p(y), rows, int(dt)
     check(_lib.lib().ntk_gemv_rp_fused(arr, len(segs), _p(x), in_features, _p(norm_w), eps, _p(resid), int(silu_pair),
                                        stream), "gemv_rp_fused")
+
+
+ARENA_HIDDEN, ARENA_ATTN_OUT, ARENA_GATE = 1, 2, 3
+
+
+def decode_arena_slot(slot: int) -> int:
+    p = _lib.lib().ntk_decode_arena_slot(int(slot))
+    if not p:
+        raise _lib.NtkError(-1, "ntk_decode_arena_slot(%d)" % slot)
+    return int(p)
+
+
+def upload_to(ptr: int, a: np.ndarray) -> None:
+    a = np.ascontiguousarray(a)
+    _lib.lib().nt_hip_memcpy_h2d(ptr, a.ctypes.data_as(C.c_void_p), a.nbytes)
+
+
+def gemv_static_x() -> int:
+    return int(_lib.lib().ntk_debug_gemv_static_x())
 
 
 def _gemm_quant_f16(segs, X, n_tokens, in_features, resid=None, row_max=None, partials=None, stream=None, keep=None, repacked=False, workspace=None,
```

New measurement: 561.6 tokens/s, median of 6. 1.01x the previous value.
